# KennethLangedal/GNN-MWVC

Hardware: AMD Instinct MI355X
Metric: GNN forward edges/sec (higher is better)
Workload: dtype f32

## Files before the change

gnn-mwvc_amd/csrc/gnnvc_engine.cpp:

```cpp
#include <cmath>

#include "gnnvc_engine_state.h"

namespace {

struct Cursor {
    const char *p, *end;
    bool token(std::string &out) {
        while (p < end && isspace((unsigned char)*p)) ++p;
        if (p >= end) return false;
        const char *s = p;
        while (p < end && !isspace((unsigned char)*p)) ++p;
        out.assign(s, p);
        return true;
    }
    bool size(uint32_t &v) {
        std::string t;
        if (!token(t)) return false;
        char *q = nullptr;
        unsigned long x = strtoul(t.c_str(), &q, 10);
        if (!q || *q) return false;
        v = (uint32_t)x;
        return true;
    }
// ... 147 lines not shown
            const bool model_end = bare || at + 2 == left;
            const int end = bare ? gnnvc::kEndNone : L[at + 1].kind == kRelu ? gnnvc::kEndRelu
                            : (L[at + 1].kind == kSigmoid && model_end) ? gnnvc::kEndSigmoid : -1;
            gok = sp.nd < gnnvc::kMaxDenseLayers && (int)L[at].k == k && end >= 0;
            if (!gok) break;
            if (sp.nd == 0) sp.param_offset = L[at].w_off;
            sp.wn[sp.nd++] = k = (int)L[at].m;
            sp.end = end;
            sp.model_last = model_end;
            sp.sigmoid_last = end == gnnvc::kEndSigmoid;
            at += bare ? 1 : 2;
        }
        gok = gok && sp.nd >= 1 && (at == left || L[at].kind == kGraph);
        if (!gok) break;
        sp.n3 = sp.wn[sp.nd - 1];
        if (sp.nd == 3) { sp.n1 = sp.wn[0]; sp.n2 = sp.wn[1]; }
        sp.big_lds = e->big_lds;
        sp.feat_width = e->feat_width;
        gok = gnnvc::stage_any_fits(sp);
        gs.push_back(sp);
        f = sp.n3;
        i += at;
    }
    if (gok && !gs.empty()) e->gstages = std::move(gs);
}

int upload_params(gnnvc_engine *e) {
    std::vector<float> flat;
    for (const auto &l : e->layers)
        if (l.kind == kLinear) {
            flat.insert(flat.end(), l.W.begin(), l.W.end());
            flat.insert(flat.end(), l.bias.begin(), l.bias.end());
        }
    HIP_TRY(e, e->params.reserve(flat.size() + 64));
    if (!flat.empty())
        HIP_TRY(e, hipMemcpy(e->params.p, flat.data(), flat.size() * sizeof(float), hipMemcpyHostToDevice));
    return GNNVC_OK;
}

struct StageChoice {
    enum Sums {
        kGather,
        kLdsTable,
        kBlocked,
        kCompactPrepared,
        kCompactWhole,
        kTableTiles
    } sums = kGather;
    bool mfma = false;
    bool fused_counts = false;
    bool rounds = false;
    bool emit = false;
    bool emit_t4 = false;
    uint32_t long_thresh = 0xFFFFFFFFu;
    gnnvc::SortedOrder sorted;
};

int choose_stage(gnnvc_engine *e, int stage, uint32_t lo, uint32_t hi, const float *in, const float *out, bool in_forward,
                 StageChoice &c) {
    const bool longs = e->n_long > 0;
    const gnnvc::StagePlan &sp = e->stages[stage];
    if (e->pg.c4_prepared_stage != -1 && (stage != e->pg.c4_prepared_stage || out == e->c4_prepared_in)) e->pg.c4_prepared_stage = -1;
    const int fused_in = in_forward ? e->c4_fused_for : -1;
    e->c4_fused_for = -1;
    const bool may_emit = in_forward && e->pg.c4_ready && !e->pg.c4_range_mode && e->c4_base == 0 && e->c4_end == e->g.n && !longs &&
                          (size_t)stage + 1 < e->stages.size() && e->stages[stage + 1].f == 16 && lo == 0 && hi == e->g.n &&
                          e->opt.mfma != 1 && !e->pg.c4_stage_off[stage + 1];
    c.long_thresh = (sp.f == 16) ? e->thresh_f16 : e->long_thresh;
    c.mfma = e->opt.mfma == 1 || (e->opt.mfma == 2 && sp.f == 16);
    const bool t4 = in_forward && e->t4_now && lo == 0 && hi == e->g.n;
    c.emit_t4 = t4 && (size_t)stage + 1 < e->stages.size();
    if (stage == 0) {
        if (e->pg.graph_uses >= 1 && !e->pg.lt_tried) {
            int rc = build_lds_table(e);
            if (rc) return rc;
        }
        const uint32_t lt_need = std::min(192u, e->lt_chunks - e->lt_chunks / 4u);
        const bool lt_fits = e->pg.lt_ready && !e->pg.lt_off && hi > lo &&
                             (e->lt_mapped ? (lo == 0 && hi == e->g.n)
                                           : (lo >= e->lt_base && hi <= e->lt_end &&
                                              ((hi - 1 - e->lt_base) / e->lt_rows - (lo - e->lt_base) / e->lt_rows + 1) >= lt_need));
        if (e->pg.graph_uses >= 1 && !lt_fits && !e->pg.blocked_tried) {
            int rc = build_blocked(e);
            if (rc) return rc;
        }
        ++e->pg.graph_uses;
        c.sums = lt_fits ? StageChoice::kLdsTable : (e->pg.blocked_ready ? StageChoice::kBlocked : StageChoice::kGather);
        if (lt_fits && in_forward) e->pg.lt_used = true;
        if (lt_fits && e->lt_mapped) c.long_thresh = e->lt_plan_thresh;
        c.emit = may_emit;
        if (c.sums != StageChoice::kGather) return GNNVC_OK;
    } else if (sp.f == 16 && t4) {
        c.sums = StageChoice::kTableTiles;
    } else if (sp.f == 16) {
        const bool first_too = e->opt.compact_first_entries && e->g.nnz >= e->opt.compact_first_entries && lo == 0 && hi == e->g.n && in_forward;
        if (!e->pg.c4_range_mode && (e->pg.graph_uses >= 2 || first_too) && !e->pg.c4_tried) {
            int rc = build_compact(e);
            if (rc) return rc;
        }
        const bool whole_plan = e->pg.c4_ready && e->c4_base == 0 && e->c4_end == e->g.n && !e->pg.c4_stage_off[stage];
        const bool prepared = e->pg.c4_ready && e->pg.c4_prepared_stage == stage && e->c4_prepared_in == in &&
                              lo >= e->c4_base && hi <= e->c4_end && hi > lo;
        if (prepared && !longs) {
            const uint32_t nchunks = (hi - 1 - e->c4_base) / e->c4_rows - (lo - e->c4_base) / e->c4_rows + 1;
            if (nchunks >= 128u) c.sums = StageChoice::kCompactPrepared;
        } else if (!e->pg.c4_range_mode && whole_plan && !longs && (uint64_t)(hi - lo) * 2 >= e->g.n) {
// ... 41 lines not shown
        gr.off = e->gi_off.p;
        gr.slab = e->gi_slab.p;
        gr.agg = e->gi_agg.p;
        if (e->gi_maxseg > 1) {
            gr.segsum = e->gi_segsum.p;
            gr.segmap = e->gi_segmap.p;
            gr.maxseg = e->gi_maxseg;
        }
        gather_first = side && (e->opt.giant_gather_first < 0 ? (!long_on_main && (e->giant_entries <= (16ull << 20) || plain_f1))
                                                               : e->opt.giant_gather_first != 0);
        if (gather_first) HIP_TRY(e, gnnvc::launch_giant_stage(giant, gr, giant_from, gnnvc::GiantPart::kGather));
    }
    if (side) {
        HIP_TRY(e, hipEventRecord(e->ev_fork, e->stream));
        if (side_long) HIP_TRY(e, hipStreamWaitEvent(e->long_stream, e->ev_fork, 0));
    }
    if (e->n_giant) {
        if (long_on_main) HIP_TRY(e, hipStreamWaitEvent(e->giant_stream, e->ev_fork, 0));
        giant.stream = s_giant;
        HIP_TRY(e, gnnvc::launch_giant_stage(giant, gr, giant_from, gather_first ? gnnvc::GiantPart::kAfterGather : gnnvc::GiantPart::kAll));
        if (long_on_main) HIP_TRY(e, hipEventRecord(e->ev_giant, e->giant_stream));
    }
    const uint32_t long_from = gv.prune_eff ? std::min(thr, gv.eff_thresh) : thr;
    if ((e->n_giant < e->n_long || giant_from > e->giant_thresh) && long_from < giant_from) {
        gnnvc::StageCall lng = call;
        lng.stream = s_long;
        HIP_TRY(e, gnnvc::launch_long_stage(lng, {.list = e->long_list.p, .n = e->n_long, .min_deg = thr, .max_deg = giant_from}));
    }
    if (side_long) HIP_TRY(e, hipEventRecord(e->ev_long, e->long_stream));
    return GNNVC_OK;
}

int launch_main(gnnvc_engine *e, const StageChoice &c, const gnnvc::StageCall &call, const gnnvc::SortedOrder &so_p, int stage) {
    const gnnvc::StagePlan &sp = *call.sp;
    const GraphDev &gv = *call.g;
    const uint32_t lo = call.row_lo, hi = call.row_hi;
    const float *in = call.in;
    gnnvc::StageCall plain = call;
    plain.g = &e->g;
    gnnvc::EmitArgs emit;
    auto arm_emit = [&]() -> int {
        if (!c.emit) return GNNVC_OK;
        const bool zero = e->c4_emit_zero;
        e->c4_emit_zero = false;
        if (!zero) {
            ++e->plan_memsets;
            HIP_TRY(e, hipMemsetAsync(e->c4_emit_counts.p, 0, gnnvc::kEmitCounters * sizeof(unsigned long long), e->stream));
        }
        emit.spec = e->c4_desc.p + gnnvc_engine::kDescWords * stage;
        emit.table = e->c4_table.p;
        emit.counts = e->c4_emit_counts.p;
        e->c4_fused_for = stage + 1;
        return GNNVC_OK;
    };
    auto pilot = [&]() -> int {
        if (!c.emit || e->pg.c4_seeded[stage + 1] || !e->opt.pilot_rows) return GNNVC_OK;
        e->pg.c4_seeded[stage + 1] = true;
        const uint32_t rows = std::min(e->opt.pilot_rows, hi - lo);
        if ((uint64_t)rows * 8 > (uint64_t)(hi - lo)) return GNNVC_OK;
        uint32_t *cons = e->c4_desc.p + gnnvc_engine::kDescWords * stage;
        e->c4_emit_zero = false;
        ++e->plan_memsets;
        HIP_TRY(e, hipMemsetAsync(e->c4_emit_counts.p, 0, gnnvc::kEmitCounters * sizeof(unsigned long long), e->stream));
        gnnvc::EmitArgs pe;
        pe.spec = e->c4_desc.p + 2 * gnnvc_engine::kDescWords + 4;
        pe.table = e->c4_table.p;
        pe.counts = e->c4_emit_counts.p;
        gnnvc::StageCall first = plain;
        first.row_hi = lo + rows;
        first.logits = nullptr;
        HIP_TRY(e, gnnvc::launch_stage(first, {.interleave = true, .emit = pe}));
        HIP_TRY(e, gnnvc::compact_choose(e->c4_emit_counts.p, 64, rows, cons, 1u, e->stream, true));
        e->c4_emit_zero = true;
        return GNNVC_OK;
    };
    if (c.emit_t4) {
        const int cons = stage + 1;
        emit.spec = e->t4_desc_of(cons, e->t4_parity);
        emit.table = e->t4_table[cons - 1].p;
        emit.counts = e->t4_counts_of(cons, e->t4_parity);
    }
    if (c.sums == StageChoice::kTableTiles) {
        uint32_t *d_in = e->t4_desc_of(stage, e->t4_parity), *d_out = e->t4_desc_of(stage, e->t4_parity ^ 1u);
        const bool solo = e->t4_fit_seen[stage] && e->opt.t4_solo;
        HIP_TRY(e, gnnvc::launch_stage_t4(plain, {.table_in = e->t4_table[stage - 1].p,
                                                  .counts_in = e->t4_counts_of(stage, e->t4_parity),
                                                  .counts_zero = e->t4_counts_of(stage, e->t4_parity ^ 1u),
                                                  .desc_in = d_in, .desc_out = d_out, .emit = emit, .interleave = e->interleave, .solo = solo}));
        if (solo) return GNNVC_OK;
        return hip_rc(e, gnnvc::launch_stage(call, {.long_thresh = c.long_thresh, .mfma = c.mfma, .interleave = e->interleave,
                                                    .skip_flag = d_out + 8}));
    }
    if (c.sums == StageChoice::kLdsTable || c.sums == StageChoice::kBlocked) {
        int rc = pilot();
        if (rc) return rc;
        rc = arm_emit();
        if (rc) return rc;
    }
    if (c.sums == StageChoice::kLdsTable) {
        ++e->plan_memsets;
        return hip_rc(e, gnnvc::launch_stage0_lds_table(plain, lds_table_plan(e), e->lt_bytes.p, e->blk_acc.p, e->lt_bad.p,
                                                        {.long_thresh = c.long_thresh, .mfma = e->opt.mfma == 1,
                                                         .interleave = e->interleave, .emit = emit}));
    }
    if (c.sums == StageChoice::kBlocked)
        return hip_rc(e, gnnvc::launch_stage0_blocked(plain,
                                                      {.nblocks = e->blk_count, .bp = e->blk_ptr.p, .colb = e->blk_col.p, .acc = e->blk_acc.p},
                                                      {.long_thresh = e->long_thresh, .mfma = e->opt.mfma == 1,
                                                       .interleave = e->interleave, .emit = emit}));
    gnnvc::CompactSums sums;
    uint32_t *desc = nullptr;
    if (c.sums == StageChoice::kCompactPrepared || c.sums == StageChoice::kCompactWhole) {
        desc = e->c4_desc.p + gnnvc_engine::kDescWords * (stage - 1);
        e->c4_last_desc = gnnvc_engine::kDescWords * (stage - 1);
        if (c.sums == StageChoice::kCompactWhole) e->pg.fit_used[stage] = true;
        sums = {.acc4 = e->c4_acc.p, .c4desc = desc, .agg16 = e->c4_agg16.p, .table_in = (call.skip & 1u) ? e->c4_table.p : nullptr};
        const bool whole = c.sums == StageChoice::kCompactWhole;
        if (whole && !c.fused_counts) HIP_TRY(e, gnnvc::column_counts(in, e->g.n, e->c4_counts.p, e->stream));
        const bool fused = whole && c.fused_counts;
        const int what = !whole ? 2 : (c.rounds ? 1 : 3);
        if (fused) e->c4_emit_zero = false;
        if (!(what & 1)) ++e->plan_memsets;
        HIP_TRY(e, gnnvc::launch_compact_gather(e->g, compact_plan(e), in, fused ? e->c4_emit_counts.p : e->c4_counts.p, fused ? 64 : 1,
                                                desc, e->c4_table.p, e->c4_acc.p, lo, hi, e->c4_dirty.p, e->c4_dirty_cap,
                                                e->c4_agg16.p, e->stream, what, c.rounds ? e->c4_round_counts.p : nullptr, 256u * e->c4_rows, fused));
        if (fused) e->c4_emit_zero = true;
    }
    if (c.sums != StageChoice::kLdsTable && c.sums != StageChoice::kBlocked) {
        int rc = pilot();
        if (rc) return rc;
        rc = arm_emit();
        if (rc) return rc;
    }
    const gnnvc::SortedOrder *sop = c.sorted.n ? &c.sorted : nullptr;
    if (c.sums == StageChoice::kGather && e->opt.wide && e->g.n <= (sp.f == 16 ? e->opt.wide_max_n16 : e->opt.wide_max_n) && !e->g.sliced() && e->n_long == 0 && !sop &&
        !sums.acc4 && !emit.counts && gv.prune_bad == nullptr && gv.zero_bits == nullptr && sp.variant >= 0 && sp.variant <= 2) {
        e->pg.wide_used = true;
        e->stage_wide = true;
        return hip_rc(e, gnnvc::launch_stage_wide(plain));
    }
    HIP_TRY(e, gnnvc::launch_stage(call, {.long_thresh = c.long_thresh, .mfma = c.mfma, .so = sop, .interleave = e->interleave,
                                          .sums = sums, .mfma_agg = e->opt.mfma == 1, .emit = emit, .dense_part = !c.rounds,
                                          .so_pruned = so_p.vertex ? &so_p : nullptr}));
    if (!c.rounds) return GNNVC_OK;
    const uint32_t rows = e->c4_rows, c0 = (lo - e->c4_base) / rows, c1 = (hi - 1 - e->c4_base) / rows;
    const uint32_t nrounds = (c1 - c0) / 256u + 1u;
    if (nrounds > gnnvc::compact_rounds()) return fail(e, GNNVC_ERR_UNSUPPORTED, "too many rounds of the compact-table plan");
    {
        int rc = ensure_round_events(e, nrounds);
        if (rc) return rc;
    }
    for (uint32_t k = 0; k < nrounds; ++k) {
        const uint32_t ca = c0 + 256u * k, cb = std::min(c1 + 1u, ca + 256u);
        const uint32_t ra = std::max(lo, e->c4_base + ca * rows);
        const uint32_t rb = (uint32_t)std::min<uint64_t>(hi, (uint64_t)e->c4_base + (uint64_t)cb * rows);
        uint32_t *const count = e->c4_round_counts.p + k;
        const uint32_t slot_base = 256u * k * rows;
        HIP_TRY(e, gnnvc::compact_sums(e->g, compact_plan(e), desc, e->c4_table.p, e->c4_acc.p, ra, rb, e->c4_dirty.p, e->c4_dirty_cap,
                                       e->stream, count));
        const bool last = k + 1 == nrounds;
        hipStream_t ds = last ? e->stream : e->aux_stream;
        if (!last) {
            HIP_TRY(e, hipEventRecord(e->round_ev[k], e->stream));
            HIP_TRY(e, hipStreamWaitEvent(e->aux_stream, e->round_ev[k], 0));
        }
        HIP_TRY(e, gnnvc::compact_fix(e->g, in, desc, e->c4_dirty.p, e->c4_dirty_cap, e->c4_agg16.p, count, slot_base, ds,
                                      64));
        gnnvc::StageCall round = plain;
        round.row_lo = ra;
        round.row_hi = rb;
        round.stream = ds;
        HIP_TRY(e, gnnvc::launch_dense_sigmoid(round, sums, 0xFFFFFFFFu));
    }
    if (nrounds > 1) {
        HIP_TRY(e, hipEventRecord(e->ev_join, e->aux_stream));
        HIP_TRY(e, hipStreamWaitEvent(e->stream, e->ev_join, 0));
    }
    return GNNVC_OK;
}

std::string describe_stage(const gnnvc_engine *e, const StageChoice &c, const GraphDev &gv) {
    static const char *const kSums[] = {"gather", "lds_table", "blocked", "compact_prepared", "compact_whole", "table_tiles"};
    char buf[320];
    int at = snprintf(buf, sizeof buf, "sums=%s%s mfma=%d sorted_tiles=%d rounds=%d emit=%d pruned=%d filtered=%d short_lists=%d",
                      kSums[c.sums], e->stage_wide ? " (wide tiles)" : "", c.mfma ? 1 : 0, c.sorted.n ? 1 : 0, c.rounds ? 1 : 0,
                      (c.emit || c.emit_t4) ? 1 : 0, gv.prune_bad ? 1 : 0, gv.zero_bits ? 1 : 0, gv.short_col ? 1 : 0);
    if (e->n_long > 0 && at > 0 && at < (int)sizeof buf) {
        const char *lq = e->side_join == 1 ? "side" : "main";
        const char *gq = e->side_join == 0 ? "main" : (e->side_join == 1 ? "side" : "giant");
        at += snprintf(buf + at, sizeof buf - at, " long_rows=%u (from degree %u, %s queue)", e->n_long, c.long_thresh, lq);
        if (e->n_giant && at < (int)sizeof buf) snprintf(buf + at, sizeof buf - at, " giant_rows=%u (%s queue)", e->n_giant, gq);
    }
    return buf;
}

int run_stage(gnnvc_engine *e, int stage, uint32_t lo, uint32_t hi, const float *in, float *out, float *logits,
              bool in_forward = false, std::string *plan = nullptr) {
    e->stage_wide = false;
    StageChoice c;
    int rc = choose_stage(e, stage, lo, hi, in, out, in_forward, c);
    if (rc) return rc;
    const bool longs = e->n_long > 0;
    GraphDev gv;
    gnnvc::SortedOrder so_p;
    rc = gather_view(e, stage, lo, hi, in, c.sums == StageChoice::kGather, c.sorted.n != 0, gv, so_p, c.mfma, c.long_thresh);
    if (rc) return rc;
    gnnvc::StageCall call = stage_call(e, e->stages[stage], in, out, logits, lo, hi);
    call.g = &gv;
    if (longs) {
        rc = launch_side_rows(e, call, c.long_thresh, call.sp->f == 1 && c.sums == StageChoice::kGather);
        if (rc) return rc;
    }
    rc = launch_main(e, c, call, so_p, stage);
    if (rc) return rc;
    if (longs && e->side_join) {
        if (e->side_join == 1) HIP_TRY(e, hipStreamWaitEvent(e->stream, e->ev_long, 0));
        else if (e->n_giant) HIP_TRY(e, hipStreamWaitEvent(e->stream, e->ev_giant, 0));
    }
    if (plan) *plan = describe_stage(e, c, gv);
    return GNNVC_OK;
}

bool audit_tick(gnnvc_engine *e) {
    if (!e->opt.audit_period) return false;
    return ++e->audit_calls % e->opt.audit_period == 0;
}

int audit_stage(gnnvc_engine *e, int stage, uint32_t lo, uint32_t hi, const float *in, float *out, float *logits, std::string &plan,
                bool hook = true) {
    const std::vector<StagePlan> &st = e->stage_list();
    const size_t slot = e->audit_pending.size();
    if (slot == 0) {
        HIP_TRY(e, e->audit_rec.reserve(std::max<size_t>(st.size(), 1) * gnnvc::kAuditWords));
        HIP_TRY(e, hipMemsetAsync(e->audit_rec.p, 0, e->audit_rec.cap * sizeof(unsigned long long), e->stream));
    }
    if (slot >= st.size()) return fail(e, GNNVC_ERR_STATE, "more audited stages than the model has");
    const gnnvc::StagePlan &sp = st[stage];
    if (hook && e->opt.audit_flip_stage == stage && e->opt.audit_flip_row >= lo && e->opt.audit_flip_row < hi)
        HIP_TRY(e, gnnvc::launch_audit_flip(out, (size_t)e->opt.audit_flip_row * (size_t)sp.n3, e->stream));
    const gnnvc::StageCall call = stage_call(e, sp, in, out, sp.sigmoid_last ? logits : nullptr, lo, hi);
    unsigned long long *rec = e->audit_rec.p + slot * gnnvc::kAuditWords;
    if (e->generic_on()) HIP_TRY(e, gnnvc::launch_audit_any(call, rec, e->opt.audit_repair != 0));
    else HIP_TRY(e, gnnvc::launch_audit_stage(call, rec, e->opt.audit_repair != 0));
    e->audit_pending.push_back(gnnvc_engine::AuditCheck{stage, lo, hi, std::move(plan)});
    return GNNVC_OK;
}

int audit_finish(gnnvc_engine *e, int rc) {
    if (!e->audit_now) return rc;
    e->audit_now = false;
    std::vector<gnnvc_engine::AuditCheck> checks;
    checks.swap(e->audit_pending);
    if (rc != GNNVC_OK || checks.empty()) return rc;
    const size_t words = checks.size() * gnnvc::kAuditWords;
    HIP_TRY(e, e->audit_pin.reserve(std::max(e->stage_list().size(), checks.size()) * gnnvc::kAuditWords));
// ... 589 lines not shown
            unsigned long long info[2] = {0, 0};
            if (hipStreamSynchronize(e->stream) != hipSuccess ||
                hipMemcpy(info, e->filter_info.p + 4 * st, sizeof info, hipMemcpyDeviceToHost) != hipSuccess)
                return GNNVC_ERR_DEVICE;
            *value = (long)(info[0] * 100ull / e->g.nnz);
        }
    }
    else if (k == "pruned_vertices_stage1" || k == "pruned_vertices_stage2") *value = e->prune[k.back() - '0'].ready ? (long)e->prune[k.back() - '0'].members : 0;
    else if (k == "pruned_entries_stage1" || k == "pruned_entries_stage2") *value = e->prune[k.back() - '0'].ready ? (long)e->prune[k.back() - '0'].kept : 0;
    else if (k == "pruned_predicted_stage1") *value = e->prune[1].ready && e->prune[1].predicted ? 1 : 0;
    else if (k == "pruned_borrowed_stage2") *value = e->borrowed[2] ? 1 : 0;
    else if (k == "pruned_from_previous_stage2") *value = e->prune[2].ready && e->prune[2].from_prev ? 1 : 0;
    else if (k == "pruned_last_ok_stage1" || k == "pruned_last_ok_stage2") {
        const int st = k.back() - '0';
        *value = 0;
        if (e->prune[st].ready || e->borrowed[st]) {
            uint32_t bad = 1;
            if (hipSetDevice(e->device) != hipSuccess || hipStreamSynchronize(e->stream) != hipSuccess ||
                hipMemcpy(&bad, e->prune_flags.p + st, sizeof bad, hipMemcpyDeviceToHost) != hipSuccess)
                return GNNVC_ERR_DEVICE;
            *value = bad == 0 ? 1 : 0;
        }
    }
    else if (k == "wide_tiles_used") *value = e->pg.wide_used ? 1 : 0;
    else if (k == "table_tiles_active") *value = e->t4_ok ? 1 : 0;
    else if (k == "table_tiles_fit_stage1" || k == "table_tiles_fit_stage2") {
        *value = 0;
        if (e->t4_ok && e->t4_desc.p) {
            uint32_t fit = 0;
            gnnvc_engine *m = const_cast<gnnvc_engine *>(e);
            if (hipSetDevice(e->device) != hipSuccess || hipStreamSynchronize(e->stream) != hipSuccess ||
                hipMemcpy(&fit, m->t4_desc_of(k.back() - '0', e->t4_parity) + 8, sizeof fit, hipMemcpyDeviceToHost) != hipSuccess)
                return GNNVC_ERR_DEVICE;
            *value = (long)fit;
        }
    }
    else if (k == "lds_table_off") *value = e->pg.lt_off ? 1 : 0;
    else if (k == "lds_table_bits") *value = e->pg.lt_ready ? (long)e->lt_bits : 0;
    else if (k == "compact_gather_off_stage1" || k == "compact_gather_off_stage2") *value = e->pg.c4_stage_off[k.back() - '0'] ? 1 : 0;
    else if (k == "compact_gather_blocks") *value = e->pg.c4_ready ? (long)e->c4_nblocks : 0;
    else if (k == "compact_gather_last_ok" || k == "compact_gather_last_dirty" || k == "compact_gather_last_passes" ||
             k == "compact_table_written_by_producer") {
        *value = 0;
        if (e->pg.c4_ready && e->c4_desc.p) {
            uint32_t d[8] = {0};
            if (hipSetDevice(e->device) != hipSuccess || hipStreamSynchronize(e->stream) != hipSuccess ||
                hipMemcpy(d, e->c4_desc.p + e->c4_last_desc, sizeof d, hipMemcpyDeviceToHost) != hipSuccess)
                return GNNVC_ERR_DEVICE;
            if (k == "compact_table_written_by_producer") *value = (d[0] && !d[6]) ? 1 : 0;
            else *value = k == "compact_gather_last_ok" ? (d[0] ? 1 : 0) : (k == "compact_gather_last_passes" ? (long)d[0] : (long)d[5]);
        }
    }
    else if (k == "plan_memsets_last_forward") *value = (long)e->plan_memsets;
    else if (k == "lds_table_active") *value = e->pg.lt_ready ? 1 : 0;
    else if (k == "lds_table_last_ok") {
        *value = 0;
        if (e->pg.lt_ready && e->lt_bad.p) {
            uint32_t bad = 1;
            if (hipSetDevice(e->device) != hipSuccess || hipStreamSynchronize(e->stream) != hipSuccess ||
                hipMemcpy(&bad, e->lt_bad.p, sizeof bad, hipMemcpyDeviceToHost) != hipSuccess)
                return GNNVC_ERR_DEVICE;
            *value = bad == 0 ? 1 : 0;
        }
    }
    else if (k == "lds_table_mapped") *value = e->pg.lt_ready && e->lt_mapped ? 1 : 0;
    else if (k == "lds_table_blocks") *value = e->pg.lt_ready ? (long)e->lt_blocks : 0;
    else if (k == "lds_table_chunks") *value = e->pg.lt_ready ? (long)e->lt_chunks : 0;
    else if (k == "lds_table_steps") *value = e->pg.lt_ready ? (long)e->lt_steps_total : 0;
    else if (k == "blocked_stage0_active") *value = e->pg.blocked_ready ? 1 : 0;
    else if (k == "blocked_blocks") *value = e->pg.blocked_ready ? (long)e->blk_count : 0;
    else if (k == "block_cols") *value = e->pg.blocked_ready ? (long)e->blk_cols : 0;
    else if (k == "long_rows") *value = (long)e->n_long;
    else if (k == "plan_build_us") *value = (long)(e->pg.plan_build_ms * 1000.0);
    else if (k == "handoff_build_us") *value = (long)(e->handoff_build_ms * 1000.0);
    else if (k == "handoff_early_us") *value = (long)(e->pg.early_ms * 1000.0);
    else if (k == "graph_uses") *value = (long)e->pg.graph_uses;
    else if (k == "slice_rows") *value = e->empty_slice ? 0 : (long)(e->g.hi() - e->g.lo());
    else if (k == "slice_entries") *value = (long)e->g.nnz;
    else if (k == "giant_rows") *value = (long)e->n_giant;
    else if (k == "giant_segments") *value = e->n_giant ? (long)e->gi_maxseg : 0;
    else if (k == "giant_entries") *value = (long)e->giant_entries;
    else if (k == "giant_row_threshold") *value = e->n_giant ? (long)e->giant_thresh : 0;
    else if (k == "sorted_tiles_active") *value = e->sorted_wanted ? 1 : 0;
    else if (k == "tile_waste_x100") *value = (long)(e->srt_waste * 100.0);
    else if (k == "heavy_tail_x1000") *value = (long)(e->srt_tail * 1000.0);
    else if (k == "interleaved_tiles") *value = e->interleave ? 1 : 0;
    else if (k == "long_row_threshold") *value = e->n_long ? (long)e->long_thresh : 0;
    else return GNNVC_ERR_INVALID;
    return GNNVC_OK;
}

int gnnvc_num_layers(const gnnvc_engine *e) { return e ? (int)e->layers.size() : GNNVC_ERR_INVALID; }
int gnnvc_is_fused(const gnnvc_engine *e) { return e ? (e->stage_list().empty() ? 0 : 1) : GNNVC_ERR_INVALID; }
int gnnvc_in_width(const gnnvc_engine *e) { return e ? e->in_width : GNNVC_ERR_INVALID; }
int gnnvc_out_width(const gnnvc_engine *e) { return e ? e->out_width : GNNVC_ERR_INVALID; }
int gnnvc_num_stages(const gnnvc_engine *e) { return e ? (int)e->stage_list().size() : GNNVC_ERR_INVALID; }

int gnnvc_stage_widths(const gnnvc_engine *e, int stage, int *in_width, int *out_width) {
    if (!e || stage < 0 || stage >= (int)e->stage_list().size()) return GNNVC_ERR_INVALID;
    if (in_width) *in_width = e->stage_list()[stage].f;
    if (out_width) *out_width = e->stage_list()[stage].n3;
    return GNNVC_OK;
}

extern "C++" {
template <class RP>
// ... 494 lines not shown
        if (e->stage_list().empty()) return fail(e, GNNVC_ERR_UNSUPPORTED, "model is not fused into stages: there is nothing to audit");
        e->audit_now = true;
    } else {
        e->audit_now = audit && !e->stages.empty() && !e->generic_on();
    }
    const int rc = audit_finish(e, forward_single(e, d_x, d_scores, d_logits));
    if (audit && e->opt.audit_log) audit_log_line(e, rc);
    return rc;
}

int gnnvc_forward_device(gnnvc_engine *e, const float *d_x, float *d_scores, float *d_logits) {
    if (!e) return GNNVC_ERR_INVALID;
    return forward_device_impl(e, d_x, d_scores, d_logits, audit_tick(e), false);
}

int gnnvc_forward_audited_device(gnnvc_engine *e, const float *d_x, float *d_scores, float *d_logits) {
    if (!e) return GNNVC_ERR_INVALID;
    return forward_device_impl(e, d_x, d_scores, d_logits, true, true);
}

static int forward_single(gnnvc_engine *e, const float *d_x, float *d_scores, float *d_logits) {
    if (!e->have_graph) return fail(e, GNNVC_ERR_STATE, "no graph attached");
    const uint32_t n = e->g.n;
    e->ev_count = 0;
    e->live_seen.clear();
    if (e->layers.empty()) return fail(e, GNNVC_ERR_STATE, "engine was created without a model");
    if (n == 0) return GNNVC_OK;
    if (e->g.sliced() || e->empty_slice)
        return fail(e, GNNVC_ERR_STATE, "this engine holds a slice of the graph: run it stage by stage (gnnvc_stage_forward_device)");
    if (!d_x || !d_scores) return fail(e, GNNVC_ERR_INVALID, "null feature buffers");
    int rc = use_device(e);
    if (rc) return rc;
    e->plan_memsets = 0;
    e->generic_ran = e->generic_on();
    e->heavy_last_rows = 0;
    e->ggiant_last_rows = 0;
    e->ggiant_last_segmented = false;
    if (e->generic_ran || e->stages.empty()) {
        rc = ensure_events(e, 2);
        if (rc) return rc;
        if (e->opt.timing >= 1) HIP_TRY(e, hipEventRecord(e->ev[0], e->stream));
        rc = e->generic_ran ? forward_generic(e, d_x, d_scores, d_logits) : forward_unfused(e, d_x, d_scores, d_logits);
        if (rc) return rc;
        if (e->opt.timing >= 1) HIP_TRY(e, hipEventRecord(e->ev[1], e->stream));
        e->ev_count = e->opt.timing >= 1 ? 2 : 0;
        e->ev_stages = false;
        return GNNVC_OK;
    }
    const size_t ns = e->stages.size();
    rc = ensure_events(e, ns + 1);
    if (rc) return rc;
    const float *cur = d_x;
    e->c4_fused_for = -1;
    e->pg.c4_prepared_stage = -1;
    if (e->pg.fit_pending && hipEventQuery(e->ev_fit) == hipSuccess) {
        e->pg.fit_pending = false;
        const uint32_t before = e->pg.lt_unfit_runs + e->t4_unfit_runs + e->pg.c4_unfit_runs[1] + e->pg.c4_unfit_runs[2];
        const bool seen1 = e->t4_fit_seen[1], seen2 = e->t4_fit_seen[2];
        if (e->pg.lt_used && e->pg.lt_ready) {
            e->pg.lt_unfit_runs = e->fit_pin.p[2] != 0u ? e->pg.lt_unfit_runs + 1 : 0u;
            if (e->pg.lt_unfit_runs >= (e->lt_mapped ? 1u : 3u)) e->pg.lt_off = true;
        }
        if (e->t4_used && e->t4_ok) {
            e->t4_unfit_runs = e->fit_pin.p[3] == 0u ? e->t4_unfit_runs + 1 : 0u;
            if (e->t4_unfit_runs >= 4u) e->t4_ok = false;
            e->t4_fit_seen[1] = e->fit_pin.p[3] != 0u;
            e->t4_fit_seen[2] = e->fit_pin.p[4] != 0u;
        }
        for (int s = 1; s <= 2; ++s) {
            if (!e->pg.fit_used[s]) continue;
            if (s == 2 && e->pg.fit_used[1] && e->fit_pin.p[0] == 0u) continue;
            e->pg.c4_unfit_runs[s] = e->fit_pin.p[s - 1] == 0u ? e->pg.c4_unfit_runs[s] + 1 : 0u;
            if (e->pg.c4_unfit_runs[s] >= 3u) e->pg.c4_stage_off[s] = true;
        }
        const uint32_t after = e->pg.lt_unfit_runs + e->t4_unfit_runs + e->pg.c4_unfit_runs[1] + e->pg.c4_unfit_runs[2];
        const bool calm = after == 0u && before == 0u && seen1 == e->t4_fit_seen[1] && seen2 == e->t4_fit_seen[2];
        e->pg.fit_calm = calm ? e->pg.fit_calm + 1u : 0u;
    }
    if (!e->pg.fit_pending) {
        for (int s = 0; s < 4; ++s) e->pg.fit_used[s] = false;
        e->pg.lt_used = false;
        e->t4_used = false;
    }
    struct SinkGuard {
        ~SinkGuard() { gnnvc::set_kernel_trace(nullptr); }
    } sink_guard;
    if (e->opt.ktrace && e->ktrace.used < 16384) {
        e->ktrace.stream = e->stream;
        gnnvc::set_kernel_trace(&e->ktrace);
    }
    e->t4_now = e->t4_ok && (e->t4_choice_live || e->pg.graph_uses >= 1);
    const bool build_under_stage0 = ns >= 2 && !e->pg.c4_tried && !e->pg.c4_range_mode && e->aux_stream && e->n_long == 0 && !e->sorted_wanted &&
                                    e->opt.compact_first_entries && e->g.nnz >= e->opt.compact_first_entries;
    if (e->opt.timing >= 1 || build_under_stage0) HIP_TRY(e, hipEventRecord(e->ev[0], e->stream));
    if (e->opt.poison)
        for (size_t b = 0; b + 1 < ns && b < 2; ++b) HIP_TRY(e, hipMemsetAsync(e->h[b].p, 0xFF, (size_t)n * 16 * sizeof(float), e->stream));
    for (size_t s = 0; s < ns; ++s) {
        const bool last = s + 1 == ns;
        float *dst = last ? d_scores : e->h[s & 1].p;
        std::string plan;
        rc = run_stage(e, (int)s, 0, n, cur, dst, last ? d_logits : nullptr, true, e->audit_now ? &plan : nullptr);
        if (rc) break;
        if (e->audit_now && (rc = audit_stage(e, (int)s, 0, n, cur, dst, last ? d_logits : nullptr, plan)) != GNNVC_OK) break;
        if ((e->opt.timing >= 2 || (last && e->opt.timing == 1)) && hipEventRecord(e->ev[s + 1], e->stream) != hipSuccess) { rc = fail(e, GNNVC_ERR_DEVICE, "hipEventRecord failed"); break; }
        if (s == 0 && build_under_stage0 && !e->pg.c4_tried) {
            HIP_TRY(e, hipStreamWaitEvent(e->aux_stream, e->ev[0], 0));
// ... 511 lines not shown
```

gnn-mwvc_amd/csrc/gnnvc_engine_state.h:

```cpp
#pragma once
#include <hip/hip_runtime_api.h>

#include <algorithm>
#include <chrono>
#include <cctype>
#include <cstdarg>
#include <cstdio>
#include <cstdlib>
#include <cstring>
#include <new>
#include <string>
#include <vector>

#include "../../include/gnnvc.h"
#include "gnnvc_device_mem.h"
#include "gnnvc_kernels.h"
#include "gnnvc_multi.h"
#include "gnnvc_options.h"

using gnnvc::GraphDev;
using gnnvc::StagePlan;

namespace gnnvc_eng {

// ... 13 lines not shown
using gnnvc::PinBuf;
using gnnvc_eng::Layer;
using namespace gnnvc_eng;

struct gnnvc_engine {
    int device = 0;
    gnnvc::MultiState *multi = nullptr;
    std::string name;
    std::vector<Layer> layers;
    std::vector<StagePlan> stages;
    std::vector<StagePlan> gstages;
    bool generic_ran = false;
    uint32_t big_lds = 0;
    uint32_t feat_width = 0;
    uint32_t patterns = 0;
    uint32_t live_percent = 0;
    std::vector<uint8_t> live_seen;
    bool generic_on() const { return !gstages.empty() && (opt.generic == 2 || (opt.generic == 1 && stages.empty())); }
    const std::vector<StagePlan> &stage_list() const { return generic_on() ? gstages : stages; }
    uint32_t heavy_from = 512;
    uint32_t heavy_last_rows = 0;
    uint32_t ggiant_from = 16384;
    int ggiant_segments = -1;
    uint32_t ggiant_last_rows = 0;
    bool ggiant_last_segmented = false;
    int in_width = 1, out_width = 1;
    int max_width = 1;
    bool ends_in_sigmoid = false;
    float ws = 120.0f;

    gnnvc::Options opt;
    gnnvc::Stream own_stream, aux_stream;
    hipStream_t stream = nullptr;
    std::vector<gnnvc::Event> ev;
    int ev_count = 0;
    bool ev_stages = false;

    DevBuf<float> params;
    struct PerGraph {
        bool wide_used = false;
        bool blocked_ready = false, blocked_tried = false;
        uint32_t graph_uses = 0;
        bool lt_ready = false, lt_tried = false;
        bool lt_used = false, lt_off = false;
        uint32_t lt_unfit_runs = 0;
        bool c4_ready = false, c4_tried = false;
        bool c4_range_mode = false;
        int c4_prepared_stage = -1;
        bool c4_seeded[4] = {false, false, false, false};
        bool fit_pending = false, fit_used[4] = {false, false, false, false}, c4_stage_off[4] = {false, false, false, false};
        uint32_t c4_unfit_runs[4] = {0, 0, 0, 0};
        uint32_t fit_calm = 0;
        uint32_t fit_skip = 0;
        int short_from = 0;
        bool heavy_known = false;
        uint32_t heavy_rows = 0, heavy_thresh = 0;
        uint64_t heavy_entries = 0;
        uint32_t giant_from = 0, giant_rows = 0, giant_blocks = 0, giant_maxseg = 0, giant_min = 0xFFFFFFFFu;
        int giant_seg = -1;
        uint64_t giant_entries = 0;
        double plan_build_ms = 0.0;
        double early_ms = 0.0;
    };
    PerGraph pg;
    GraphDev g;
    bool have_graph = false;
    DevBuf<uint32_t> rowptr, col, w, nw;
    PinBuf<uint32_t> pin_rowptr, pin_col, pin_w, pin_nw;
    PinBuf<uint32_t> pin_small;
    uint32_t staged_n = 0;
    uint64_t staged_nnz = 0, staged_sent = 0;
    bool staging = false;
    DevBuf<float> x, h[2], scores, logits;
    DevBuf<float> scratch[2];
    DevBuf<float> live_table;
    DevBuf<unsigned long long> live_desc;

    uint32_t blk_count = 0, blk_cols = 0;
    DevBuf<uint32_t> blk_ptr, blk_col, blk_scratch, blk_flag;
    DevBuf<float> blk_acc;
    uint32_t lt_bits = 8;
    bool lt_mapped = false;
    uint32_t lt_plan_thresh = 0xFFFFFFFFu;
    DevBuf<uint32_t> lt_rowmap, lt_first, lt_bstart;
    uint32_t lt_rows = 0, lt_chunks = 0, lt_blocks = 0, lt_steps_total = 0, lt_last_entry = 0;
    uint32_t lt_base = 0, lt_end = 0;
    struct PlanBuild {
        bool open = false, mapped = false;
        uint32_t base = 0, end = 0, slice_rows = 0, slices = 0, chunks = 0, rows = 0, nblocks = 0, bc = 0, slack = 0, done = 0;
        uint32_t plan_rows = 0, passes = 1;
        uint64_t entry_cap = 0, plan_nnz = 0;
        gnnvc::PlanMap pm;
    };
    PlanBuild lt_pb, c4_pb;
    bool early_open = false, early_declined = false;
    gnnvc::Event ev_piece;
    DevBuf<uint8_t> lt_bytes;
    DevBuf<uint32_t> lt_entries, lt_segcnt, lt_stepptr, lt_stepcnt, lt_bad;
    DevBuf<uint4> lt_steps;
    uint32_t c4_rows = 0, c4_chunks = 0, c4_steps_total = 0, c4_block = 0, c4_last_entry = 0, c4_nblocks = 0;
    DevBuf<uint32_t> c4_entries, c4_segcnt, c4_stepptr, c4_stepcnt, c4_desc;
    uint32_t c4_nslices = 0;
    DevBuf<uint32_t> c4_map_vertex;
    DevBuf<uint32_t> map_coarse;
    DevBuf<uint4> c4_map_meta;
    DevBuf<uint4> c4_steps;
    DevBuf<float> c4_table, c4_acc, c4_agg16;
    DevBuf<uint32_t> c4_round_counts;
    std::vector<gnnvc::Event> round_ev;
    DevBuf<uint32_t> c4_dirty;
    uint32_t c4_dirty_cap = 0;
    DevBuf<unsigned long long> c4_counts, c4_emit_counts;
    uint32_t plan_memsets = 0;
    bool c4_emit_zero = false;
    uint32_t c4_base = 0, c4_end = 0;
    const float *c4_prepared_in = nullptr;
    int c4_fused_for = -1;
    struct PrunePlan {
        bool tried = false, ready = false, deferred = false;
        bool predicted = false, verified = false;
        void forget() { tried = ready = deferred = predicted = verified = false; }
        bool from_prev = false;
        uint64_t kept = 0;
        uint64_t members = 0;
        DevBuf<uint32_t> prp, pcol, heavy;
        DevBuf<uint32_t> svertex;
        DevBuf<uint4> smeta;
        uint32_t sn = 0;
        bool slist = false;
        uint32_t eff_thresh = 0xFFFFFFFFu;
    };
    PrunePlan prune[4];
    DevBuf<uint32_t> prune_flags, prune_scratch, prune_off;
    DevBuf<unsigned long long> prune_mask;
    int side_join = 0;
    DevBuf<uint32_t> filter_bits[4];
    DevBuf<unsigned long long> filter_info;
    bool filtered[4] = {false, false, false, false};
    bool borrowed[4] = {false, false, false, false};
    uint32_t short_min = 0, short_max = 0;
    bool short_used[4] = {false, false, false, false};
    PinBuf<uint32_t> fit_pin;
    gnnvc::Event ev_fit;
    int c4_last_desc = 0;
    static constexpr int kDescWords = 16;

    bool t4_ok = false;
    bool t4_used = false;
    bool t4_fit_seen[4] = {false, false, false, false};
    uint32_t t4_unfit_runs = 0;
    uint32_t *fit_dev = nullptr;
    bool t4_now = false;
    bool t4_choice_live = false;
    uint32_t t4_parity = 0;
    DevBuf<float> t4_table[2];
    DevBuf<uint32_t> t4_desc;
    DevBuf<unsigned long long> t4_counts[2];
    unsigned long long *t4_counts_of(int stage, uint32_t parity) { return t4_counts[stage - 1].p + (size_t)parity * gnnvc::kEmitCounters; }
    uint32_t *t4_desc_of(int stage, uint32_t parity) { return t4_desc.p + ((size_t)(stage - 1) * 2 + parity) * 16; }

    uint32_t thresh_f16 = 0xFFFFFFFFu;
    bool interleave = false;
    bool sorted_wanted = false;
    struct SortedRange {
        bool valid = false, use = false;
        uint32_t lo = 0, hi = 0, n = 0;
        uint64_t stamp = 0;
        DevBuf<uint32_t> vertex;
        DevBuf<uint4> meta;
// ... 172 lines not shown
```

gnn-mwvc_amd/csrc/gnnvc_kernels.h:

```cpp
#pragma once
#include <hip/hip_runtime_api.h>
#include <stdint.h>
#include <hip/hip_vector_types.h>

#include <atomic>
#include <vector>

#include "gnnvc_device_mem.h"

namespace gnnvc {

struct GraphDev {
    uint32_t n = 0;
    uint64_t nnz = 0;
    const uint32_t *rowptr = nullptr;
    const uint32_t *col = nullptr;
    const uint32_t *w = nullptr;
    const uint32_t *nw = nullptr;
    uint32_t row_base = 0, row_end = 0;
    const uint32_t *prp = nullptr, *pcol = nullptr, *prune_bad = nullptr;
    uint32_t prune_eff = 0, eff_giant = 0xFFFFFFFFu, eff_thresh = 0xFFFFFFFFu;
    const uint32_t *zero_bits = nullptr;
    const unsigned long long *zero_info = nullptr;
    uint32_t zero_min_pct = 50;
// ... 14 lines not shown
};

constexpr int kMaxDenseLayers = 6;
struct StagePlan {
    int f = 0;
    int n1 = 0, n2 = 0, n3 = 0;
    int sigmoid_last = 0;
    size_t param_offset = 0;
    int variant = -1;
    int nd = 3;
    int wn[kMaxDenseLayers] = {0, 0, 0, 0, 0, 0};
    uint32_t big_lds = 0;
    uint32_t feat_width = 0;
    int dense = 0;
    int end = 0;
    int model_last = 0;
    uint32_t patterns = 0;
    uint32_t skip_ok = 0;
};

struct SortedOrder {
    uint32_t n = 0;
    const uint32_t *vertex = nullptr;
    const uint4 *meta = nullptr;
};

struct KernelTraceSink {
    struct Rec {
        const char *name = nullptr;
        Event a, b;
    };
    hipStream_t stream = nullptr;
    std::vector<Rec> recs;
    size_t used = 0;
};
void set_kernel_trace(KernelTraceSink *sink);

int stage_variant(int f, int n1, int n2, int n3, int sigmoid_last);

struct StageCall {
    const StagePlan *sp = nullptr;
    const GraphDev *g = nullptr;
    float ws = 0.0f;
    const float *params = nullptr;
    const float *in = nullptr;
    float *out = nullptr, *logits = nullptr;
    uint32_t row_lo = 0, row_hi = 0;
    hipStream_t stream = nullptr;
    uint32_t skip = 0;
    float *live_table = nullptr;
    void *live_desc = nullptr;
};

struct EmitArgs {
    const uint32_t *spec = nullptr;
    float *table = nullptr;
    unsigned long long *counts = nullptr;
};
constexpr int kEmitCounters = 64 * 17;

struct CompactSums {
    const float *acc4 = nullptr;
    const uint32_t *c4desc = nullptr;
    const float *agg16 = nullptr;
    const float *table_in = nullptr;
};

struct TileArgs {
    uint32_t long_thresh = 0xFFFFFFFFu;
    bool mfma = false;
    const SortedOrder *so = nullptr;
    bool interleave = false;
    CompactSums sums;
    const uint32_t *skip_flag = nullptr;
    bool mfma_agg = false;
    EmitArgs emit;
    bool dense_part = true;
    const SortedOrder *so_pruned = nullptr;
};
hipError_t launch_stage(const StageCall &c, const TileArgs &a);
struct GraphClassArgs {
    bool cuts = false, waste = false, longs = false;
    uint32_t waste_thresh = 0xFFFFFFFFu, heavy_from = 1, long_thresh = 0xFFFFFFFFu;
    uint32_t *long_list = nullptr;
};
hipError_t classify_graph(const GraphDev &g, const GraphClassArgs &a, uint32_t *dev_words, uint32_t *out_dev, hipStream_t stream);

struct VerdictWords {
    const uint32_t *src[8] = {nullptr, nullptr, nullptr, nullptr, nullptr, nullptr, nullptr, nullptr};
};
hipError_t write_verdicts(const VerdictWords &vw, uint32_t *out_dev, hipStream_t stream);

constexpr int kAuditWords = 8;
hipError_t launch_audit_stage(const StageCall &c, unsigned long long *rec, bool repair);
hipError_t launch_audit_any(const StageCall &c, unsigned long long *rec, bool repair);
hipError_t launch_audit_flip(float *out, size_t at, hipStream_t stream);

constexpr int kAnyMaxF = 32, kAnySmallHidden = 64, kAnyBigHidden = 128, kAnyMaxLast = 32;
constexpr int kAnyFeatMax = 64;
constexpr uint32_t kPatternPrologue = 1u, kPatternOpenEnd = 2u;
enum { kEndRelu = 0, kEndSigmoid = 1, kEndNone = 2 };
struct AnyRoute {
    bool ok = false, big = false, feat = false;
    int threads = 256;
    size_t lds256 = 0, lds = 0;
};
AnyRoute stage_any_route(const StagePlan &sp);
bool stage_any_fits(const StagePlan &sp);
hipError_t allow_big_stages();
hipError_t allow_feat_stages();
hipError_t allow_dynamic_lds(const void *func, int bytes, std::atomic<uint64_t> &done);
struct AnyHeavyRows {
    const uint32_t *list = nullptr;
    uint32_t n = 0, from = 0;
    float *hsum = nullptr;
    uint32_t below = 0xFFFFFFFFu;
};
enum class AnyRows { kAll, kLight, kListed };
hipError_t launch_stage_any(const StageCall &c, AnyRows rows = AnyRows::kAll, const AnyHeavyRows &hr = AnyHeavyRows());
hipError_t launch_any_heavy_sums(const StageCall &c, const AnyHeavyRows &hr);
hipError_t launch_any_live(const StageCall &c, uint32_t max_percent);

hipError_t launch_stage_wide(const StageCall &c);
struct TableTileArgs {
    const float *table_in = nullptr;
    const unsigned long long *counts_in = nullptr;
    unsigned long long *counts_zero = nullptr;
    const uint32_t *desc_in = nullptr;
    uint32_t *desc_out = nullptr;
// ... 16 lines not shown

hipError_t find_long_rows(const GraphDev &g, uint32_t thresh, uint32_t *list, uint32_t *count,
                          hipStream_t stream);
struct LongRows {
    const uint32_t *list = nullptr;
    uint32_t n = 0, min_deg = 0, max_deg = 0xFFFFFFFFu;
};
hipError_t launch_long_stage(const StageCall &c, const LongRows &lr);

struct GiantRows {
    uint32_t n = 0, blocks = 0;
    const void *meta = nullptr;
    const unsigned long long *off = nullptr;
    float *slab = nullptr, *agg = nullptr;
    float *segsum = nullptr;
    void *segmap = nullptr;
    uint32_t maxseg = 0;
};
uint32_t giant_segments(uint32_t len);
uint32_t giant_window();
uint32_t giant_block();
hipError_t find_giant_rows(const GraphDev &g, const uint32_t *list, uint32_t n_long, uint32_t thresh, void *meta, uint32_t *count,
                           hipStream_t stream);
enum class GiantPart { kAll, kGather, kAfterGather };
hipError_t launch_giant_stage(const StageCall &c, const GiantRows &gr, uint32_t min_deg, GiantPart part);
hipError_t launch_giant_sums(const GiantRows &gr, uint32_t F, uint32_t row_lo, uint32_t row_hi, hipStream_t stream);

struct AnyGiantRows {
    GiantRows gr;
    const uint32_t *pos = nullptr;
};
hipError_t find_any_giant_rows(const GraphDev &g, const uint32_t *list, uint32_t n_list, uint32_t thresh, void *meta, uint32_t *count,
                               hipStream_t stream);
enum class AnyGiantPart { kGather, kPlace };
hipError_t launch_any_giant(const StageCall &c, const AnyGiantRows &ar, float *hsum, AnyGiantPart part);
hipError_t stream_sums(const float *streams_dev, uint32_t streams, uint32_t len, void *meta, unsigned long long *off, float *agg,
                       int mode , hipStream_t stream, float *segsum = nullptr,
                       void *segmap = nullptr);

size_t blocked_scan_scratch_elems(size_t n_elems);
hipError_t build_blocked_index(const GraphDev &g, uint32_t wb, uint32_t nblocks, uint32_t long_thresh,
                               uint32_t *bp, uint32_t *colb, uint32_t *scratch, uint32_t *bad_flag,
                               hipStream_t stream);
struct BlockedPlan {
    uint32_t nblocks = 0;
    const uint32_t *bp = nullptr, *colb = nullptr;
    float *acc = nullptr;
};
struct Stage0Args {
    uint32_t long_thresh = 0xFFFFFFFFu;
    bool mfma = false;
    bool interleave = false;
    EmitArgs emit;
};
hipError_t launch_stage0_blocked(const StageCall &c, const BlockedPlan &bp, const Stage0Args &a);

hipError_t launch_graph_layer(const GraphDev &g, float ws, uint32_t f, const float *in,
                              float *out, hipStream_t stream);
hipError_t launch_linear(uint32_t n, uint32_t k, uint32_t m, const float *in, const float *W,
                         const float *bias, float *out, hipStream_t stream);
hipError_t launch_relu(size_t count, const float *in, float *out, hipStream_t stream);
hipError_t launch_sigmoid(size_t count, const float *in, float *out, hipStream_t stream);
hipError_t launch_sgemm(int ta, int tb, uint32_t m, uint32_t n, uint32_t k, const float *A,
                        uint32_t lda, const float *B, uint32_t ldb, float beta, float *C,
                        uint32_t ldc, hipStream_t stream);

uint32_t lds_table_max_rows(uint32_t bits = 8);
uint32_t lds_table_bits_for(uint32_t kmax);
size_t lds_table_bytes_for(uint32_t bits, size_t n);
hipError_t lds_table_wmax(const uint32_t *w, uint32_t n, uint32_t *wmax, hipStream_t stream);
struct PlanMap {
    const uint32_t *rowmap = nullptr, *first = nullptr, *bstart = nullptr;
    const uint16_t *coarse = nullptr;
};
uint32_t lds_table_block(uint32_t bits = 8);
uint32_t lds_table_step();
uint32_t lds_table_record_words();
hipError_t lds_table_wsteps(const GraphDev &g, uint32_t slice_rows, uint32_t nchunks, uint32_t nblocks, const uint32_t *seg_cnt,
                            const uint32_t *step_ptr, uint32_t *step_count, uint32_t *recs, bool write, uint32_t slack,
                            hipStream_t stream, const PlanMap &pm = PlanMap(), uint32_t row_base = 0, uint32_t row_end = 0xFFFFFFFFu,
                            uint32_t bits = 8);
bool lds_table_is_flat(uint32_t rows_per_chunk, const PlanMap &pm = PlanMap());
hipError_t lds_table_count(const GraphDev &g, uint32_t rows_per_chunk, uint32_t nchunks, uint32_t nblocks, uint32_t block_cols,
                           uint32_t *seg_cnt, uint32_t *bad, hipStream_t stream, uint32_t row_base = 0,
                           uint32_t row_end = 0xFFFFFFFFu, const PlanMap &pm = PlanMap(), uint32_t chunk0 = 0,
                           uint32_t chunk1 = 0xFFFFFFFFu);
hipError_t lds_table_steps(const GraphDev &g, uint32_t rows_per_chunk, uint32_t nchunks, uint32_t nblocks, const uint32_t *seg_cnt,
                           const uint32_t *step_ptr, uint32_t *step_count, void *steps, bool write, hipStream_t stream,
                           uint32_t row_base = 0, uint32_t row_end = 0xFFFFFFFFu, uint32_t cap = 0 ,
                           uint32_t slack = 0 ,
                           uint32_t block_cols = 0 ,
                           const PlanMap &pm = PlanMap());
hipError_t lds_table_scatter(const GraphDev &g, uint32_t rows_per_chunk, uint32_t nchunks, uint32_t nblocks, uint32_t block_cols,
                             const uint32_t *seg_cnt, uint32_t *entries, hipStream_t stream, uint32_t shift,
                             uint32_t row_base, uint32_t row_end, uint32_t slack, const PlanMap &pm,
                             uint32_t *bad ,
                             uint32_t chunk0 = 0, uint32_t chunk1 = 0xFFFFFFFFu);
hipError_t prune_mark_zero(const GraphDev &g, const float *feat, uint32_t *heavy_bits, hipStream_t stream);
hipError_t predict_zero_rows(const StagePlan &sp0, const GraphDev &g, float ws, const float *params, uint32_t *heavy_bits, hipStream_t stream);
hipError_t filter_mark(const GraphDev &g, const float *feat, uint32_t *bits, unsigned long long *info, hipStream_t stream,
                       const uint32_t *prev_bits = nullptr, const unsigned long long *prev_info = nullptr);
hipError_t prune_mass(const GraphDev &g, const uint32_t *heavy_bits, unsigned long long *mass, hipStream_t stream,
                      const uint32_t *prev_bits = nullptr);
hipError_t prune_count(const GraphDev &g, const uint32_t *heavy_bits, unsigned long long *mask, uint32_t *off, uint32_t *scratch,
                       hipStream_t stream);
hipError_t prune_fill(const GraphDev &g, const unsigned long long *mask, const uint32_t *off, uint32_t *pcol, uint32_t *prp,
                      hipStream_t stream);
hipError_t prune_check(const GraphDev &g, const float *feat, const uint32_t *heavy_bits, uint32_t *bad, hipStream_t stream);
hipError_t deal_rows(const GraphDev &g, const uint32_t *sorted_rows, uint32_t m, uint32_t slice_rows, uint32_t nslices,
                     uint32_t *rowmap, uint32_t *weight, hipStream_t stream);
hipError_t mass_bounds(const GraphDev &g, unsigned long long target, uint32_t count, uint32_t *cand, hipStream_t stream);
struct LdsTablePlan {
    uint32_t rows_per_chunk = 0;
    uint32_t plan_base = 0, plan_end = 0xFFFFFFFFu;
    uint32_t bits = 8;
    uint32_t last_entry = 0;
    uint32_t mapped_chunks = 0;
    const uint32_t *step_ptr = nullptr;
    const void *steps = nullptr;
    const uint32_t *entries = nullptr;
    const uint32_t *rowmap = nullptr;
};
hipError_t launch_stage0_lds_table(const StageCall &c, const LdsTablePlan &lp, uint8_t *wbyte, float *acc, uint32_t *bad,
                                   const Stage0Args &a);

uint32_t compact_max_rows();
uint32_t compact_block();
uint32_t compact_shift();
uint32_t compact_slices();
uint32_t compact_step();
uint32_t compact_rounds();
struct CompactPlan {
    uint32_t rows_per_chunk = 0, block_cols = 0, nblocks = 0, plan_base = 0, plan_end = 0;
    uint32_t last_entry = 0;
    uint32_t nslices = 0;
    uint32_t max_passes = 1;
    const uint32_t *step_ptr = nullptr;
    const void *steps = nullptr;
    const uint32_t *entries = nullptr;
    const uint32_t *rowmap = nullptr;
};
hipError_t launch_compact_gather(const GraphDev &g, const CompactPlan &cp, const float *in, unsigned long long *counts,
                                 int count_slots, uint32_t *desc, float *table, float *acc4, uint32_t row_lo, uint32_t row_hi,
                                 uint32_t *dirty_rows, uint32_t dirty_cap, float *agg16, hipStream_t stream,
                                 int what = 3 ,
                                 uint32_t *round_counts = nullptr ,
                                 uint32_t round_stride = 0 ,
                                 bool clear_counts = false );

hipError_t compact_choose(unsigned long long *counts, int count_slots, uint32_t rows, uint32_t *desc, uint32_t max_passes,
                          hipStream_t stream, bool clear_counts = false);
hipError_t compact_sums(const GraphDev &g, const CompactPlan &cp, uint32_t *desc, const float *table, float *acc4, uint32_t row_lo,
                        uint32_t row_hi, uint32_t *dirty_rows, uint32_t dirty_cap, hipStream_t stream,
                        uint32_t *round_count = nullptr);
hipError_t compact_fix(const GraphDev &g, const float *in, uint32_t *desc, const uint32_t *dirty_rows, uint32_t dirty_cap,
                       float *agg16, const uint32_t *dirty_count, uint32_t slot_base, hipStream_t stream, uint32_t blocks = 1024);

hipError_t derive_tails(const GraphDev &old_g, const uint32_t *old_row, uint32_t n_new, const uint32_t *rowptr_new, uint32_t *new_of,
                        uint32_t *tail, uint32_t *bad, hipStream_t stream);
hipError_t derive_fill(const GraphDev &old_g, const uint32_t *old_row, const uint32_t *new_of, const uint32_t *rowptr_new,
                       const uint32_t *tail_ptr, const uint32_t *tail_cols, uint32_t n_new, uint32_t *col_new, hipStream_t stream);
hipError_t row_hashes(const GraphDev &g, unsigned long long *out, hipStream_t stream);

hipError_t score_keys(const float *scores, size_t n, float *keys, uint8_t *above_half, hipStream_t stream);

hipError_t live_columns(const float *feat, size_t rows, uint32_t *mask, hipStream_t stream);
hipError_t column_counts(const float *feat, size_t rows, unsigned long long *counts, hipStream_t stream);
hipError_t pack_rows(const float *feat, uint32_t row_lo, uint32_t row_hi, uint32_t mask, uint32_t kp, float *dense,
                     uint32_t *exc, uint32_t cap, uint32_t *flag, hipStream_t stream);
hipError_t unpack_rows(const float *dense, const uint32_t *exc, uint32_t cap, uint32_t row_lo, uint32_t row_hi,
                       uint32_t mask, uint32_t kp, float *feat, hipStream_t stream);

hipError_t unpack_gathered(const float *buf, uint32_t world, uint32_t skip, size_t piece_words, uint32_t dense_rows,
                           uint32_t cap, uint32_t per, uint32_t off, uint32_t size, uint32_t n, uint32_t mask, uint32_t kp,
                           float *feat, hipStream_t stream);

struct UnpackPiece {
    const float *region;
    uint32_t row_lo, row_hi;
};
hipError_t push_piece(const float *region, uint32_t rows, uint32_t kp, uint32_t cap, uint32_t n_dst, float *const *dst, hipStream_t stream);
hipError_t unpack_pieces(const UnpackPiece *pieces, uint32_t n_pieces, uint32_t cap, uint32_t mask, uint32_t kp, float *feat, hipStream_t stream);
hipError_t push_rows(const float *src, size_t words, uint32_t n_dst, float *const *dst, hipStream_t stream);

hipError_t launch_reduction_flags(const GraphDev &g, uint32_t max_degree, uint8_t *flags, hipStream_t stream);

hipError_t validate_graph(const GraphDev &g, uint32_t *flags, hipStream_t stream);
hipError_t validate_rowptr(const GraphDev &g, uint32_t *flags, hipStream_t stream);
hipError_t narrow_rowptr(const void *in_u64, uint32_t *out, size_t count, hipStream_t stream);

hipError_t streams_run_side_by_side(hipStream_t a, hipStream_t b, bool *yes);
hipError_t launch_zero_pad_row(float *buf, uint32_t n, uint32_t width, hipStream_t stream);

}
```

gnn-mwvc_amd/csrc/gnnvc_kernels.hip:

```cpp
#include <hip/hip_runtime.h>

#include <algorithm>
#include <atomic>

#include "exact_sum.h"
#include "expf_glibc.h"
#include "gnnvc_kernels.h"

namespace gnnvc {

namespace {

#ifndef GNNVC_PHASE_PROBE
#define GNNVC_PHASE_PROBE 0
#endif
#if GNNVC_PHASE_PROBE
__device__ unsigned long long *gnnvc_probe_buf = nullptr;
__device__ int gnnvc_probe_kind = 0;
__device__ __forceinline__ void probe_mark(int kind, int phase) {
    if (gnnvc_probe_buf && gnnvc_probe_kind == kind && (threadIdx.x & 63) == 0)
        gnnvc_probe_buf[((size_t)blockIdx.x * 4 + (threadIdx.x >> 6)) * 16 + phase] = wall_clock64();
}
#define GNNVC_PROBE(kind, phase) probe_mark(kind, phase)
#else
// ... 200 lines not shown
    float acc = 0.0f;
#pragma unroll
    for (int r = 0; r < 4; ++r) acc = __builtin_fmaf(d[r], w[r], acc);
    float t = __shfl_xor(acc, 32);
    acc = h ? t : acc;
#pragma unroll
    for (int r = 0; r < 4; ++r) acc = __builtin_fmaf(d[r], w[r], acc);
    t = __shfl_xor(acc, 32);
    acc = h ? acc : t;
#pragma unroll
    for (int r = 4; r < 8; ++r) acc = __builtin_fmaf(d[r], w[r], acc);
    t = __shfl_xor(acc, 32);
    acc = h ? t : acc;
#pragma unroll
    for (int r = 4; r < 8; ++r) acc = __builtin_fmaf(d[r], w[r], acc);
    return acc;
}

template <int N1, int N2, int N3, bool SIGMOID>
__device__ __forceinline__ void mfma_tail(f32x16 (&d)[2], const float *__restrict__ W2, const float *__restrict__ b2,
                                          const float *__restrict__ W3, const float *__restrict__ b3, float *T,
                                          int v, int h, float (&logit)[2]) {
    static_assert(N1 == 32, "layer-2 input is a full 32-feature tile");
    float a[16];
    mfma_load_a<N2, 16>(W2, v, h, a);
#pragma unroll
    for (int vt = 0; vt < 2; ++vt) {
        d[vt] = mfma_layer_acc<32>(d[vt], a);
        mfma_bias_act<N2, 0>(d[vt], b2, h);
    }
    if constexpr (SIGMOID) {
        static_assert(N2 == 16 && N3 == 1, "sigmoid tail is 16 -> 1");
#pragma unroll
        for (int vt = 0; vt < 2; ++vt) logit[vt] = mfma_tail_16to1(d[vt], W3, h) + b3[0];
    } else {
        static_assert(N3 == 16, "feature stages emit 16 floats per vertex");
        mfma_load_a<N3, N2 / 2>(W3, v, h, a);
#pragma unroll
        for (int vt = 0; vt < 2; ++vt) {
            d[vt] = mfma_layer_acc<N2>(d[vt], a);
            mfma_bias_act<N3, 0>(d[vt], b3, h);
        }
        wave_lds_sync();
#pragma unroll
        for (int vt = 0; vt < 2; ++vt)
#pragma unroll
            for (int r = 0; r < 8; ++r) T[(32 * vt + v) * kOutPitch + mfma_feat(r, h)] = d[vt][r];
    }
}

typedef float c4row __attribute__((ext_vector_type(4)));
constexpr int kEmitSlots = 64, kEmitStride = 17;

__device__ __forceinline__ void c4_emit_with(const float *trow, uint32_t nz, uint32_t u, bool mine, int lane, uint32_t spec_ok,
                                             uint32_t s0, uint32_t s1, uint32_t s2, uint32_t s3, c4row *__restrict__ table,
                                             unsigned long long *__restrict__ counts) {
    uint32_t my = 0;
#pragma unroll
    for (int cidx = 0; cidx < 16; ++cidx) {
        const uint32_t cnt = (uint32_t)__popcll(__ballot(mine && (nz >> cidx & 1u)));
        if (lane == cidx) my = cnt;
    }
    const uint32_t rows = (uint32_t)__popcll(__ballot(mine));
    if (lane == 16) my = rows;
    if (lane <= 16 && my) atomicAdd(&counts[(blockIdx.x & (kEmitSlots - 1)) * kEmitStride + lane], (unsigned long long)my);
    if (spec_ok == 1u && mine) {
        const float a = trow[s0], b = trow[s1], c = trow[s2], d = trow[s3];
        c4row out = {a == 0.0f ? 0.0f : a, b == 0.0f ? 0.0f : b, c == 0.0f ? 0.0f : c, d == 0.0f ? 0.0f : d};
        const bool odd = !(a >= 0.0f) || !(b >= 0.0f) || !(c >= 0.0f) || !(d >= 0.0f);
        if (odd || (nz & ~((1u << s0) | (1u << s1) | (1u << s2) | (1u << s3))))
            out[0] = __uint_as_float(__float_as_uint(out[0]) | 0x80000000u);
        if (odd) out[1] = __uint_as_float(__float_as_uint(out[1]) | 0x80000000u);
        table[u] = out;
    }
}
__device__ __forceinline__ void c4_emit(const float *trow, uint32_t nz, uint32_t u, bool mine, int lane,
                                        const uint32_t *__restrict__ spec, c4row *__restrict__ table,
                                        unsigned long long *__restrict__ counts) {
    const uint32_t ok = spec[0];
    c4_emit_with(trow, nz, u, mine, lane, ok, ok == 1u ? spec[1] : 0u, ok == 1u ? spec[2] : 0u, ok == 1u ? spec[3] : 0u,
                 ok == 1u ? spec[4] : 0u, table, counts);
}

template <int LANE>
__device__ __forceinline__ uint32_t put_lane(uint32_t v, uint32_t s ) {
    asm("v_writelane_b32 %0, %1, %2" : "+v"(v) : "s"(s), "n"(LANE));
    return v;
}
template <int J>
__device__ __forceinline__ void c4_count_cols(const float (&x)[16], unsigned long long mm, uint32_t tcols, uint32_t &my,
                                              unsigned long long &stray) {
    if constexpr (J < 16) {
        const unsigned long long nzj = __ballot(x[J] != 0.0f);
        my = put_lane<J>(my, (uint32_t)__popcll(nzj & mm));
        stray |= (tcols >> J & 1u) ? 0ull : nzj;
        c4_count_cols<J + 1>(x, mm, tcols, my, stray);
    }
}
__device__ __forceinline__ void c4_emit_regs(const float (&x)[16], const float *trow, uint32_t u, bool mine, int lane,
                                             const uint32_t *__restrict__ spec, c4row *__restrict__ table,
                                             unsigned long long *__restrict__ counts) {
    const uint32_t ok = spec[0];
    const uint32_t s0 = ok == 1u ? spec[1] : 0u, s1 = ok == 1u ? spec[2] : 0u, s2 = ok == 1u ? spec[3] : 0u, s3 = ok == 1u ? spec[4] : 0u;
    const uint32_t tcols = (1u << (s0 & 31u)) | (1u << (s1 & 31u)) | (1u << (s2 & 31u)) | (1u << (s3 & 31u));
    const unsigned long long mm = __ballot(mine);
    unsigned long long stray = 0;
    uint32_t my = 0;
    c4_count_cols<0>(x, mm, tcols, my, stray);
    my = put_lane<16>(my, (uint32_t)__popcll(mm));
    if (lane <= 16 && my) atomicAdd(&counts[(blockIdx.x & (kEmitSlots - 1)) * kEmitStride + lane], (unsigned long long)my);
    if (ok == 1u && mine) {
        const float a = trow[s0], b = trow[s1], c = trow[s2], d = trow[s3];
        c4row out = {a == 0.0f ? 0.0f : a, b == 0.0f ? 0.0f : b, c == 0.0f ? 0.0f : c, d == 0.0f ? 0.0f : d};
        const bool odd = !(a >= 0.0f) || !(b >= 0.0f) || !(c >= 0.0f) || !(d >= 0.0f);
        if (odd || (stray >> lane & 1ull)) out[0] = __uint_as_float(__float_as_uint(out[0]) | 0x80000000u);
        if (odd) out[1] = __uint_as_float(__float_as_uint(out[1]) | 0x80000000u);
        table[u] = out;
    }
}

#ifndef GNNVC_EMIT_REGS
#define GNNVC_EMIT_REGS 1
#endif
__device__ __forceinline__ void c4_emit_row(const float (&x)[16], const float *trow, uint32_t u, bool mine, int lane,
                                            const uint32_t *__restrict__ spec, c4row *__restrict__ table,
                                            unsigned long long *__restrict__ counts) {
    if constexpr (GNNVC_EMIT_REGS) {
        c4_emit_regs(x, trow, u, mine, lane, spec, table, counts);
    } else {
        uint32_t nz = 0;
#pragma unroll
        for (int j = 0; j < 16; ++j) nz |= (x[j] != 0.0f ? 1u : 0u) << j;
        c4_emit(trow, nz, u, mine, lane, spec, table, counts);
    }
}

__device__ __forceinline__ bool filter_worth_info(const GraphDev &g, const unsigned long long *info) {
    return info[0] * 100ull >= g.nnz * (unsigned long long)g.zero_min_pct;
}
__device__ __forceinline__ bool filter_worth(const GraphDev &g) { return g.zero_bits != nullptr && filter_worth_info(g, g.zero_info); }

template <int N1, int N2, int N3, bool SIGMOID, int S, bool MFMA, bool SORTED, bool AGGONLY = false, bool FILTER = false>
__global__ __launch_bounds__(kBlock) __attribute__((amdgpu_waves_per_eu(3))) void k_stage_f16(
        GraphDev g, float ws, const float4 *__restrict__ fin, float *__restrict__ fout,
        float *__restrict__ logits, const float *__restrict__ P, uint32_t row_lo,
        uint32_t row_hi, uint32_t long_thresh, const uint32_t *__restrict__ srt_vertex,
        const uint4 *__restrict__ srt_meta, uint32_t n_sorted, int interleave,
        const float4 *__restrict__ acc4, const uint32_t *__restrict__ c4desc, const float4 *__restrict__ agg16,
        const uint32_t *__restrict__ emit_spec, c4row *__restrict__ emit_table, unsigned long long *__restrict__ emit_counts,
        const uint32_t *__restrict__ srt_vertex_p = nullptr, const uint4 *__restrict__ srt_meta_p = nullptr, uint32_t n_sorted_p = 0) {
    __shared__ __attribute__((aligned(16))) float lds[kWavesPerBlock][kRegionFloats];
    const int lane = threadIdx.x & 63;
    GNNVC_PROBE((SIGMOID ? 2 : 1), 0);
    float *T = lds[threadIdx.x >> 6];
    uint32_t *stage = reinterpret_cast<uint32_t *>(T);
    if constexpr (AGGONLY) {
        if (c4desc[0] == 0) return;
    } else {
        if (c4desc && c4desc[0] != 0) return;
    }
    const bool pruned = !AGGONLY && g.prune_bad != nullptr && *g.prune_bad == 0u;
    const uint32_t *__restrict__ grp = pruned ? g.prp : g.rowptr;
    const uint32_t *__restrict__ gcol = pruned ? g.pcol : g.col;
    const bool by_left = pruned && g.prune_eff != 0u;
    const bool filt = FILTER && !pruned && filter_worth(g);
    if (SORTED && by_left) {
        srt_vertex = srt_vertex_p;
        srt_meta = srt_meta_p;
        n_sorted = n_sorted_p;
    }
    const uint32_t ntiles = SORTED ? (n_sorted + kWave - 1) / kWave : (row_hi - row_lo + kWave - 1) / kWave;
    const uint32_t grid_tiles = SORTED ? (max(n_sorted, n_sorted_p) + kWave - 1) / kWave : ntiles;
    uint32_t tile = tile_for_wave(grid_tiles, SORTED || interleave);
    if (tile >= ntiles) return;
    if (SORTED && GNNVC_SORTED_MIX) {
        tile = (tile & 1u) ? ntiles - 1u - (tile >> 1) : (tile >> 1);
    }
    const uint32_t v0 = row_lo + tile * kWave;

    uint32_t u, rs, re;
    bool mine;
    float f_deg, f_w, f_nw;
    if constexpr (SORTED) {
        const uint32_t slot = tile * kWave + lane;
        mine = slot < n_sorted;
        const uint32_t sl = mine ? slot : n_sorted - 1;
// ... 216 lines not shown
}

template <int N>
__device__ __forceinline__ void fma_term(f32x2 (&acc)[N / 2], float a, const float *__restrict__ Wrow) {
    const f32x2 aa = {a, a};
#pragma unroll
    for (int j = 0; j < N / 2; ++j) acc[j] = __builtin_elementwise_fma(aa, f32x2{Wrow[2 * j], Wrow[2 * j + 1]}, acc[j]);
}
template <int N>
__device__ __forceinline__ uint32_t bias_relu(const f32x2 (&acc)[N / 2], float (&out)[N], const float *__restrict__ b) {
    uint32_t live = 0;
#pragma unroll
    for (int j = 0; j < N; ++j) out[j] = relu_live(acc[j / 2][j % 2] + b[j], live);
    return live;
}
template <int K, int N>
__device__ __forceinline__ uint32_t dense_relu_live(const float (&in)[K], float (&out)[N], const float *__restrict__ W,
                                                    const float *__restrict__ b) {
    f32x2 acc[N / 2];
#pragma unroll
    for (int j = 0; j < N / 2; ++j) acc[j] = f32x2{0.0f, 0.0f};
#pragma unroll
    for (int k = 0; k < K; ++k) fma_term<N>(acc, in[k], W + k * N);
    return bias_relu<N>(acc, out, b);
}
template <int K, int N>
__device__ __forceinline__ void live_terms(f32x2 (&acc)[N / 2], const float (&in)[K], const float *__restrict__ W, uint32_t all) {
    static_assert(K % 2 == 0, "inputs in pairs");
    f32x2 pin[K / 2];
#pragma unroll
    for (int k = 0; k < K / 2; ++k) {
        pin[k] = f32x2{in[2 * k], in[2 * k + 1]};
        asm volatile("" : "+v"(pin[k]));
    }
#pragma unroll
    for (int k = 0; k < K; ++k) {
        const float a = pin[k / 2][k % 2];
        if (__any(((__float_as_uint(a) << 1) | all) != 0u)) fma_term<N>(acc, a, W + k * N);
#pragma unroll
        for (int j = 0; j < N / 2; ++j) asm volatile("" : "+v"(acc[j]));
    }
}
#ifndef GNNVC_ROUTE_C_GROUPS
#define GNNVC_ROUTE_C_GROUPS 1
#endif

template <int N1, int N2, int N3, bool SIGMOID>
__global__ __launch_bounds__(kBlock) void k_dense_f16(GraphDev g, float ws, const float4 *__restrict__ fin, float *__restrict__ fout,
                                                      float *__restrict__ logits, const float *__restrict__ P, uint32_t row_lo,
                                                      uint32_t row_hi, const float4 *__restrict__ acc4,
                                                      const uint32_t *__restrict__ c4desc, const float4 *__restrict__ agg16,
                                                      const float4 *table_in , uint32_t long_thresh,
                                                      const uint32_t *__restrict__ emit_spec, c4row *__restrict__ emit_table,
                                                      unsigned long long *__restrict__ emit_counts, uint32_t skip) {
    static_assert(SIGMOID ? N3 == 1 : N3 == 16, "a feature stage writes 16 floats per row, the last stage one score");
    __shared__ float lds[SIGMOID ? 1 : kWavesPerBlock][SIGMOID ? 1 : kWave * kOutPitch];
    if (c4desc[0] == 0) return;
    const int lane = threadIdx.x & 63;
    const uint32_t uu = row_lo + blockIdx.x * kBlock + threadIdx.x;
    const uint32_t u = uu < row_hi ? uu : row_hi - 1;
    const uint32_t deg = g.rowptr[u + 1] - g.rowptr[u];
    const bool mine = uu < row_hi && deg < long_thresh;
    const uint32_t npass = c4desc[0];
    const uint32_t d0 = c4desc[1], d1 = c4desc[2], d2 = c4desc[3], d3 = c4desc[4];
    const float4 a = acc4[u];
    const bool dirty = (__float_as_uint(a.x) >> 31) != 0;
    const float4 t = (table_in != nullptr && npass == 1u) ? table_in[u] : make_float4(-0.0f, 0.f, 0.f, 0.f);
    const bool stray = (__float_as_uint(t.x) >> 31) != 0;
    const float f_deg = (float)deg, f_w = (float)g.w[u] / ws, f_nw = (float)g.nw[u] / ws;
    const float *W1 = P, *b1 = W1 + 35 * N1;
    const float *W2 = b1 + N1, *b2 = W2 + N1 * N2;
    const float *W3 = b2 + N2, *b3 = W3 + N2 * N3;
    float x1[N1];
    uint32_t live1;
    const bool ascending = (d0 < d1 || d1 == 0xFFFFFFFFu) && (d1 < d2 || d2 == 0xFFFFFFFFu) && (d2 < d3 || d3 == 0xFFFFFFFFu);
    if (!__any(stray) && (ascending || !__any(dirty))) {
        static_assert(N1 % 2 == 0, "outputs in pairs");
        f32x2 acc[N1 / 2];
        auto own_terms = [&]() {
            if (d0 == 0u) fma_term<N1>(acc, t.x, W1 + 16 * N1);
            fma_term<N1>(acc, f_deg, W1 + 17 * N1);
            fma_term<N1>(acc, f_w, W1 + 18 * N1);
            fma_term<N1>(acc, f_nw, W1 + 19 * N1);
            if (d0 >= 4u && d0 < 16u) fma_term<N1>(acc, t.x, W1 + (16u + d0) * N1);
            if (d1 >= 4u && d1 < 16u) fma_term<N1>(acc, t.y, W1 + (16u + d1) * N1);
            if (d2 >= 4u && d2 < 16u) fma_term<N1>(acc, t.z, W1 + (16u + d2) * N1);
            if (d3 >= 4u && d3 < 16u) fma_term<N1>(acc, t.w, W1 + (16u + d3) * N1);
        };
#pragma unroll
        for (int j = 0; j < N1 / 2; ++j) acc[j] = f32x2{0.0f, 0.0f};
        if (!__any(dirty)) {
            if (d0 < 16u) fma_term<N1>(acc, a.x, W1 + d0 * N1);
            if (d1 < 16u) fma_term<N1>(acc, a.y, W1 + d1 * N1);
            if (d2 < 16u) fma_term<N1>(acc, a.z, W1 + d2 * N1);
            if (d3 < 16u) fma_term<N1>(acc, a.w, W1 + d3 * N1);
        } else {
            const size_t slot = dirty ? (size_t)__float_as_uint(a.y) : 0;
            const float4 g0 = agg16[slot * 4], g1 = agg16[slot * 4 + 1], g2 = agg16[slot * 4 + 2], g3 = agg16[slot * 4 + 3];
            const float gg[16] = {g0.x, g0.y, g0.z, g0.w, g1.x, g1.y, g1.z, g1.w, g2.x, g2.y, g2.z, g2.w, g3.x, g3.y, g3.z, g3.w};
            float v[16], c0 = a.x, c1 = a.y, c2 = a.z, c3 = a.w;
            uint32_t e0 = d0, e1 = d1, e2 = d2, e3 = d3;
#pragma unroll
            for (int k = 0; k < 16; ++k) {
                float clean = 0.0f;
                if ((uint32_t)k == e0) {
                    clean = c0;
                    c0 = c1; c1 = c2; c2 = c3;
                    e0 = e1; e1 = e2; e2 = e3; e3 = 0xFFFFFFFFu;
                }
                v[k] = dirty ? gg[k] : clean;
                asm volatile("" : "+v"(v[k]));
            }
#pragma unroll
            for (int k = 0; k < 16; ++k)
                if (__any((__float_as_uint(v[k]) << 1) != 0u)) fma_term<N1>(acc, v[k], W1 + k * N1);
        }
        own_terms();
        live1 = bias_relu<N1>(acc, x1, b1);
    } else if constexpr (GNNVC_ROUTE_C_GROUPS) {
        const uint32_t all = (skip & 1u) ? 0u : 1u;
        f32x2 acc[N1 / 2];
        {
            float s[16];
#pragma unroll
            for (int k = 0; k < 16; ++k) s[k] = 0.0f;
            for (uint32_t qp = 0; qp < npass; ++qp) {
                const uint32_t *dc = c4desc + (qp == 0 ? 1 : 4 + 4 * qp);
                const uint32_t e0 = dc[0], e1 = dc[1], e2 = dc[2], e3 = dc[3];
                const float4 aq = qp == 0 ? a : acc4[(size_t)qp * g.n + u];
#pragma unroll
                for (int k = 0; k < 16; ++k)
                    s[k] = ((uint32_t)k == e0) ? aq.x : ((uint32_t)k == e1) ? aq.y : ((uint32_t)k == e2) ? aq.z : ((uint32_t)k == e3) ? aq.w : s[k];
            }
            if (__any(dirty)) {
                const size_t slot = dirty ? (size_t)__float_as_uint(a.y) : 0;
                const float4 g0 = agg16[slot * 4], g1 = agg16[slot * 4 + 1], g2 = agg16[slot * 4 + 2], g3 = agg16[slot * 4 + 3];
                const float gg[16] = {g0.x, g0.y, g0.z, g0.w, g1.x, g1.y, g1.z, g1.w, g2.x, g2.y, g2.z, g2.w, g3.x, g3.y, g3.z, g3.w};
#pragma unroll
                for (int k = 0; k < 16; ++k) s[k] = dirty ? gg[k] : s[k];
            }
#pragma unroll
            for (int j = 0; j < N1 / 2; ++j) acc[j] = f32x2{0.0f, 0.0f};
            live_terms<16, N1>(acc, s, W1, all);
        }
        size_t own = (size_t)u * 4;
        {
            float s[4] = {fin[own].x, f_deg, f_w, f_nw};
            live_terms<4, N1>(acc, s, W1 + 16 * N1, all);
        }
        {
            asm volatile("" : "+v"(own));
            const float4 h1 = fin[own + 1], h2 = fin[own + 2], h3 = fin[own + 3];
            float s[12] = {h1.x, h1.y, h1.z, h1.w, h2.x, h2.y, h2.z, h2.w, h3.x, h3.y, h3.z, h3.w};
            live_terms<12, N1>(acc, s, W1 + 20 * N1, all);
        }
        live1 = bias_relu<N1>(acc, x1, b1);
    } else {
        const float4 h0 = fin[(size_t)u * 4], h1 = fin[(size_t)u * 4 + 1], h2 = fin[(size_t)u * 4 + 2], h3 = fin[(size_t)u * 4 + 3];
        float x0[32];
#pragma unroll
        for (int k = 0; k < 16; ++k) x0[k] = 0.0f;
        for (uint32_t qp = 0; qp < npass; ++qp) {
            const uint32_t *dc = c4desc + (qp == 0 ? 1 : 4 + 4 * qp);
            const uint32_t e0 = dc[0], e1 = dc[1], e2 = dc[2], e3 = dc[3];
            const float4 aq = qp == 0 ? a : acc4[(size_t)qp * g.n + u];
#pragma unroll
            for (int k = 0; k < 16; ++k)
                x0[k] = ((uint32_t)k == e0) ? aq.x : ((uint32_t)k == e1) ? aq.y : ((uint32_t)k == e2) ? aq.z : ((uint32_t)k == e3) ? aq.w : x0[k];
        }
        if (__any(dirty)) {
            const size_t slot = dirty ? (size_t)__float_as_uint(a.y) : 0;
            const float4 g0 = agg16[slot * 4], g1 = agg16[slot * 4 + 1], g2 = agg16[slot * 4 + 2], g3 = agg16[slot * 4 + 3];
            const float gg[16] = {g0.x, g0.y, g0.z, g0.w, g1.x, g1.y, g1.z, g1.w, g2.x, g2.y, g2.z, g2.w, g3.x, g3.y, g3.z, g3.w};
#pragma unroll
            for (int k = 0; k < 16; ++k) x0[k] = dirty ? gg[k] : x0[k];
        }
        x0[16] = h0.x;
        x0[17] = f_deg;
        x0[18] = f_w;
        x0[19] = f_nw;
        x0[20] = h1.x; x0[21] = h1.y; x0[22] = h1.z; x0[23] = h1.w;
        x0[24] = h2.x; x0[25] = h2.y; x0[26] = h2.z; x0[27] = h2.w;
        x0[28] = h3.x; x0[29] = h3.y; x0[30] = h3.z; x0[31] = h3.w;
        live1 = dense_live<32, N1, 0>(x0, x1, W1, b1, (skip & 1u) != 0);
    }
    float x2[N2], x3[N3];
    const uint32_t live2 = dense_live<N1, N2, 0, !SIGMOID>(x1, x2, W2, b2, (skip & 2u) != 0, live1);
    if constexpr (SIGMOID) dense<N2, N2, N3, 1>(x2, x3, W3, b3);
    else dense_live<N2, N3, 0, true>(x2, x3, W3, b3, (skip & 4u) != 0, live2);
    if constexpr (SIGMOID) {
        if (mine) {
            if (logits) logits[u] = x3[0];
            fout[u] = sigmoid_ref(x3[0]);
        }
    } else {
        float *T = lds[threadIdx.x >> 6];
#pragma unroll
        for (int j = 0; j < 16; ++j) T[lane * kOutPitch + j] = x3[j];
        if (emit_counts) c4_emit_row(x3, &T[lane * kOutPitch], u, mine, lane, emit_spec, emit_table, emit_counts);
        wave_lds_sync();
        const int q = lane >> 2, c = lane & 3;
#pragma unroll
        for (int p = 0; p < 4; ++p) {
            const int src_lane = 16 * p + q;
            const float *src = &T[src_lane * kOutPitch + 4 * c];
            const float4 o = make_float4(src[0], src[1], src[2], src[3]);
            const uint32_t row = __shfl(u, src_lane);
            if (__shfl((int)mine, src_lane)) reinterpret_cast<float4 *>(fout)[(size_t)row * 4 + c] = o;
        }
    }
}

struct T4Choice {
    uint32_t fit, d0, d1, d2, d3;
};
__device__ __forceinline__ T4Choice t4_choose(const unsigned long long *__restrict__ counts, uint32_t n, const uint32_t *__restrict__ desc_in,
                                              uint32_t *__restrict__ desc_out, int lane, bool write) {
    unsigned long long part[kEmitStride], mine = 0;
#pragma unroll
    for (int t = 0; t < kEmitStride; ++t) part[t] = counts[t * 64 + lane];
    for (int c = 0; c < kEmitStride; ++c) {
        unsigned long long v = 0;
#pragma unroll
        for (int t = 0; t < kEmitStride; ++t) v += ((t * 64 + lane) % kEmitStride == c) ? part[t] : 0ull;
#pragma unroll
        for (int off = 32; off; off >>= 1)
            v += ((unsigned long long)__shfl_xor((unsigned)(v >> 32), off) << 32) | __shfl_xor((unsigned)v, off);
        if (lane == c) mine = v;
    }
    const unsigned long long rows = ((unsigned long long)__shfl((unsigned)(mine >> 32), 16) << 32) | __shfl((unsigned)mine, 16);
    const bool prev_ok = desc_in[0] == 1u && rows == n;
    const uint32_t p1 = desc_in[1], p2 = desc_in[2], p3 = desc_in[3], p4 = desc_in[4];
    T4Choice r = {0u, 0xFFFFFFFFu, 0xFFFFFFFFu, 0xFFFFFFFFu, 0xFFFFFFFFu};
    uint32_t np = 0;
    if (rows == n) {
        const unsigned long long c = lane < 16 ? mine : 0ull;
        uint32_t rank = 0;
#pragma unroll
        for (int k = 0; k < 16; ++k) {
            const unsigned long long ck = ((unsigned long long)__shfl((unsigned)(c >> 32), k) << 32) | __shfl((unsigned)c, k);
            rank += (ck > c || (ck == c && k < lane)) ? 1u : 0u;
        }
        unsigned long long rest = (lane < 16 && rank >= 4u) ? c : 0ull;
#pragma unroll
        for (int off = 8; off; off >>= 1)
            rest += ((unsigned long long)__shfl_xor((unsigned)(rest >> 32), off) << 32) | __shfl_xor((unsigned)rest, off);
        rest = ((unsigned long long)__shfl((unsigned)(rest >> 32), 0) << 32) | __shfl((unsigned)rest, 0);
        if (rest <= (unsigned long long)n / 512) np = 1;
        const unsigned long long cm = np ? __ballot(lane < 16 && rank < 4u) : 0ull;
        const uint32_t m0 = (uint32_t)cm, m1 = m0 & (m0 - 1), m2 = m1 & (m1 - 1), m3 = m2 & (m2 - 1);
        r.d0 = m0 ? (uint32_t)__builtin_ctz(m0) : 0xFFFFFFFFu;
        r.d1 = m1 ? (uint32_t)__builtin_ctz(m1) : 0xFFFFFFFFu;
        r.d2 = m2 ? (uint32_t)__builtin_ctz(m2) : 0xFFFFFFFFu;
        r.d3 = m3 ? (uint32_t)__builtin_ctz(m3) : 0xFFFFFFFFu;
        r.fit = (np == 1u && prev_ok && p1 == r.d0 && p2 == r.d1 && p3 == r.d2 && p4 == r.d3) ? 1u : 0u;
    }
    if (write && lane == 0) {
        desc_out[0] = np;
        desc_out[1] = r.d0; desc_out[2] = r.d1; desc_out[3] = r.d2; desc_out[4] = r.d3;
        desc_out[5] = 0; desc_out[6] = 0; desc_out[7] = 0;
        desc_out[8] = prev_ok ? 1u : 0u;
// ... 379 lines not shown
        const bool valid = uu < row_hi;
        const uint32_t u = valid ? uu : row_hi - 1;
        const uint32_t rs = g.rowptr[u], re_full = g.rowptr[u + 1];
        const uint32_t re = valid ? re_full : rs;
        const float xself = xin[u];
        float agg = 0.0f;
        uint32_t n0 = g.col[rs + j], n1 = g.col[rs + 4 + j];
        for (uint32_t e = rs; e < re; e += 8) {
            const bool in0 = e + j < re, in1 = e + 4 + j < re;
            const float r0 = xin[in0 ? n0 : u], r1 = xin[in1 ? n1 : u];
            n0 = g.col[e + 8 + j];
            n1 = g.col[e + 12 + j];
            const float a0 = in0 ? r0 : 0.0f, a1 = in1 ? r1 : 0.0f;
#define GNNVC_QUAD_BCAST(x_, t_) __builtin_bit_cast(float, __builtin_amdgcn_update_dpp(0, __builtin_bit_cast(int, x_), (t_) * 0x55, 0xf, 0xf, false))
            agg += GNNVC_QUAD_BCAST(a0, 0);
            agg += GNNVC_QUAD_BCAST(a0, 1);
            agg += GNNVC_QUAD_BCAST(a0, 2);
            agg += GNNVC_QUAD_BCAST(a0, 3);
            agg += GNNVC_QUAD_BCAST(a1, 0);
            agg += GNNVC_QUAD_BCAST(a1, 1);
            agg += GNNVC_QUAD_BCAST(a1, 2);
            agg += GNNVC_QUAD_BCAST(a1, 3);
#undef GNNVC_QUAD_BCAST
        }
        if (j == 0) {
            float *row = &A[vq * kWidePitch];
            row[0] = agg;
            row[1] = xself;
            row[2] = (float)(re_full - rs);
            row[3] = (float)g.w[u] / ws;
            row[4] = (float)g.nw[u] / ws;
        }
    }
    __syncthreads();
    const float *W1 = P, *b1 = W1 + 5 * N1;
    const float *W2 = b1 + N1, *b2 = W2 + N1 * N2;
    const float *W3 = b2 + N2, *b3 = W3 + N2 * N3;
    float x0[5];
#pragma unroll
    for (int k = 0; k < 5; ++k) x0[k] = A[lane * kWidePitch + k];
    float o1[N1 / 4];
    dense_cols<5, 5, N1, N1 / 4, 0>(x0, o1, W1, b1, (N1 / 4) * q);
    wide_tail<N1, N2, N3, false>(o1, A, B, W2, b2, W3, b3, lane, q, v0, row_hi, fout, nullptr);
}

template <int N1, int N2, int N3, int S, bool MFMA, bool SLIM = false>
__global__ __launch_bounds__(kBlock) void k_stage_f1(
        GraphDev g, float ws, const float *__restrict__ xin, float *__restrict__ fout,
        const float *__restrict__ P, uint32_t row_lo, uint32_t row_hi,
        const uint32_t *__restrict__ ep, const uint32_t *__restrict__ ecol,
        const float *__restrict__ acc_in, uint32_t long_thresh, int interleave,
        const uint32_t *__restrict__ acc_bad,
        const uint32_t *__restrict__ emit_spec, c4row *__restrict__ emit_table, unsigned long long *__restrict__ emit_counts,
        const uint32_t *__restrict__ srt_vertex, const uint4 *__restrict__ srt_meta, uint32_t n_sorted, uint32_t skip) {
    static_assert(!(SLIM && MFMA), "the matrix cores' input tile needs the full region");
    __shared__ __attribute__((aligned(16))) float lds[kWavesPerBlock][SLIM ? kSlimRegionFloats : kRegionFloats];
    const bool acc_full = acc_bad && *acc_bad == 0;
    if (acc_bad && !acc_full) acc_in = nullptr;
    const bool sorted = srt_vertex != nullptr;
    const int lane = threadIdx.x & 63;
    float *T = lds[threadIdx.x >> 6];
    uint32_t *stage = reinterpret_cast<uint32_t *>(T);
    const uint32_t ntiles = sorted ? (n_sorted + kWave - 1) / kWave : (row_hi - row_lo + kWave - 1) / kWave;
    uint32_t tile = tile_for_wave(ntiles, sorted || interleave != 0);
    if (tile >= ntiles) return;
    if (sorted && GNNVC_SORTED_MIX) tile = (tile & 1u) ? ntiles - 1u - (tile >> 1) : (tile >> 1);
    const uint32_t v0 = row_lo + tile * kWave;
    uint32_t u, uc, deg, rs, re;
    bool mine, staged = false;
    uint32_t sbase = 0;
    float f_w, f_nw;
    if (sorted) {
        const uint32_t slot = tile * kWave + lane;
        const bool in = slot < n_sorted;
        const uint4 meta = srt_meta[in ? slot : n_sorted - 1];
        u = uc = srt_vertex[in ? slot : n_sorted - 1];
        deg = meta.y - meta.x;
        mine = in && deg < long_thresh;
        rs = meta.x;
        re = mine ? meta.y : rs;
        f_w = (float)meta.z / ws;
        f_nw = (float)meta.w / ws;
    } else {
        u = v0 + lane;
        const bool valid = u < row_hi;
        uc = valid ? u : row_hi - 1;
        deg = g.rowptr[uc + 1] - g.rowptr[uc];
        mine = valid && deg < long_thresh;
        rs = ep[uc];
        re = (mine && !acc_full) ? ep[uc + 1] : rs;
        const uint32_t c0 = __builtin_amdgcn_readfirstlane(rs);
        const uint32_t vend = (v0 + kWave < row_hi) ? v0 + kWave : row_hi;
        if constexpr (!SLIM) {
            const uint32_t c1 = acc_full ? c0 : ep[vend];
            staged = (c1 - c0) <= kStageCap;
            if (staged) sbase = stage_cols(ecol, c0, c1, stage, lane);
        }
        f_w = (float)g.w[uc] / ws;
        f_nw = (float)g.nw[uc] / ws;
    }
    const float f_deg = (float)deg;
    const float xself = xin[uc];
    float agg = acc_in ? acc_in[uc] : 0.0f;
    wave_lds_sync();

    for (uint32_t eb = rs; eb < re; eb += S) {
        float xs[S];
// ... 3 lines not shown
            const uint32_t cv = (!SLIM && staged) ? stage[ee - sbase] : ecol[ee];
            const float v = xin[(ee < re) ? cv : uc];
            xs[s] = (ee < re) ? v : 0.0f;
        }
#pragma unroll
        for (int s = 0; s < S; ++s) agg += xs[s];
    }
    float x0[5];
    x0[0] = agg;
    x0[1] = xself;
    x0[2] = f_deg;
    x0[3] = f_w;
    x0[4] = f_nw;
    const float *W1 = P, *b1 = W1 + 5 * N1;
    const float *W2 = b1 + N1, *b2 = W2 + N1 * N2;
    const float *W3 = b2 + N2, *b3 = W3 + N2 * N3;
    float x1[N1];
    uint32_t live1 = 0;
    if constexpr (MFMA) dense<5, 5, N1, 0>(x0, x1, W1, b1);
    else live1 = dense_relu_live<5, N1>(x0, x1, W1, b1);
    static_assert(N3 == 16, "feature stages emit 16 floats per vertex");
    const int q = lane >> 2, c = lane & 3;
    wave_lds_sync();
    if constexpr (MFMA) {
#pragma unroll
        for (int j = 0; j < N1; ++j) T[lane * kInPitch + j] = x1[j];
        wave_lds_sync();
        const int v = lane & 31, h = lane >> 5;
        f32x16 d[2];
        float a[16];
        mfma_load_a<N2, 16>(W2, v, h, a);
#pragma unroll
        for (int vt = 0; vt < 2; ++vt) {
            d[vt] = mfma_layer_lds(T, vt, v, h, a);
            mfma_bias_act<N2, 0>(d[vt], b2, h);
        }
        mfma_load_a<N3, N2 / 2>(W3, v, h, a);
#pragma unroll
        for (int vt = 0; vt < 2; ++vt) {
            d[vt] = mfma_layer_acc<N2>(d[vt], a);
            mfma_bias_act<N3, 0>(d[vt], b3, h);
        }
        wave_lds_sync();
#pragma unroll
        for (int vt = 0; vt < 2; ++vt)
#pragma unroll
            for (int r = 0; r < 8; ++r) T[(32 * vt + v) * kOutPitch + mfma_feat(r, h)] = d[vt][r];
    } else {
        float x2[N2], x3[N3];
        const uint32_t live2 = dense_live<N1, N2, 0, true>(x1, x2, W2, b2, (skip & 2u) != 0, live1);
        dense_live<N2, N3, 0, true>(x2, x3, W3, b3, (skip & 4u) != 0, live2);
#pragma unroll
        for (int j = 0; j < 16; ++j) T[lane * kOutPitch + j] = x3[j];
        if (emit_counts) c4_emit_row(x3, &T[lane * kOutPitch], u, mine, lane, emit_spec, emit_table, emit_counts);
    }
    wave_lds_sync();
#pragma unroll
    for (int p = 0; p < 4; ++p) {
        const uint32_t row = __shfl(u, 16 * p + q);
        const float *src = &T[(16 * p + q) * kOutPitch + 4 * c];
        const float4 o = make_float4(src[0], src[1], src[2], src[3]);
        if (__shfl((int)mine, 16 * p + q)) reinterpret_cast<float4 *>(fout)[(size_t)row * 4 + c] = o;
    }
}

__global__ __launch_bounds__(256) void k_find_long(GraphDev g, uint32_t thresh, uint32_t *__restrict__ list,
                                                   uint32_t *__restrict__ count) {
    __shared__ unsigned long long part[4];
    __shared__ uint32_t wcnt[4][4];
    __shared__ uint32_t trip_first;
    const uint32_t lane = threadIdx.x & 63, wave = threadIdx.x >> 6;
    const uint64_t lo = g.lo(), hi = g.hi();
    unsigned long long mine = 0;
    for (uint64_t base = lo + (uint64_t)blockIdx.x * 1024u; base < hi; base += (uint64_t)gridDim.x * 1024u) {
        uint32_t d[4];
        unsigned long long m[4];
#pragma unroll
        for (int j = 0; j < 4; ++j) {
            const uint64_t u = base + 256u * j + threadIdx.x;
            d[j] = u < hi ? g.rowptr[u + 1] - g.rowptr[u] : 0u;
            m[j] = __ballot(u < hi && d[j] >= thresh);
            if (lane == 0) wcnt[j][wave] = (uint32_t)__popcll(m[j]);
        }
        __syncthreads();
        if (threadIdx.x == 0) {
            uint32_t total = 0;
#pragma unroll
            for (int k = 0; k < 16; ++k) total += wcnt[k >> 2][k & 3];
            trip_first = total ? atomicAdd(count, total) : 0u;
        }
        __syncthreads();
#pragma unroll
        for (int j = 0; j < 4; ++j) {
            const uint64_t u = base + 256u * j + threadIdx.x;
            if (u < hi && d[j] >= thresh) {
                uint32_t before = trip_first;
                for (int k = 0; k < 4 * j + (int)wave; ++k) before += wcnt[k >> 2][k & 3];
                list[before + (uint32_t)__popcll(m[j] & ((1ull << lane) - 1ull))] = (uint32_t)u;
                mine += d[j];
            }
        }
        __syncthreads();
    }
#pragma unroll
    for (int off = 32; off; off >>= 1)
        mine += ((unsigned long long)__shfl_xor((unsigned)(mine >> 32), off) << 32) | __shfl_xor((unsigned)mine, off);
    if (lane == 0) part[threadIdx.x >> 6] = mine;
// ... 1334 lines not shown
                s1 += ltw_sel(r[3] == r[1], val[3]);
                float s2 = a[2] + val[2];
                s2 += ltw_sel(r[3] == r[2], val[3]);
                float s3 = a[3] + val[3];
                const bool o0 = h0 && r[0] == r[3], o1 = h1 && r[1] == r[3], o2 = h2 && r[2] == r[3], o3 = h3;
                float x = o0 ? s0 : o1 ? s1 : o2 ? s2 : s3;
                bool more = (o0 || o1 || o2 || o3) && r[3] != kLtwNoRow;
                for (;;) {
#pragma unroll
                    for (int k = 0; k < 4; ++k) x += ltw_sel(more && nr[k] == r[3], nv[k]);
                    more = more && nr[3] == r[3];
                    if (!__any(more)) break;
#pragma unroll
                    for (int k = 0; k < 4; ++k) {
                        nr[k] = lane_next(nr[k]);
                        nv[k] = lane_next(nv[k]);
                        if (lane == 63) nr[k] = kLtwNoRow;
                    }
                }
                if (o0) s0 = x;
                if (o1) s1 = x;
                if (o2) s2 = x;
                if (o3) s3 = x;
                if (h0) A[r[0]] = s0;
                if (h1) A[r[1]] = s1;
                if (h2) A[r[2]] = s2;
                if (h3) A[r[3]] = s3;
            }
            __syncthreads();
#pragma unroll
            for (int k = 0; k < SW; ++k) reinterpret_cast<u32x4 *>(slice)[tid + 1024 * k] = sr[k];
            __syncthreads();
        }
    }
    for (uint32_t i = lane; i < slice_rows; i += 64) {
        const uint32_t row = rowmap ? rowmap[(size_t)(chunk * 16 + wave) * slice_rows + i] : row0 + i;
        if (row < row_end) agg[row] = A[i];
    }
}

constexpr uint32_t kC4Block = 131072;
constexpr uint32_t kC4Shift = 18;
constexpr uint32_t kC4Slices = 16;
constexpr uint32_t kC4MaxPasses = 3;
constexpr uint32_t kC4SliceRows = 632;
constexpr uint32_t kC4MaxRows = kC4Slices * kC4SliceRows;
constexpr int kC4LaneEntries = 3;
constexpr uint32_t kC4Step = 64u * kC4LaneEntries;
constexpr uint32_t kC4DirtyWords = (kC4SliceRows + 31) / 32;
constexpr uint32_t kC4NoRow = (1u << (32 - kC4Shift)) - 1u;
constexpr uint32_t kC4Rounds = 64;
static_assert(kC4SliceRows < kC4NoRow - 1u, "row field too narrow");

__global__ __launch_bounds__(64) void k_c4_choose(unsigned long long *__restrict__ counts, int slots, uint32_t n,
                                                  uint32_t *__restrict__ desc, uint32_t max_passes, uint32_t *__restrict__ round_counts,
                                                  uint32_t round_stride, int clear_counts) {
    const int lane = threadIdx.x;
    unsigned long long mine = 0;
    if (slots == 1) {
        mine = lane < 16 ? counts[lane] : (lane == 16 ? (unsigned long long)n : 0ull);
    } else {
        unsigned long long part[kEmitStride];
#pragma unroll
        for (int t = 0; t < kEmitStride; ++t) {
            const int idx = t * 64 + lane;
            part[t] = idx < slots * kEmitStride ? counts[idx] : 0ull;
            if (clear_counts && idx < slots * kEmitStride) counts[idx] = 0ull;
        }
        for (int c = 0; c < kEmitStride; ++c) {
            unsigned long long v = 0;
#pragma unroll
            for (int t = 0; t < kEmitStride; ++t) v += ((t * 64 + lane) % kEmitStride == c) ? part[t] : 0ull;
#pragma unroll
            for (int off = 32; off; off >>= 1)
                v += ((unsigned long long)__shfl_xor((unsigned)(v >> 32), off) << 32) | __shfl_xor((unsigned)v, off);
            if (lane == c) mine = v;
        }
    }
    const unsigned long long rows = ((unsigned long long)__shfl((unsigned)(mine >> 32), 16) << 32) | __shfl((unsigned)mine, 16);
    static_assert(kC4Rounds == 64, "one lane per round counter");
    if (round_counts) round_counts[lane] = (uint32_t)lane * round_stride;
    if (lane == 0) desc[5] = 0u;
    const bool prev_ok = desc[0] == 1u;
    const uint32_t p1 = desc[1], p2 = desc[2], p3 = desc[3], p4 = desc[4];
    if (rows != n) {
        if (lane == 0) {
            desc[0] = 0;
            desc[6] = 0;
        }
        return;
    }
    const unsigned long long c = lane < 16 ? mine : 0ull;
    uint32_t rank = 0;
#pragma unroll
    for (int k = 0; k < 16; ++k) {
        const unsigned long long ck = ((unsigned long long)__shfl((unsigned)(c >> 32), k) << 32) | __shfl((unsigned)c, k);
        rank += (ck > c || (ck == c && k < lane)) ? 1u : 0u;
    }
    uint32_t np = 0;
#pragma unroll
    for (uint32_t t = 3; t >= 1; --t) {
        unsigned long long rest = (lane < 16 && rank >= 4 * t) ? c : 0ull;
#pragma unroll
        for (int off = 8; off; off >>= 1)
            rest += ((unsigned long long)__shfl_xor((unsigned)(rest >> 32), off) << 32) | __shfl_xor((unsigned)rest, off);
        rest = ((unsigned long long)__shfl((unsigned)(rest >> 32), 0) << 32) | __shfl((unsigned)rest, 0);
        if (t <= max_passes && rest <= (unsigned long long)n / 512) np = t;
    }
    const bool chosen = lane < 16 && rank < 4 * np;
    const unsigned long long cm = __ballot(chosen);
    const uint32_t pos = (uint32_t)__popcll(cm & ((1ull << lane) - 1ull));
    const uint32_t c0 = (uint32_t)__builtin_ctzll(cm | (1ull << 63));
    const uint32_t m1 = (uint32_t)(cm & (cm - 1)), m2 = m1 & (m1 - 1), m3 = m2 & (m2 - 1);
    const uint32_t c1 = m1 ? (uint32_t)__builtin_ctz(m1) : 64u, c2 = m2 ? (uint32_t)__builtin_ctz(m2) : 64u,
                   c3 = m3 ? (uint32_t)__builtin_ctz(m3) : 64u;
    const bool table_written = slots > 1 && prev_ok && np == 1u && p1 == c0 && p2 == c1 && p3 == c2 && p4 == c3;
    if (lane < 12) desc[lane < 4 ? 1 + lane : 4 + lane] = 0xFFFFFFFFu;
    if (chosen) desc[pos < 4 ? 1 + pos : 4 + pos] = (uint32_t)lane;
    if (lane == 0) {
        desc[0] = np;
        desc[6] = (np && !table_written) ? 1u : 0u;
    }
}

__global__ __launch_bounds__(256) void k_c4_compact(const float4 *__restrict__ feat, uint32_t n, uint32_t *__restrict__ desc,
                                                    f32x4 *__restrict__ table) {
    if (!desc[0] || !desc[6]) return;
    const uint32_t npass = desc[0];
    uint32_t mask = 0;
    for (uint32_t q = 0; q < npass; ++q)
        for (int k = 0; k < 4; ++k) {
            const uint32_t cc = desc[(q == 0 ? 1 : 4 + 4 * q) + k];
            if (cc < 16u) mask |= 1u << cc;
        }
    bool negative = false;
    for (size_t v = (size_t)blockIdx.x * blockDim.x + threadIdx.x; v <= n; v += (size_t)gridDim.x * blockDim.x) {
        uint32_t nz = 0;
        float r[16];
        if (v < n) {
            const float4 q0 = feat[v * 4], q1 = feat[v * 4 + 1], q2 = feat[v * 4 + 2], q3 = feat[v * 4 + 3];
            const float rr[16] = {q0.x, q0.y, q0.z, q0.w, q1.x, q1.y, q1.z, q1.w, q2.x, q2.y, q2.z, q2.w, q3.x, q3.y, q3.z, q3.w};
#pragma unroll
            for (int i = 0; i < 16; ++i) {
                r[i] = rr[i];
                nz |= (rr[i] != 0.0f ? 1u : 0u) << i;
                negative |= rr[i] < 0.0f;
            }
        }
        for (uint32_t q = 0; q < npass; ++q) {
            f32x4 out = {0.0f, 0.0f, 0.0f, 0.0f};
            if (v < n) {
                const uint32_t *dc = desc + (q == 0 ? 1 : 4 + 4 * q);
                const float *row = reinterpret_cast<const float *>(feat) + v * 16;
#pragma unroll
                for (int k = 0; k < 4; ++k) {
                    const uint32_t cc = dc[k];
                    const float a = cc < 16u ? row[cc] : 0.0f;
                    out[k] = a == 0.0f ? 0.0f : a;
                }
                if (nz & ~mask) out[0] = __uint_as_float(__float_as_uint(out[0]) | 0x80000000u);
            }
            table[(size_t)q * ((size_t)n + 1) + v] = out;
        }
        (void)r;
    }
    if (__any(negative) && (threadIdx.x & 63) == 0) atomicAnd(&desc[0], 0u);
}

__device__ __forceinline__ f32x4 lane_next(f32x4 v) {
    f32x4 r;
#pragma unroll
    for (int i = 0; i < 4; ++i) r[i] = __uint_as_float(lane_next(__float_as_uint(v[i])));
    return r;
}
__device__ __forceinline__ f32x4 c4_sel(bool c, f32x4 v) {
    return f32x4{c ? v[0] : 0.0f, c ? v[1] : 0.0f, c ? v[2] : 0.0f, c ? v[3] : 0.0f};
}

template <int TAG>
__global__ __launch_bounds__(1024) void k_c4_agg(const uint32_t *__restrict__ step_ptr, const uint4 *__restrict__ steps,
                                                 const uint32_t *__restrict__ entries, const f32x4 *__restrict__ table,
                                                 f32x4 *__restrict__ agg, uint32_t n, uint32_t slice_rows, uint32_t slice0,
                                                 uint32_t slice1, uint32_t nslices, uint32_t last_entry, uint32_t *__restrict__ desc,
                                                 uint32_t *__restrict__ dirty_rows, uint32_t dirty_cap, uint32_t block_cols,
                                                 uint32_t nblocks, uint32_t row_base, uint32_t row_end, uint32_t pass,
                                                 const uint32_t *__restrict__ rowmap, uint32_t *__restrict__ dirty_count) {
    extern __shared__ __attribute__((aligned(16))) unsigned char c4_smem[];
    if (desc[0] <= pass) return;
    const uint32_t lane = threadIdx.x & 63, wave = threadIdx.x >> 6;
    f32x4 *A = reinterpret_cast<f32x4 *>(c4_smem) + wave * slice_rows;
    uint32_t *dirty = reinterpret_cast<uint32_t *>(c4_smem + (size_t)kC4Slices * slice_rows * 16) + wave * kC4DirtyWords;
    for (uint32_t base = slice0 + blockIdx.x * kC4Slices; base < slice1; base += gridDim.x * kC4Slices) {
        const bool live = base + wave < slice1;
        const uint32_t wc = live ? base + wave : nslices;
        const uint32_t row0 = row_base + (live ? wc * slice_rows : 0u);
        uint32_t cur_blk = 0;
        for (uint32_t i = lane; i < slice_rows; i += 64) A[i] = f32x4{0.0f, 0.0f, 0.0f, 0.0f};
        if (lane < kC4DirtyWords) dirty[lane] = 0;
        const uint32_t st0 = __builtin_amdgcn_readfirstlane(step_ptr[wc]);
        const int nsteps = (int)(__builtin_amdgcn_readfirstlane(step_ptr[wc + 1]) - st0);
        constexpr int E = kC4LaneEntries;
        uint32_t e[4][E];
        f32x4 v[2][E];
        uint32_t cb[4], cnt[4], bk[4];
#pragma unroll
        for (int a = 0; a < 4; ++a) {
            cb[a] = 0;
            bk[a] = 0;
            cnt[a] = 0;
#pragma unroll
// ... 89 lines not shown
                        f32x4 x = sum[E - 1];
#pragma unroll
                        for (int i = E - 1; i >= 0; --i) {
                            o[i] = h[i] && r[i] == r[E - 1];
                            any_o = any_o || o[i];
                            if (o[i]) x = sum[i];
                        }
                        bool more = any_o && r[E - 1] != kC4NoRow;
                        for (;;) {
#pragma unroll
                            for (int k = 0; k < E; ++k) x += c4_sel(more && nr[k] == r[E - 1], nv[k]);
                            more = more && nr[E - 1] == r[E - 1];
                            if (!__any(more)) break;
#pragma unroll
                            for (int k = 0; k < E; ++k) {
                                nr[k] = lane_next(nr[k]);
                                nv[k] = lane_next(nv[k]);
                                if (lane == 63) nr[k] = kC4NoRow;
                            }
                        }
#pragma unroll
                        for (int i = 0; i < E; ++i) {
                            if (o[i]) sum[i] = x;
                            if (h[i]) A[r[i]] = sum[i];
                        }
                    }
                }
            }
        }
        while (cur_blk < nblocks) {
            __syncthreads();
            ++cur_blk;
        }
        if (live)
            for (uint32_t i = lane; i < slice_rows; i += 64) {
                const uint32_t row = rowmap ? rowmap[(size_t)wc * slice_rows + i] : row0 + i;
                if (row >= row_end) continue;
                f32x4 a = A[i];
                if (dirty[i >> 5] >> (i & 31) & 1u) {
                    if (pass == 0) {
                        const uint32_t slot = atomicAdd(dirty_count, 1u);
                        if (slot < dirty_cap) dirty_rows[slot] = row;
                        a[0] = __uint_as_float(0x80000000u);
                        a[1] = __uint_as_float(slot < dirty_cap ? slot : 0xFFFFFFFFu);
                    }
                }
                agg[row] = a;
            }
    }
}

__global__ __launch_bounds__(256) void k_c4_fix(GraphDev g, const float4 *__restrict__ fin, uint32_t *__restrict__ desc,
                                                const uint32_t *__restrict__ dirty_rows, uint32_t dirty_cap,
                                                float4 *__restrict__ agg16, const uint32_t *__restrict__ dirty_count, uint32_t slot_base) {
    if (!desc[0]) return;
    const uint32_t first = min(slot_base, dirty_cap);
    const uint32_t count = min(*dirty_count, dirty_cap);
    if (dirty_count != desc + 5 && blockIdx.x == 0 && threadIdx.x == 0) atomicAdd(&desc[5], *dirty_count - slot_base);
    const uint32_t c = threadIdx.x & 3;
    for (uint32_t slot = first + ((blockIdx.x * blockDim.x + threadIdx.x) >> 2); slot < count; slot += (gridDim.x * blockDim.x) >> 2) {
        const uint32_t u = dirty_rows[slot];
        uint32_t e = g.rowptr[u];
        const uint32_t end = g.rowptr[u + 1];
        float4 a = make_float4(0.f, 0.f, 0.f, 0.f);
        for (; e + 1 < end; e += 2) {
            const float4 r0 = fin[(size_t)g.col[e] * 4 + c], r1 = fin[(size_t)g.col[e + 1] * 4 + c];
            a.x += r0.x; a.y += r0.y; a.z += r0.z; a.w += r0.w;
            a.x += r1.x; a.y += r1.y; a.z += r1.z; a.w += r1.w;
        }
        if (e < end) {
            const float4 r0 = fin[(size_t)g.col[e] * 4 + c];
            a.x += r0.x; a.y += r0.y; a.z += r0.z; a.w += r0.w;
        }
        agg16[(size_t)slot * 4 + c] = a;
    }
}

__global__ __launch_bounds__(256) void k_prune_mark_zero(const float4 *__restrict__ feat, uint32_t n, uint32_t *__restrict__ heavy_bits) {
    const uint32_t u = blockIdx.x * blockDim.x + threadIdx.x;
    bool zero = false;
    if (u < n) {
        const float4 a = feat[(size_t)u * 4], b = feat[(size_t)u * 4 + 1], c = feat[(size_t)u * 4 + 2], d = feat[(size_t)u * 4 + 3];
        zero = !(a.x != 0.f || a.y != 0.f || a.z != 0.f || a.w != 0.f || b.x != 0.f || b.y != 0.f || b.z != 0.f || b.w != 0.f ||
                 c.x != 0.f || c.y != 0.f || c.z != 0.f || c.w != 0.f || d.x != 0.f || d.y != 0.f || d.z != 0.f || d.w != 0.f);
    }
    const unsigned long long m = __ballot(zero);
    const uint32_t w0 = (u & ~63u) >> 5, words = (n + 31) / 32;
    if ((threadIdx.x & 63) == 0 && w0 < words) heavy_bits[w0] = (uint32_t)m;
    if ((threadIdx.x & 63) == 1 && w0 + 1 < words) heavy_bits[w0 + 1] = (uint32_t)(m >> 32);
}

template <int N1, int N2, int N3>
__global__ __launch_bounds__(256) void k_predict_zero_f1(GraphDev g, float ws, const float *__restrict__ P, uint32_t *__restrict__ heavy_bits) {
    const uint32_t u = blockIdx.x * blockDim.x + threadIdx.x;
    const uint32_t uc = u < g.n ? u : g.n - 1;
    const uint32_t deg = g.rowptr[uc + 1] - g.rowptr[uc];
    bool zero = false;
    if (__any(u < g.n && deg != 0)) {
        float x0[5];
        x0[1] = (float)g.w[uc] / ws;
        x0[2] = (float)deg;
        x0[3] = x0[1];
        x0[4] = (float)g.nw[uc] / ws;
        x0[0] = x0[4];
        const float *W1 = P, *b1 = W1 + 5 * N1;
        const float *W2 = b1 + N1, *b2 = W2 + N1 * N2;
        const float *W3 = b2 + N2, *b3 = W3 + N2 * N3;
        float x1[N1], x2[N2], x3[N3];
        dense<5, 5, N1, 0>(x0, x1, W1, b1);
        dense<N1, N1, N2, 0>(x1, x2, W2, b2);
        dense<N2, N2, N3, 1>(x2, x3, W3, b3);
        float top = x3[0], scale = 0.0f;
#pragma unroll
        for (int j = 0; j < N3; ++j) {
            top = x3[j] > top ? x3[j] : top;
            scale = fabsf(x3[j]) > scale ? fabsf(x3[j]) : scale;
        }
#pragma unroll
        for (int k = 0; k < N2; ++k) scale = x2[k] > scale ? x2[k] : scale;
        zero = u < g.n && deg != 0 && top <= -1e-3f * (1.0f + scale);
    }
    const unsigned long long m = __ballot(zero);
    const uint32_t w0 = (u & ~63u) >> 5, words = (g.n + 31) / 32;
    if ((threadIdx.x & 63) == 0 && w0 < words) heavy_bits[w0] = (uint32_t)m;
    if ((threadIdx.x & 63) == 1 && w0 + 1 < words) heavy_bits[w0 + 1] = (uint32_t)(m >> 32);
}

// ... 1024 lines not shown
    const dim3 grid((c.row_hi - c.row_lo + kWave - 1) / kWave), block(kBlock);
    const float *P = c.params + sp.param_offset;
    switch (sp.variant) {
    case 0:
        GNNVC_LAUNCH((k_stage_w1<32, 32, 16>), grid, block, 0, c.stream, *c.g, c.ws, c.in, c.out, P, c.row_lo, c.row_hi);
        break;
    case 1:
        GNNVC_LAUNCH((k_stage_w16<32, 32, 16, false>), grid, block, 0, c.stream, *c.g, c.ws, reinterpret_cast<const float4 *>(c.in), c.out,
                     (float *)nullptr, P, c.row_lo, c.row_hi);
        break;
    case 2:
        GNNVC_LAUNCH((k_stage_w16<32, 16, 1, true>), grid, block, 0, c.stream, *c.g, c.ws, reinterpret_cast<const float4 *>(c.in), c.out,
                     c.logits, P, c.row_lo, c.row_hi);
        break;
    default:
        return hipErrorInvalidValue;
    }
    return hipGetLastError();
}

#ifndef GNNVC_T4_S
#define GNNVC_T4_S 4
#endif
hipError_t launch_stage_t4(const StageCall &c, const TableTileArgs &a) {
    if (c.row_hi <= c.row_lo) return hipSuccess;
    const StagePlan &sp = *c.sp;
    if (sp.f != 16 || (sp.variant != 1 && sp.variant != 2) || !a.table_in || !a.counts_in || !a.counts_zero || a.counts_zero == a.counts_in ||
        !a.desc_in || !a.desc_out || a.desc_in == a.desc_out)
        return hipErrorInvalidValue;
    const uint32_t ntiles = (c.row_hi - c.row_lo + kWave - 1) / kWave;
    const uint32_t per_xcd = (ntiles + 7) / 8;
    const uint32_t blocks_per_xcd = (per_xcd + kWavesPerBlock - 1) / kWavesPerBlock;
    const dim3 grid(blocks_per_xcd * 8 + 1), block(kBlock);
    const float *P = c.params + sp.param_offset;
    const float4 *in4 = reinterpret_cast<const float4 *>(c.in), *tab = reinterpret_cast<const float4 *>(a.table_in);
    if (sp.variant == 1)
        GNNVC_LAUNCH((k_stage_t4<32, 32, 16, false, GNNVC_T4_S>), grid, block, 0, c.stream, *c.g, c.ws, in4, c.out, (float *)nullptr, P,
                     c.row_lo, c.row_hi, a.interleave ? 1 : 0, tab, a.counts_in, a.counts_zero, a.desc_in, a.desc_out, a.emit.spec,
                     reinterpret_cast<c4row *>(a.emit.table), a.emit.counts, a.solo ? 1 : 0);
    else
        GNNVC_LAUNCH((k_stage_t4<32, 16, 1, true, GNNVC_T4_S>), grid, block, 0, c.stream, *c.g, c.ws, in4, c.out, c.logits, P,
                     c.row_lo, c.row_hi, a.interleave ? 1 : 0, tab, a.counts_in, a.counts_zero, a.desc_in, a.desc_out,
                     (const uint32_t *)nullptr, (c4row *)nullptr, (unsigned long long *)nullptr, a.solo ? 1 : 0);
    return hipGetLastError();
}

hipError_t launch_dense_sigmoid(const StageCall &c, const CompactSums &s, uint32_t long_thresh) {
    if (c.row_hi <= c.row_lo) return hipSuccess;
    if (c.sp->f != 16 || c.sp->variant != 2 || !s.acc4 || !s.c4desc) return hipErrorInvalidValue;
    const dim3 grid((c.row_hi - c.row_lo + kBlock - 1) / kBlock), block(kBlock);
    GNNVC_LAUNCH((k_dense_f16<32, 16, 1, true>), grid, block, 0, c.stream, *c.g, c.ws, reinterpret_cast<const float4 *>(c.in), c.out,
                       c.logits, c.params + c.sp->param_offset, c.row_lo, c.row_hi, reinterpret_cast<const float4 *>(s.acc4), s.c4desc,
                       reinterpret_cast<const float4 *>(s.agg16), reinterpret_cast<const float4 *>(s.table_in), long_thresh,
                       (const uint32_t *)nullptr, (c4row *)nullptr, (unsigned long long *)nullptr, c.skip);
    return hipGetLastError();
}

hipError_t launch_stage(const StageCall &c, const TileArgs &a) {
    if (c.row_hi <= c.row_lo) return hipSuccess;
    const StagePlan &sp = *c.sp;
    const GraphDev &g = *c.g;
    const SortedOrder *so = a.so, *so_pruned = a.so_pruned;
    const CompactSums &s = a.sums;
    const bool sorted = so && so->n > 0;
    const bool with_p = sorted && g.prune_eff && so_pruned && so_pruned->vertex;
    if (g.prune_eff && sorted && !with_p) return hipErrorInvalidValue;
    if (so && so->n == 0 && !with_p) return hipSuccess;
    const uint32_t n_p = with_p ? so_pruned->n : 0u;
    const uint32_t ntiles = sorted ? (std::max(so->n, n_p) + kWave - 1) / kWave : (c.row_hi - c.row_lo + kWave - 1) / kWave;
    const uint32_t per_xcd = (ntiles + 7) / 8;
    const uint32_t blocks_per_xcd = (per_xcd + kWavesPerBlock - 1) / kWavesPerBlock;
    const dim3 grid(blocks_per_xcd * 8), block(kBlock);
    const float *P = c.params + sp.param_offset;
    const float4 *in4 = reinterpret_cast<const float4 *>(c.in);
    const float *nofloat = nullptr;
    const int il = a.interleave ? 1 : 0;
    switch (sp.variant * 2 + (a.mfma ? 1 : 0)) {
    case 0:
        GNNVC_LAUNCH((k_stage_f1<32, 32, 16, 4, false>), grid, block, 0, c.stream, g, c.ws, c.in, c.out, P,
                           c.row_lo, c.row_hi, g.rowptr, g.col, nofloat, a.long_thresh, il, (const uint32_t *)nullptr,
                           a.emit.spec, reinterpret_cast<c4row *>(a.emit.table), a.emit.counts, sorted ? so->vertex : nullptr,
                           sorted ? reinterpret_cast<const uint4 *>(so->meta) : nullptr, sorted ? so->n : 0u, c.skip);
        break;
    case 1:
        GNNVC_LAUNCH((k_stage_f1<32, 32, 16, 4, true>), grid, block, 0, c.stream, g, c.ws, c.in, c.out, P,
                           c.row_lo, c.row_hi, g.rowptr, g.col, nofloat, a.long_thresh, il, (const uint32_t *)nullptr,
                           (const uint32_t *)nullptr, (c4row *)nullptr, (unsigned long long *)nullptr,
                           sorted ? so->vertex : nullptr, sorted ? reinterpret_cast<const uint4 *>(so->meta) : nullptr,
                           sorted ? so->n : 0u, c.skip);
        break;
#ifndef GNNVC_GATHER_S
#define GNNVC_GATHER_S 2
#endif
#ifndef GNNVC_GATHER_S_SORTED
#define GNNVC_GATHER_S_SORTED 3
#endif
#define GNNVC_F16_ARGS(SIG_, MF_, LG_)                                                                              \
                       grid, block, 0, c.stream, g, c.ws, in4, c.out,                                               \
                       LG_, P, c.row_lo, c.row_hi, a.long_thresh, sorted ? so->vertex : nullptr,                    \
                       sorted ? so->meta : nullptr, sorted ? so->n : 0u, il,                                        \
                       (const float4 *)nullptr, s.acc4 ? s.c4desc : a.skip_flag, (const float4 *)nullptr,           \
                       (MF_ || SIG_) ? nullptr : a.emit.spec, reinterpret_cast<c4row *>((MF_ || SIG_) ? nullptr : a.emit.table), \
                       (MF_ || SIG_) ? nullptr : a.emit.counts,                                                     \
                       with_p ? so_pruned->vertex : nullptr, with_p ? so_pruned->meta : nullptr, n_p
#define GNNVC_LAUNCH_X(...) GNNVC_LAUNCH(__VA_ARGS__)
#define GNNVC_LAUNCH_F16(N2_, N3_, SIG_, MF_, SRT_, S_, LG_) \
    GNNVC_LAUNCH_X((k_stage_f16<32, N2_, N3_, SIG_, S_, MF_, SRT_>), GNNVC_F16_ARGS(SIG_, MF_, LG_))
#define GNNVC_LAUNCH_F16F(N2_, N3_, SIG_, MF_, SRT_, S_, LG_, FLT_) \
    GNNVC_LAUNCH_X((k_stage_f16<32, N2_, N3_, SIG_, S_, MF_, SRT_, false, FLT_>), GNNVC_F16_ARGS(SIG_, MF_, LG_))
    case 2:
        if (sorted) GNNVC_LAUNCH_F16(32, 16, false, false, true, GNNVC_GATHER_S_SORTED, nullptr);
        else GNNVC_LAUNCH_F16(32, 16, false, false, false, GNNVC_GATHER_S, nullptr);
        break;
    case 3:
        if (g.zero_bits) {
            if (sorted) GNNVC_LAUNCH_F16F(32, 16, false, true, true, GNNVC_GATHER_S_SORTED, nullptr, true);
            else GNNVC_LAUNCH_F16F(32, 16, false, true, false, GNNVC_GATHER_S, nullptr, true);
        } else if (sorted) GNNVC_LAUNCH_F16(32, 16, false, true, true, GNNVC_GATHER_S_SORTED, nullptr);
        else GNNVC_LAUNCH_F16(32, 16, false, true, false, GNNVC_GATHER_S, nullptr);
        break;
    case 4:
        if (sorted) GNNVC_LAUNCH_F16(16, 1, true, false, true, GNNVC_GATHER_S_SORTED, c.logits);
        else GNNVC_LAUNCH_F16(16, 1, true, false, false, GNNVC_GATHER_S, c.logits);
        break;
    case 5:
        if (g.zero_bits) {
            if (sorted) GNNVC_LAUNCH_F16F(16, 1, true, true, true, GNNVC_GATHER_S_SORTED, c.logits, true);
            else GNNVC_LAUNCH_F16F(16, 1, true, true, false, GNNVC_GATHER_S, c.logits, true);
        } else if (sorted) GNNVC_LAUNCH_F16(16, 1, true, true, true, GNNVC_GATHER_S_SORTED, c.logits);
        else GNNVC_LAUNCH_F16(16, 1, true, true, false, GNNVC_GATHER_S, c.logits);
        break;
#undef GNNVC_LAUNCH_F16
#undef GNNVC_LAUNCH_F16F
#undef GNNVC_F16_ARGS
#undef GNNVC_LAUNCH_X
    default:
        return hipErrorInvalidValue;
    }
    if (s.acc4 && sp.f == 16 && a.dense_part) {
        const uint32_t nt = (c.row_hi - c.row_lo + kWave - 1) / kWave;
        const dim3 grid((((nt + 7) / 8 + kWavesPerBlock - 1) / kWavesPerBlock) * 8);
#define GNNVC_LAUNCH_AGG(N2_, N3_, SIG_, MF_, LG_)                                                        \
        GNNVC_LAUNCH((k_stage_f16<32, N2_, N3_, SIG_, 2, MF_, false, true>), grid, block, 0, c.stream, g, c.ws, in4, \
                           c.out, LG_, P, c.row_lo, c.row_hi, a.long_thresh, (const uint32_t *)nullptr, (const uint4 *)nullptr, \
                           0u, il, reinterpret_cast<const float4 *>(s.acc4), s.c4desc, reinterpret_cast<const float4 *>(s.agg16), \
                           (MF_ || SIG_) ? nullptr : a.emit.spec, reinterpret_cast<c4row *>((MF_ || SIG_) ? nullptr : a.emit.table), \
                           (MF_ || SIG_) ? nullptr : a.emit.counts)
        if (sp.variant == 1) {
            if (a.mfma_agg) {
                GNNVC_LAUNCH_AGG(32, 16, false, true, nullptr);
            } else {
                const dim3 dgrid((c.row_hi - c.row_lo + kBlock - 1) / kBlock);
                GNNVC_LAUNCH((k_dense_f16<32, 32, 16, false>), dgrid, block, 0, c.stream, g, c.ws, in4, c.out, (float *)nullptr, P, c.row_lo, c.row_hi,
                                   reinterpret_cast<const float4 *>(s.acc4), s.c4desc, reinterpret_cast<const float4 *>(s.agg16),
                                   reinterpret_cast<const float4 *>(s.table_in), a.long_thresh, a.emit.spec,
                                   reinterpret_cast<c4row *>(a.emit.table), a.emit.counts, c.skip);
            }
        } else {
            if (a.mfma_agg) GNNVC_LAUNCH_AGG(16, 1, true, true, c.logits);
            else return launch_dense_sigmoid(c, s, a.long_thresh);
        }
#undef GNNVC_LAUNCH_AGG
    }
    return hipGetLastError();
}

__global__ void k_spin(unsigned long long ticks) {
    const unsigned long long t0 = wall_clock64();
    for (int i = 0; i < (1 << 22) && wall_clock64() - t0 < ticks; ++i) __builtin_amdgcn_s_sleep(16);
}
struct WordList {
    const uint32_t *src[24];
};
__global__ void k_words(WordList wl, uint32_t *__restrict__ out) {
    const int i = threadIdx.x;
    if (i < 24 && wl.src[i]) out[i] = *wl.src[i];
}
hipError_t classify_graph(const GraphDev &g, const GraphClassArgs &a, uint32_t *dev_words, uint32_t *out_dev, hipStream_t stream) {
    hipError_t rc = hipMemsetAsync(dev_words, 0, 16 * sizeof(uint32_t), stream);
    if (rc != hipSuccess) return rc;
    WordList wl;
    for (auto &p : wl.src) p = nullptr;
    wl.src[0] = dev_words;
    if (g.n) GNNVC_LAUNCH(k_validate_graph, dim3(2048), dim3(256), 0, stream, g, dev_words);
    const uint32_t lo = g.lo(), hi = g.hi();
    if (a.cuts && hi > lo)
        for (int k = 0; k <= 8; ++k) wl.src[1 + k] = g.rowptr + lo + (size_t)((uint64_t)(hi - lo) * k / 8);
    if (a.waste && hi > lo) {
        GNNVC_LAUNCH(k_tile_waste, dim3(std::min<unsigned>((hi - lo + 255) / 256, 512u)), dim3(256), 0, stream, g, lo, hi, a.waste_thresh,
                     reinterpret_cast<unsigned long long *>(dev_words + 2), a.heavy_from);
        for (int k = 0; k < 4; ++k) wl.src[10 + k] = dev_words + 2 + k;
    }
    if (a.longs && hi > lo && a.long_list) {
        GNNVC_LAUNCH(k_find_long, dim3(std::min<unsigned>((hi - lo + 1023) / 1024, 2048u)), dim3(256), 0, stream, g, a.long_thresh, a.long_list,
                     dev_words + 8);
        for (int k = 0; k < 4; ++k) wl.src[14 + k] = dev_words + 8 + k;
    }
    GNNVC_LAUNCH(k_words, dim3(1), dim3(64), 0, stream, wl, out_dev);
    return hipGetLastError();
}

__global__ void k_verdicts(VerdictWords vw, uint32_t *__restrict__ out) {
    const int i = threadIdx.x;
    if (i < 8) out[i] = vw.src[i] ? *vw.src[i] : 0u;
}
hipError_t write_verdicts(const VerdictWords &vw, uint32_t *out_dev, hipStream_t stream) {
    GNNVC_LAUNCH(k_verdicts, dim3(1), dim3(64), 0, stream, vw, out_dev);
    return hipGetLastError();
}
// ... 101 lines not shown
    return hipGetLastError();
}

static hipError_t scan_u32(uint32_t *data, size_t n, uint32_t *scratch, hipStream_t stream) {
    if (n == 0) return hipSuccess;
    const size_t chunks = (n + kScanChunk - 1) / kScanChunk;
    GNNVC_LAUNCH(k_scan_chunks, dim3((unsigned)chunks), dim3(256), 0, stream, data, n, scratch);
    if (chunks > 1) {
        hipError_t rc = scan_u32(scratch, chunks, scratch + chunks, stream);
        if (rc != hipSuccess) return rc;
        GNNVC_LAUNCH(k_scan_add, dim3((unsigned)((n + 255) / 256)), dim3(256), 0, stream, data, n,
                           scratch);
    }
    return hipGetLastError();
}

size_t blocked_scan_scratch_elems(size_t n_elems) { return n_elems / 2048 + 8192; }

hipError_t build_blocked_index(const GraphDev &g, uint32_t wb, uint32_t nblocks, uint32_t long_thresh,
                               uint32_t *bp, uint32_t *colb, uint32_t *scratch, uint32_t *bad_flag,
                               hipStream_t stream) {
    const size_t elems = (size_t)nblocks * g.n + 1;
    hipError_t rc = hipMemsetAsync(bp, 0, elems * sizeof(uint32_t), stream);
    if (rc != hipSuccess) return rc;
    rc = hipMemsetAsync(bad_flag, 0, sizeof(uint32_t), stream);
    if (rc != hipSuccess) return rc;
    const unsigned nb = (g.n + 255) / 256;
    GNNVC_LAUNCH(k_blk_count, dim3(nb), dim3(256), 0, stream, g, wb, long_thresh, bp, bad_flag);
    rc = scan_u32(bp, elems, scratch, stream);
    if (rc != hipSuccess) return rc;
    GNNVC_LAUNCH(k_blk_scatter, dim3(nb), dim3(256), 0, stream, g, wb, long_thresh, bp, colb);
    return hipGetLastError();
}

hipError_t launch_stage0_blocked(const StageCall &c, const BlockedPlan &bp, const Stage0Args &a) {
    if (c.row_hi <= c.row_lo) return hipSuccess;
    const StagePlan &sp = *c.sp;
    const GraphDev &g = *c.g;
    if (sp.variant != 0) return hipErrorInvalidValue;
    const unsigned nb = (c.row_hi - c.row_lo + 255) / 256;
    for (uint32_t k = 0; k + 1 < bp.nblocks; ++k)
        GNNVC_LAUNCH(k_blk_accumulate, dim3(nb), dim3(256), 0, c.stream, bp.bp + (size_t)k * g.n, bp.colb, c.in,
                           bp.acc, c.row_lo, c.row_hi, k == 0 ? 1 : 0);
    const uint32_t ntiles = (c.row_hi - c.row_lo + kWave - 1) / kWave;
    const uint32_t per_xcd = (ntiles + 7) / 8;
    const uint32_t blocks_per_xcd = (per_xcd + kWavesPerBlock - 1) / kWavesPerBlock;
    const uint32_t *ep = bp.bp + (size_t)(bp.nblocks - 1) * g.n;
    const float *acc_in = bp.nblocks > 1 ? bp.acc : nullptr;
    const dim3 grid(blocks_per_xcd * 8), block(kBlock);
    if (a.mfma)
        GNNVC_LAUNCH((k_stage_f1<32, 32, 16, 4, true>), grid, block, 0, c.stream, g, c.ws, c.in, c.out,
                           c.params + sp.param_offset, c.row_lo, c.row_hi, ep, bp.colb, acc_in, a.long_thresh, a.interleave ? 1 : 0,
                           (const uint32_t *)nullptr, (const uint32_t *)nullptr, (c4row *)nullptr, (unsigned long long *)nullptr,
                           (const uint32_t *)nullptr, (const uint4 *)nullptr, 0u, c.skip);
    else
        GNNVC_LAUNCH((k_stage_f1<32, 32, 16, 4, false>), grid, block, 0, c.stream, g, c.ws, c.in, c.out,
                           c.params + sp.param_offset, c.row_lo, c.row_hi, ep, bp.colb, acc_in, a.long_thresh, a.interleave ? 1 : 0,
                           (const uint32_t *)nullptr, a.emit.spec, reinterpret_cast<c4row *>(a.emit.table), a.emit.counts,
                           (const uint32_t *)nullptr, (const uint4 *)nullptr, 0u, c.skip);
    return hipGetLastError();
}

hipError_t allow_dynamic_lds(const void *func, int bytes, std::atomic<uint64_t> &done) {
    int dev = 0;
    hipError_t rc = hipGetDevice(&dev);
    if (rc != hipSuccess) return rc;
    if (dev >= 0 && dev < 64 && (done.load(std::memory_order_acquire) >> dev & 1u)) return hipSuccess;
    rc = hipFuncSetAttribute(func, hipFuncAttributeMaxDynamicSharedMemorySize, bytes);
    if (rc == hipSuccess && dev >= 0 && dev < 64) done.fetch_or(1ull << dev, std::memory_order_release);
    return rc;
}

static bool lt_flat_plan(uint32_t rows_per_chunk, const PlanMap &pm) { return !pm.rowmap && !pm.bstart && rows_per_chunk <= kLtFlatRows; }
static uint32_t lt_flat_threads() {
    return 256u;
}

uint32_t lds_table_max_rows(uint32_t bits) { return 16u * lt_slice_rows_max(bits); }
uint32_t lds_table_block(uint32_t bits) { return lt_block_cols(bits); }
uint32_t lds_table_bits_for(uint32_t kmax) { return kmax <= 255u ? 8u : (kmax <= 1023u ? 10u : (kmax <= 65535u ? 16u : 0u)); }
size_t lds_table_bytes_for(uint32_t bits, size_t n) { return lt_table_bytes(bits, n); }
uint32_t lds_table_step() { return kLtwStep; }
uint32_t lds_table_record_words() { return kLtwRec; }

hipError_t lds_table_wsteps(const GraphDev &g, uint32_t slice_rows, uint32_t nchunks, uint32_t nblocks, const uint32_t *seg_cnt,
                            const uint32_t *step_ptr, uint32_t *step_count, uint32_t *recs, bool write, uint32_t slack,
                            hipStream_t stream, const PlanMap &pm, uint32_t row_base, uint32_t row_end, uint32_t bits) {
    if (slack < 3u * nblocks + 4u) return hipErrorInvalidValue;
    if (bits != 8 && bits != 10 && bits != 16) return hipErrorInvalidValue;
    if (row_end > g.n) row_end = g.n;
    GNNVC_LAUNCH(k_ltw_steps, dim3((nchunks + 63) / 64), dim3(64), 0, stream, g, slice_rows, nchunks, nblocks, seg_cnt,
                       step_ptr, step_count, recs, write ? 1 : 0, kLtwStep, slack, lt_block_cols(bits), pm, row_base, row_end,
                       lt_piece_cols(bits));
    return hipGetLastError();
}

hipError_t lds_table_wmax(const uint32_t *w, uint32_t n, uint32_t *wmax, hipStream_t stream) {
    hipError_t rc = hipMemsetAsync(wmax, 0, sizeof(uint32_t), stream);
    if (rc != hipSuccess || !n) return rc;
    GNNVC_LAUNCH(k_lt_wmax, dim3(std::min<unsigned>((n + 255) / 256, 1024u)), dim3(256), 0, stream, w, n, wmax);
    return hipGetLastError();
}

bool lds_table_is_flat(uint32_t rows_per_chunk, const PlanMap &pm) { return lt_flat_plan(rows_per_chunk, pm); }

hipError_t lds_table_count(const GraphDev &g, uint32_t rows_per_chunk, uint32_t nchunks, uint32_t nblocks, uint32_t block_cols,
                           uint32_t *seg_cnt, uint32_t *bad, hipStream_t stream, uint32_t row_base, uint32_t row_end,
                           const PlanMap &pm, uint32_t chunk0, uint32_t chunk1) {
    if (row_end > g.n) row_end = g.n;
    if (nblocks > 4096 || block_cols > (1u << 18) || rows_per_chunk > (1u << 15)) return hipErrorInvalidValue;
    if (chunk1 > nchunks) chunk1 = nchunks;
    if (chunk0 >= chunk1) return hipSuccess;
// ... 112 lines not shown
    GNNVC_LAUNCH(k_map_deal, dim3((nslices + 3) / 4), dim3(256), 0, stream, g, sorted_rows, m, slice_rows, nslices, rowmap, weight);
    return hipGetLastError();
}

hipError_t mass_bounds(const GraphDev &g, unsigned long long target, uint32_t count, uint32_t *cand, hipStream_t stream) {
    if (!count) return hipSuccess;
    GNNVC_LAUNCH(k_mass_bounds, dim3((count + 255) / 256), dim3(256), 0, stream, g, target, count, cand);
    return hipGetLastError();
}

hipError_t launch_stage0_lds_table(const StageCall &c, const LdsTablePlan &lp, uint8_t *wbyte, float *acc, uint32_t *bad,
                                   const Stage0Args &a) {
    if (c.row_hi <= c.row_lo) return hipSuccess;
    const StagePlan &sp = *c.sp;
    const GraphDev &g = *c.g;
    if (lp.bits != 8 && lp.bits != 10 && lp.bits != 16) return hipErrorInvalidValue;
    if (lp.rowmap && lp.bits != 8) return hipErrorInvalidValue;
    const uint32_t plan_end = std::min(lp.plan_end, g.n);
    if (c.row_lo < lp.plan_base || c.row_hi > plan_end) return hipErrorInvalidValue;
    if (lp.rowmap && (c.row_lo != 0 || c.row_hi != g.n || lp.mapped_chunks == 0)) return hipErrorInvalidValue;
    if (sp.variant != 0 || lp.rows_per_chunk == 0 || lp.rows_per_chunk > 16u * lt_slice_rows_max(lp.bits) || lp.rows_per_chunk % 16u || g.nnz == 0)
        return hipErrorInvalidValue;
    hipError_t rc = hipMemsetAsync(bad, 0, sizeof(uint32_t), c.stream);
    if (rc != hipSuccess) return rc;
    const dim3 tgrid(std::min<unsigned>((g.n / 4 + 255) / 256 + 1, 4096u));
    const uint32_t c0 = lp.rowmap ? 0u : (c.row_lo - lp.plan_base) / lp.rows_per_chunk;
    const uint32_t c1 = lp.rowmap ? lp.mapped_chunks - 1 : (c.row_hi - 1 - lp.plan_base) / lp.rows_per_chunk;
    const uint32_t slice_rows = lp.rows_per_chunk / 16u;
    constexpr size_t lds_max = (size_t)16 * kLtwSliceRows * 4 + 1024 + kLtwBlock;
    static_assert(lds_max <= 160 * 1024, "LDS budget of k_lt_agg");
    const size_t lds = (size_t)16 * slice_rows * 4 + lt_lut_floats(lp.bits) * 4 + kLtwBlock;
#define GNNVC_LT_AGG(B_)                                                                                                          \
    {                                                                                                                             \
        GNNVC_LAUNCH(k_lt_bytes_x<B_>, tgrid, dim3(256), 0, c.stream, c.in, c.ws, g.n, wbyte, bad);                               \
        static std::atomic<uint64_t> lds_ok{0};                                                                                   \
        rc = allow_dynamic_lds(reinterpret_cast<const void *>(k_lt_agg<B_>), (int)lds_max, lds_ok);                               \
        if (rc != hipSuccess) return rc;                                                                                          \
        GNNVC_LAUNCH(k_lt_agg<B_>, dim3(c1 - c0 + 1), dim3(1024), lds, c.stream, lp.step_ptr,                                     \
                     reinterpret_cast<const uint32_t *>(lp.steps), lp.entries, wbyte, c.ws, acc, g.n, slice_rows, c0, lp.last_entry, bad, \
                     lp.rowmap, lp.rowmap ? 0u : lp.plan_base, lp.rowmap ? g.n : plan_end);                                       \
    }
    if (lp.bits == 8) GNNVC_LT_AGG(8)
    else if (lp.bits == 10) GNNVC_LT_AGG(10)
    else GNNVC_LT_AGG(16)
#undef GNNVC_LT_AGG
    const uint32_t ntiles = (c.row_hi - c.row_lo + kWave - 1) / kWave;
    const uint32_t per_xcd = (ntiles + 7) / 8;
    const uint32_t blocks_per_xcd = (per_xcd + kWavesPerBlock - 1) / kWavesPerBlock;
    const dim3 grid(blocks_per_xcd * 8), block(kBlock);
    if (a.mfma)
        GNNVC_LAUNCH((k_stage_f1<32, 32, 16, 4, true>), grid, block, 0, c.stream, g, c.ws, c.in, c.out, c.params + sp.param_offset,
                           c.row_lo, c.row_hi, g.rowptr, g.col, acc, a.long_thresh, a.interleave ? 1 : 0, (const uint32_t *)bad,
                           (const uint32_t *)nullptr, (c4row *)nullptr, (unsigned long long *)nullptr,
                           (const uint32_t *)nullptr, (const uint4 *)nullptr, 0u, c.skip);
    else
        GNNVC_LAUNCH((k_stage_f1<32, 32, 16, 4, false, GNNVC_STAGE0_SLIM != 0>), grid, block, 0, c.stream, g, c.ws, c.in, c.out, c.params + sp.param_offset,
                           c.row_lo, c.row_hi, g.rowptr, g.col, acc, a.long_thresh, a.interleave ? 1 : 0, (const uint32_t *)bad,
                           a.emit.spec, reinterpret_cast<c4row *>(a.emit.table), a.emit.counts,
                           (const uint32_t *)nullptr, (const uint4 *)nullptr, 0u, c.skip);
    return hipGetLastError();
}

uint32_t compact_max_rows() { return kC4MaxRows; }
uint32_t compact_block() { return kC4Block; }
uint32_t compact_shift() { return kC4Shift; }
uint32_t compact_slices() { return kC4Slices; }
uint32_t compact_step() { return kC4Step; }
uint32_t compact_rounds() { return kC4Rounds; }

hipError_t launch_compact_gather(const GraphDev &g, const CompactPlan &cp, const float *in, unsigned long long *counts,
                                 int count_slots, uint32_t *desc, float *table, float *acc4, uint32_t row_lo, uint32_t row_hi,
                                 uint32_t *dirty_rows, uint32_t dirty_cap, float *agg16, hipStream_t stream, int what,
                                 uint32_t *round_counts, uint32_t round_stride, bool clear_counts) {
    if (row_hi <= row_lo || g.nnz == 0 || row_lo < cp.plan_base || row_hi > cp.plan_end) return hipErrorInvalidValue;
    if (cp.rows_per_chunk == 0 || cp.rows_per_chunk > kC4MaxRows || cp.rows_per_chunk % kC4Slices) return hipErrorInvalidValue;
    if (cp.max_passes < 1 || cp.max_passes > kC4MaxPasses) return hipErrorInvalidValue;
    if (what & 1) {
        GNNVC_LAUNCH(k_c4_choose, dim3(1), dim3(64), 0, stream, counts, count_slots, g.n, desc, cp.max_passes, round_counts,
                     round_stride, clear_counts ? 1 : 0);
        GNNVC_LAUNCH(k_c4_compact, dim3(std::min<unsigned>((g.n + 256) / 256, 4096u)), dim3(256), 0, stream,
                           reinterpret_cast<const float4 *>(in), g.n, desc, reinterpret_cast<f32x4 *>(table));
    }
    if (!(what & 2)) return hipGetLastError();
    hipError_t rc0 = hipSuccess;
    if (!(what & 1)) rc0 = hipMemsetAsync(desc + 5, 0, sizeof(uint32_t), stream);
    if (rc0 != hipSuccess) return rc0;
    rc0 = compact_sums(g, cp, desc, table, acc4, row_lo, row_hi, dirty_rows, dirty_cap, stream);
    if (rc0 != hipSuccess) return rc0;
    return compact_fix(g, in, desc, dirty_rows, dirty_cap, agg16, desc + 5, 0, stream);
}

hipError_t compact_choose(unsigned long long *counts, int count_slots, uint32_t rows, uint32_t *desc, uint32_t max_passes,
                          hipStream_t stream, bool clear_counts) {
    GNNVC_LAUNCH(k_c4_choose, dim3(1), dim3(64), 0, stream, counts, count_slots, rows, desc, max_passes, (uint32_t *)nullptr,
                 0u, clear_counts ? 1 : 0);
    return hipGetLastError();
}

hipError_t compact_sums(const GraphDev &g, const CompactPlan &cp, uint32_t *desc, const float *table, float *acc4, uint32_t row_lo,
                        uint32_t row_hi, uint32_t *dirty_rows, uint32_t dirty_cap, hipStream_t stream, uint32_t *round_count) {
    const bool one_round = round_count != nullptr;
    uint32_t *const dirty_count = one_round ? round_count : desc + 5;
    if (row_hi <= row_lo || g.nnz == 0 || row_lo < cp.plan_base || row_hi > cp.plan_end) return hipErrorInvalidValue;
    if (cp.rows_per_chunk == 0 || cp.rows_per_chunk > kC4MaxRows || cp.rows_per_chunk % kC4Slices) return hipErrorInvalidValue;
    if (cp.rowmap && one_round) return hipErrorInvalidValue;
    const uint32_t slice_rows = cp.rows_per_chunk / kC4Slices;
    const uint32_t nslices = cp.rowmap ? cp.nslices : ((cp.plan_end - cp.plan_base + cp.rows_per_chunk - 1) / cp.rows_per_chunk) * kC4Slices;
    const uint32_t c0 = cp.rowmap ? 0u : (row_lo - cp.plan_base) / cp.rows_per_chunk;
    const uint32_t c1 = cp.rowmap ? nslices / kC4Slices : (row_hi - 1 - cp.plan_base) / cp.rows_per_chunk + 1;
    constexpr size_t lds_max = (size_t)kC4Slices * (kC4SliceRows * 16 + kC4DirtyWords * 4);
    static_assert(lds_max <= 160 * 1024, "LDS budget of k_c4_agg");
    const size_t lds = (size_t)kC4Slices * ((size_t)slice_rows * 16 + kC4DirtyWords * 4);
    static std::atomic<uint64_t> lds_ok0{0}, lds_ok1{0};
    {
        hipError_t rc = allow_dynamic_lds(reinterpret_cast<const void *>(k_c4_agg<0>), (int)lds_max, lds_ok0);
        if (rc == hipSuccess) rc = allow_dynamic_lds(reinterpret_cast<const void *>(k_c4_agg<1>), (int)lds_max, lds_ok1);
        if (rc != hipSuccess) return rc;
    }
    const dim3 grid(std::min<uint32_t>(256u, c1 - c0)), block(1024);
    for (uint32_t pass = 0; pass < cp.max_passes; ++pass) {
        const f32x4 *tq = reinterpret_cast<const f32x4 *>(table) + (size_t)pass * ((size_t)g.n + 1);
        f32x4 *aq = reinterpret_cast<f32x4 *>(acc4) + (size_t)pass * g.n;
        if (one_round)
            GNNVC_LAUNCH(k_c4_agg<1>, grid, block, lds, stream, cp.step_ptr, reinterpret_cast<const uint4 *>(cp.steps), cp.entries, tq, aq,
                               g.n, slice_rows, c0 * kC4Slices, std::min(c1 * kC4Slices, nslices), nslices, cp.last_entry, desc,
                               dirty_rows, dirty_cap, cp.block_cols, cp.nblocks, cp.plan_base, cp.plan_end, pass, cp.rowmap, dirty_count);
        else
            GNNVC_LAUNCH(k_c4_agg<0>, grid, block, lds, stream, cp.step_ptr, reinterpret_cast<const uint4 *>(cp.steps), cp.entries, tq, aq,
                               g.n, slice_rows, c0 * kC4Slices, std::min(c1 * kC4Slices, nslices), nslices, cp.last_entry, desc,
                               dirty_rows, dirty_cap, cp.block_cols, cp.nblocks, cp.plan_base, cp.plan_end, pass, cp.rowmap, dirty_count);
    }
    return hipGetLastError();
}

hipError_t compact_fix(const GraphDev &g, const float *in, uint32_t *desc, const uint32_t *dirty_rows, uint32_t dirty_cap,
                       float *agg16, const uint32_t *dirty_count, uint32_t slot_base, hipStream_t stream, uint32_t blocks) {
    GNNVC_LAUNCH(k_c4_fix, dim3(std::min<uint32_t>((dirty_cap + 63) / 64, blocks)), dim3(256), 0, stream, g,
                       reinterpret_cast<const float4 *>(in), desc, dirty_rows, dirty_cap, reinterpret_cast<float4 *>(agg16), dirty_count,
                       slot_base);
    return hipGetLastError();
}

hipError_t measure_tile_waste(const GraphDev &g, uint32_t row_lo, uint32_t row_hi, uint32_t long_thresh,
                              unsigned long long *sum_max , hipStream_t stream,
                              uint32_t heavy_from) {
    hipError_t rc = hipMemsetAsync(sum_max, 0, 2 * sizeof(unsigned long long), stream);
    if (rc != hipSuccess || row_hi <= row_lo) return rc;
    GNNVC_LAUNCH(k_tile_waste, dim3(std::min<unsigned>((row_hi - row_lo + 255) / 256, 512u)), dim3(256), 0, stream, g,
                       row_lo, row_hi, long_thresh, sum_max, heavy_from);
    return hipGetLastError();
}

hipError_t degree_histogram(const GraphDev &g, uint32_t row_lo, uint32_t row_hi, uint32_t long_thresh,
                            uint32_t bins, uint32_t *hist, hipStream_t stream, const uint32_t *skip_rowptr, uint32_t skip_from) {
    hipError_t rc = hipMemsetAsync(hist, 0, bins * sizeof(uint32_t), stream);
    if (rc != hipSuccess || row_hi <= row_lo) return rc;
    const unsigned nb = std::min<unsigned>((row_hi - row_lo + 255) / 256, 2048u);
    GNNVC_LAUNCH(k_deg_hist, dim3(nb), dim3(256), 0, stream, g, row_lo, row_hi, long_thresh, bins, hist, skip_rowptr, skip_from);
    return hipGetLastError();
}

hipError_t degree_starts(uint32_t *hist, uint32_t bins, uint32_t *info, hipStream_t stream) {
    if (bins == 0 || bins > 4096) return hipErrorInvalidValue;
    GNNVC_LAUNCH(k_deg_starts, dim3(1), dim3(64), 0, stream, hist, bins, info);
    return hipGetLastError();
}

hipError_t degree_scatter(const GraphDev &g, uint32_t row_lo, uint32_t row_hi, uint32_t long_thresh,
                          uint32_t bins, uint32_t *cursor, uint32_t *vertex, void *meta, hipStream_t stream,
                          const uint32_t *skip_rowptr, uint32_t skip_from) {
    if (row_hi <= row_lo) return hipSuccess;
    GNNVC_LAUNCH(k_deg_scatter, dim3((row_hi - row_lo + 256 * kDegScatterRows - 1) / (256 * kDegScatterRows)), dim3(256), 0, stream, g, row_lo, row_hi,
                       long_thresh, bins, cursor, vertex, reinterpret_cast<uint4 *>(meta), skip_rowptr, skip_from);
    return hipGetLastError();
}

hipError_t find_long_rows(const GraphDev &g, uint32_t thresh, uint32_t *list, uint32_t *count,
                          hipStream_t stream) {
    hipError_t rc = hipMemsetAsync(count, 0, 4 * sizeof(uint32_t), stream);
    if (rc != hipSuccess || g.hi() <= g.lo()) return rc;
    GNNVC_LAUNCH(k_find_long, dim3(std::min<unsigned>((g.hi() - g.lo() + 1023) / 1024, 2048u)), dim3(256), 0, stream, g, thresh, list, count);
    return hipGetLastError();
}

hipError_t derive_tails(const GraphDev &old_g, const uint32_t *old_row, uint32_t n_new, const uint32_t *rowptr_new, uint32_t *new_of,
                        uint32_t *tail, uint32_t *bad, hipStream_t stream) {
    hipError_t rc = hipMemsetAsync(new_of, 0xFF, (size_t)std::max<uint32_t>(old_g.n, 1u) * sizeof(uint32_t), stream);
    if (rc == hipSuccess) rc = hipMemsetAsync(bad, 0, sizeof(uint32_t), stream);
    if (rc != hipSuccess || n_new == 0) return rc;
    const dim3 grid((n_new + 255) / 256), block(256);
    GNNVC_LAUNCH(k_derive_map, grid, block, 0, stream, old_row, n_new, old_g.n, new_of, bad);
    GNNVC_LAUNCH(k_derive_tails, grid, block, 0, stream, old_g, old_row, new_of, rowptr_new, n_new, tail, bad);
// ... 313 lines not shown
```

Before: 25.82 billion.

## Skip dense row writes when compact table captures the activation rows

Adds a sparse-rows mode. Producer stages that already emit the compact 4-column table can skip writing full 16-float rows for rows whose nonzeros fit in the table. The next stage then reads those rows from the table, both in the compact gather/fix path and in the dense kernel's own-row fetch. When the consumer cannot read that form, a new expand kernel rebuilds the dense rows first. This is meant to cut global write and read traffic for activations, at the cost of extra branching and bookkeeping and a fallback expand pass.

```diff
diff --git a/gnn-mwvc_amd/csrc/gnnvc_engine.cpp b/gnn-mwvc_amd/csrc/gnnvc_engine.cpp
--- a/gnn-mwvc_amd/csrc/gnnvc_engine.cpp
+++ b/gnn-mwvc_amd/csrc/gnnvc_engine.cpp
@@ -223,6 +223,7 @@
     bool rounds = false;
     bool emit = false;
     bool emit_t4 = false;
+    bool sparse_in = false;
     uint32_t long_thresh = 0xFFFFFFFFu;
     gnnvc::SortedOrder sorted;
 };
@@ -370,6 +371,20 @@
         emit.counts = e->c4_emit_counts.p;
         e->c4_fused_for = stage + 1;
         return GNNVC_OK;
+    };
+    auto sparse_out = [&](bool f1_kernel) -> bool {
+        const int mode = GNNVC_SPARSE_ROWS;
+        if (mode == 0 || (mode == 2 && !f1_kernel) || (mode == 3 && f1_kernel)) return false;
+        if (!c.emit || !emit.counts || e->audit_now || e->n_long != 0 || (size_t)stage + 1 >= e->stages.size()) return false;
+        if (call.out != e->h[0].p && call.out != e->h[1].p) return false;
+        if ((size_t)stage + 2 < e->stages.size() && e->stages[stage + 2].f == 16 && !e->pg.c4_seeded[stage + 2] && e->opt.pilot_rows)
+            return false;
+        if (!e->opt.dense_skip) return false;
+        for (size_t s = 1; s < e->stages.size(); ++s)
+            if (e->stages[s].f == 16 && !(e->stages[s].skip_ok & 1u)) return false;
+        e->sparse_buf = call.out;
+        e->sparse_last |= 1u << stage;
+        return true;
     };
     auto pilot = [&]() -> int {
         if (!c.emit || e->pg.c4_seeded[stage + 1] || !e->opt.pilot_rows) return GNNVC_OK;
@@ -419,13 +434,15 @@
         ++e->plan_memsets;
         return hip_rc(e, gnnvc::launch_stage0_lds_table(plain, lds_table_plan(e), e->lt_bytes.p, e->blk_acc.p, e->lt_bad.p,
                                                         {.long_thresh = c.long_thresh, .mfma = e->opt.mfma == 1,
-                                                         .interleave = e->interleave, .emit = emit}));
+                                                         .interleave = e->interleave, .emit = emit,
+                                                         .sparse_out = e->opt.mfma != 1 && sparse_out(true)}));
     }
     if (c.sums == StageChoice::kBlocked)
         return hip_rc(e, gnnvc::launch_stage0_blocked(plain,
                                                       {.nblocks = e->blk_count, .bp = e->blk_ptr.p, .colb = e->blk_col.p, .acc = e->blk_acc.p},
                                                       {.long_thresh = e->long_thresh, .mfma = e->opt.mfma == 1,
-                                                       .interleave = e->interleave, .emit = emit}));
+                                                       .interleave = e->interleave, .emit = emit,
+                                                       .sparse_out = e->opt.mfma != 1 && sparse_out(true)}));
     gnnvc::CompactSums sums;
     uint32_t *desc = nullptr;
     if (c.sums == StageChoice::kCompactPrepared || c.sums == StageChoice::kCompactWhole) {
@@ -441,7 +458,8 @@
         if (!(what & 1)) ++e->plan_memsets;
         HIP_TRY(e, gnnvc::launch_compact_gather(e->g, compact_plan(e), in, fused ? e->c4_emit_counts.p : e->c4_counts.p, fused ? 64 : 1,
                                                 desc, e->c4_table.p, e->c4_acc.p, lo, hi, e->c4_dirty.p, e->c4_dirty_cap,
-                                                e->c4_agg16.p, e->stream, what, c.rounds ? e->c4_round_counts.p : nullptr, 256u * e->c4_rows, fused));
+                                                e->c4_agg16.p, e->stream, what, c.rounds ? e->c4_round_counts.p : nullptr, 256u * e->c4_rows, fused,
+                                                c.sparse_in ? const_cast<float *>(in) : nullptr));
         if (fused) e->c4_emit_zero = true;
     }
     if (c.sums != StageChoice::kLdsTable && c.sums != StageChoice::kBlocked) {
@@ -458,7 +476,10 @@
         return hip_rc(e, gnnvc::launch_stage_wide(plain));
     }
     HIP_TRY(e, gnnvc::launch_stage(call, {.long_thresh = c.long_thresh, .mfma = c.mfma, .so = sop, .interleave = e->interleave,
-                                          .sums = sums, .mfma_agg = e->opt.mfma == 1, .emit = emit, .dense_part = !c.rounds,
+                                          .sums = sums, .mfma_agg = e->opt.mfma == 1, .emit = emit,
+                                          .sparse_out = c.sums == StageChoice::kCompactWhole && sp.variant == 1 && !c.rounds &&
+                                                        e->opt.mfma != 1 && sparse_out(false),
+                                          .dense_part = !c.rounds,
                                           .so_pruned = so_p.vertex ? &so_p : nullptr}));
     if (!c.rounds) return GNNVC_OK;
     const uint32_t rows = e->c4_rows, c0 = (lo - e->c4_base) / rows, c1 = (hi - 1 - e->c4_base) / rows;
@@ -483,7 +504,7 @@
             HIP_TRY(e, hipStreamWaitEvent(e->aux_stream, e->round_ev[k], 0));
         }
         HIP_TRY(e, gnnvc::compact_fix(e->g, in, desc, e->c4_dirty.p, e->c4_dirty_cap, e->c4_agg16.p, count, slot_base, ds,
-                                      64));
+                                      64, c.sparse_in ? e->c4_table.p : nullptr));
         gnnvc::StageCall round = plain;
         round.row_lo = ra;
         round.row_hi = rb;
@@ -519,6 +540,26 @@
     int rc = choose_stage(e, stage, lo, hi, in, out, in_forward, c);
     if (rc) return rc;
     const bool longs = e->n_long > 0;
+    if (!in_forward) e->sparse_buf = nullptr;
+    if (e->sparse_buf) {
+        const float *buf = e->sparse_buf;
+        e->sparse_buf = nullptr;
+        const gnnvc::StagePlan &sp = e->stages[stage];
+        const bool copes = in_forward && buf == in && c.sums == StageChoice::kCompactWhole && c.fused_counts && !c.sorted.n && !longs &&
+                           e->opt.mfma != 1 && !e->audit_now && e->opt.dense_skip && (sp.skip_ok & 1u) &&
+                           !(c.emit && !e->pg.c4_seeded[stage + 1] && e->opt.pilot_rows);
+        if (copes) {
+            c.sparse_in = true;
+        } else {
+            if (stage < 1 || !e->c4_desc.p || !e->c4_table.p || !e->c4_emit_counts.p)
+                return fail(e, GNNVC_ERR_STATE, "sparse rows without the compact-table plan's buffers");
+            float *rows = buf == e->h[0].p ? e->h[0].p : e->h[1].p;
+            HIP_TRY(e, gnnvc::compact_expand(rows, e->g.n, e->c4_desc.p + gnnvc_engine::kDescWords * (stage - 1), e->c4_table.p,
+                                             e->c4_emit_counts.p, e->stream));
+            if (!e->sparse_expanded_now) ++e->pg.sparse_expanded;
+            e->sparse_expanded_now = true;
+        }
+    }
     GraphDev gv;
     gnnvc::SortedOrder so_p;
     rc = gather_view(e, stage, lo, hi, in, c.sums == StageChoice::kGather, c.sorted.n != 0, gv, so_p, c.mfma, c.long_thresh);
@@ -1214,6 +1255,8 @@
         }
     }
     else if (k == "plan_memsets_last_forward") *value = (long)e->plan_memsets;
+    else if (k == "sparse_rows_last_forward") *value = (long)e->sparse_last;
+    else if (k == "sparse_rows_expanded") *value = (long)e->pg.sparse_expanded;
     else if (k == "lds_table_active") *value = e->pg.lt_ready ? 1 : 0;
     else if (k == "lds_table_last_ok") {
         *value = 0;
@@ -1814,6 +1857,9 @@
     if (rc) return rc;
     const float *cur = d_x;
     e->c4_fused_for = -1;
+    e->sparse_buf = nullptr;
+    e->sparse_last = 0;
+    e->sparse_expanded_now = false;
     e->pg.c4_prepared_stage = -1;
     if (e->pg.fit_pending && hipEventQuery(e->ev_fit) == hipSuccess) {
         e->pg.fit_pending = false;
diff --git a/gnn-mwvc_amd/csrc/gnnvc_engine_state.h b/gnn-mwvc_amd/csrc/gnnvc_engine_state.h
--- a/gnn-mwvc_amd/csrc/gnnvc_engine_state.h
+++ b/gnn-mwvc_amd/csrc/gnnvc_engine_state.h
@@ -89,6 +89,7 @@
         uint32_t c4_unfit_runs[4] = {0, 0, 0, 0};
         uint32_t fit_calm = 0;
         uint32_t fit_skip = 0;
+        uint64_t sparse_expanded = 0;
         int short_from = 0;
         bool heavy_known = false;
         uint32_t heavy_rows = 0, heavy_thresh = 0;
@@ -152,6 +153,9 @@
     bool c4_emit_zero = false;
     uint32_t c4_base = 0, c4_end = 0;
     const float *c4_prepared_in = nullptr;
+    const float *sparse_buf = nullptr;
+    uint32_t sparse_last = 0;
+    bool sparse_expanded_now = false;
     int c4_fused_for = -1;
     struct PrunePlan {
         bool tried = false, ready = false, deferred = false;
diff --git a/gnn-mwvc_amd/csrc/gnnvc_kernels.h b/gnn-mwvc_amd/csrc/gnnvc_kernels.h
--- a/gnn-mwvc_amd/csrc/gnnvc_kernels.h
+++ b/gnn-mwvc_amd/csrc/gnnvc_kernels.h
@@ -90,6 +90,9 @@
     void *live_desc = nullptr;
 };
 
+#ifndef GNNVC_SPARSE_ROWS
+#define GNNVC_SPARSE_ROWS 1
+#endif
 struct EmitArgs {
     const uint32_t *spec = nullptr;
     float *table = nullptr;
@@ -113,6 +116,7 @@
     const uint32_t *skip_flag = nullptr;
     bool mfma_agg = false;
     EmitArgs emit;
+    bool sparse_out = false;
     bool dense_part = true;
     const SortedOrder *so_pruned = nullptr;
 };
@@ -235,6 +239,7 @@
     bool mfma = false;
     bool interleave = false;
     EmitArgs emit;
+    bool sparse_out = false;
 };
 hipError_t launch_stage0_blocked(const StageCall &c, const BlockedPlan &bp, const Stage0Args &a);
 
@@ -329,7 +334,8 @@
                                  int what = 3 ,
                                  uint32_t *round_counts = nullptr ,
                                  uint32_t round_stride = 0 ,
-                                 bool clear_counts = false );
+                                 bool clear_counts = false ,
+                                 float *sparse_rows = nullptr );
 
 hipError_t compact_choose(unsigned long long *counts, int count_slots, uint32_t rows, uint32_t *desc, uint32_t max_passes,
                           hipStream_t stream, bool clear_counts = false);
@@ -337,7 +343,10 @@
                         uint32_t row_hi, uint32_t *dirty_rows, uint32_t dirty_cap, hipStream_t stream,
                         uint32_t *round_count = nullptr);
 hipError_t compact_fix(const GraphDev &g, const float *in, uint32_t *desc, const uint32_t *dirty_rows, uint32_t dirty_cap,
-                       float *agg16, const uint32_t *dirty_count, uint32_t slot_base, hipStream_t stream, uint32_t blocks = 1024);
+                       float *agg16, const uint32_t *dirty_count, uint32_t slot_base, hipStream_t stream, uint32_t blocks = 1024,
+                       const float *table = nullptr );
+hipError_t compact_expand(float *rows, uint32_t n, const uint32_t *desc, const float *table, const unsigned long long *counts,
+                          hipStream_t stream);
 
 hipError_t derive_tails(const GraphDev &old_g, const uint32_t *old_row, uint32_t n_new, const uint32_t *rowptr_new, uint32_t *new_of,
                         uint32_t *tail, uint32_t *bad, hipStream_t stream);
diff --git a/gnn-mwvc_amd/csrc/gnnvc_kernels.hip b/gnn-mwvc_amd/csrc/gnnvc_kernels.hip
--- a/gnn-mwvc_amd/csrc/gnnvc_kernels.hip
+++ b/gnn-mwvc_amd/csrc/gnnvc_kernels.hip
@@ -276,7 +276,7 @@
 typedef float c4row __attribute__((ext_vector_type(4)));
 constexpr int kEmitSlots = 64, kEmitStride = 17;
 
-__device__ __forceinline__ void c4_emit_with(const float *trow, uint32_t nz, uint32_t u, bool mine, int lane, uint32_t spec_ok,
+__device__ __forceinline__ bool c4_emit_with(const float *trow, uint32_t nz, uint32_t u, bool mine, int lane, uint32_t spec_ok,
                                              uint32_t s0, uint32_t s1, uint32_t s2, uint32_t s3, c4row *__restrict__ table,
                                              unsigned long long *__restrict__ counts) {
     uint32_t my = 0;
@@ -292,17 +292,19 @@
         const float a = trow[s0], b = trow[s1], c = trow[s2], d = trow[s3];
         c4row out = {a == 0.0f ? 0.0f : a, b == 0.0f ? 0.0f : b, c == 0.0f ? 0.0f : c, d == 0.0f ? 0.0f : d};
         const bool odd = !(a >= 0.0f) || !(b >= 0.0f) || !(c >= 0.0f) || !(d >= 0.0f);
-        if (odd || (nz & ~((1u << s0) | (1u << s1) | (1u << s2) | (1u << s3))))
-            out[0] = __uint_as_float(__float_as_uint(out[0]) | 0x80000000u);
+        const bool flag = odd || (nz & ~((1u << s0) | (1u << s1) | (1u << s2) | (1u << s3))) != 0u;
+        if (flag) out[0] = __uint_as_float(__float_as_uint(out[0]) | 0x80000000u);
         if (odd) out[1] = __uint_as_float(__float_as_uint(out[1]) | 0x80000000u);
         table[u] = out;
-    }
-}
-__device__ __forceinline__ void c4_emit(const float *trow, uint32_t nz, uint32_t u, bool mine, int lane,
+        return !flag;
+    }
+    return false;
+}
+__device__ __forceinline__ bool c4_emit(const float *trow, uint32_t nz, uint32_t u, bool mine, int lane,
                                         const uint32_t *__restrict__ spec, c4row *__restrict__ table,
                                         unsigned long long *__restrict__ counts) {
     const uint32_t ok = spec[0];
-    c4_emit_with(trow, nz, u, mine, lane, ok, ok == 1u ? spec[1] : 0u, ok == 1u ? spec[2] : 0u, ok == 1u ? spec[3] : 0u,
+    return c4_emit_with(trow, nz, u, mine, lane, ok, ok == 1u ? spec[1] : 0u, ok == 1u ? spec[2] : 0u, ok == 1u ? spec[3] : 0u,
                  ok == 1u ? spec[4] : 0u, table, counts);
 }
 
@@ -321,7 +323,7 @@
         c4_count_cols<J + 1>(x, mm, tcols, my, stray);
     }
 }
-__device__ __forceinline__ void c4_emit_regs(const float (&x)[16], const float *trow, uint32_t u, bool mine, int lane,
+__device__ __forceinline__ bool c4_emit_regs(const float (&x)[16], const float *trow, uint32_t u, bool mine, int lane,
                                              const uint32_t *__restrict__ spec, c4row *__restrict__ table,
                                              unsigned long long *__restrict__ counts) {
     const uint32_t ok = spec[0];
@@ -337,25 +339,28 @@
         const float a = trow[s0], b = trow[s1], c = trow[s2], d = trow[s3];
         c4row out = {a == 0.0f ? 0.0f : a, b == 0.0f ? 0.0f : b, c == 0.0f ? 0.0f : c, d == 0.0f ? 0.0f : d};
         const bool odd = !(a >= 0.0f) || !(b >= 0.0f) || !(c >= 0.0f) || !(d >= 0.0f);
-        if (odd || (stray >> lane & 1ull)) out[0] = __uint_as_float(__float_as_uint(out[0]) | 0x80000000u);
+        const bool flag = odd || (stray >> lane & 1ull) != 0ull;
+        if (flag) out[0] = __uint_as_float(__float_as_uint(out[0]) | 0x80000000u);
         if (odd) out[1] = __uint_as_float(__float_as_uint(out[1]) | 0x80000000u);
         table[u] = out;
-    }
+        return !flag;
+    }
+    return false;
 }
 
 #ifndef GNNVC_EMIT_REGS
 #define GNNVC_EMIT_REGS 1
 #endif
-__device__ __forceinline__ void c4_emit_row(const float (&x)[16], const float *trow, uint32_t u, bool mine, int lane,
+__device__ __forceinline__ bool c4_emit_row(const float (&x)[16], const float *trow, uint32_t u, bool mine, int lane,
                                             const uint32_t *__restrict__ spec, c4row *__restrict__ table,
                                             unsigned long long *__restrict__ counts) {
     if constexpr (GNNVC_EMIT_REGS) {
-        c4_emit_regs(x, trow, u, mine, lane, spec, table, counts);
+        return c4_emit_regs(x, trow, u, mine, lane, spec, table, counts);
     } else {
         uint32_t nz = 0;
 #pragma unroll
         for (int j = 0; j < 16; ++j) nz |= (x[j] != 0.0f ? 1u : 0u) << j;
-        c4_emit(trow, nz, u, mine, lane, spec, table, counts);
+        return c4_emit(trow, nz, u, mine, lane, spec, table, counts);
     }
 }
 
@@ -678,7 +683,7 @@
                                                       const uint32_t *__restrict__ c4desc, const float4 *__restrict__ agg16,
                                                       const float4 *table_in , uint32_t long_thresh,
                                                       const uint32_t *__restrict__ emit_spec, c4row *__restrict__ emit_table,
-                                                      unsigned long long *__restrict__ emit_counts, uint32_t skip) {
+                                                      unsigned long long *__restrict__ emit_counts, uint32_t skip, uint32_t sparse) {
     static_assert(SIGMOID ? N3 == 1 : N3 == 16, "a feature stage writes 16 floats per row, the last stage one score");
     __shared__ float lds[SIGMOID ? 1 : kWavesPerBlock][SIGMOID ? 1 : kWave * kOutPitch];
     if (c4desc[0] == 0) return;
@@ -700,6 +705,8 @@
     float x1[N1];
     uint32_t live1;
     const bool ascending = (d0 < d1 || d1 == 0xFFFFFFFFu) && (d1 < d2 || d2 == 0xFFFFFFFFu) && (d2 < d3 || d3 == 0xFFFFFFFFu);
+    const bool own_fin = stray || (c4desc[7] & 1u) == 0u;
+    auto own_col = [&](uint32_t k) { return k == d0 ? t.x : k == d1 ? t.y : k == d2 ? t.z : k == d3 ? t.w : 0.0f; };
     if (!__any(stray) && (ascending || !__any(dirty))) {
         static_assert(N1 % 2 == 0, "outputs in pairs");
         f32x2 acc[N1 / 2];
@@ -771,18 +778,34 @@
         }
         size_t own = (size_t)u * 4;
         {
-            float s[4] = {fin[own].x, f_deg, f_w, f_nw};
+            float s[4] = {own_fin ? fin[own].x : own_col(0u), f_deg, f_w, f_nw};
             live_terms<4, N1>(acc, s, W1 + 16 * N1, all);
         }
         {
             asm volatile("" : "+v"(own));
-            const float4 h1 = fin[own + 1], h2 = fin[own + 2], h3 = fin[own + 3];
-            float s[12] = {h1.x, h1.y, h1.z, h1.w, h2.x, h2.y, h2.z, h2.w, h3.x, h3.y, h3.z, h3.w};
+            float s[12];
+            if (own_fin) {
+                const float4 h1 = fin[own + 1], h2 = fin[own + 2], h3 = fin[own + 3];
+                s[0] = h1.x; s[1] = h1.y; s[2] = h1.z; s[3] = h1.w;
+                s[4] = h2.x; s[5] = h2.y; s[6] = h2.z; s[7] = h2.w;
+                s[8] = h3.x; s[9] = h3.y; s[10] = h3.z; s[11] = h3.w;
+            } else {
+#pragma unroll
+                for (int k = 0; k < 12; ++k) s[k] = own_col(4u + (uint32_t)k);
+            }
             live_terms<12, N1>(acc, s, W1 + 20 * N1, all);
         }
         live1 = bias_relu<N1>(acc, x1, b1);
     } else {
-        const float4 h0 = fin[(size_t)u * 4], h1 = fin[(size_t)u * 4 + 1], h2 = fin[(size_t)u * 4 + 2], h3 = fin[(size_t)u * 4 + 3];
+        float4 h0, h1, h2, h3;
+        if (own_fin) {
+            h0 = fin[(size_t)u * 4]; h1 = fin[(size_t)u * 4 + 1]; h2 = fin[(size_t)u * 4 + 2]; h3 = fin[(size_t)u * 4 + 3];
+        } else {
+            h0 = make_float4(own_col(0u), 0.0f, 0.0f, 0.0f);
+            h1 = make_float4(own_col(4u), own_col(5u), own_col(6u), own_col(7u));
+            h2 = make_float4(own_col(8u), own_col(9u), own_col(10u), own_col(11u));
+            h3 = make_float4(own_col(12u), own_col(13u), own_col(14u), own_col(15u));
+        }
         float x0[32];
 #pragma unroll
         for (int k = 0; k < 16; ++k) x0[k] = 0.0f;
@@ -823,7 +846,11 @@
         float *T = lds[threadIdx.x >> 6];
 #pragma unroll
         for (int j = 0; j < 16; ++j) T[lane * kOutPitch + j] = x3[j];
-        if (emit_counts) c4_emit_row(x3, &T[lane * kOutPitch], u, mine, lane, emit_spec, emit_table, emit_counts);
+        bool full = mine;
+        if (emit_counts) {
+            const bool in_table = c4_emit_row(x3, &T[lane * kOutPitch], u, mine, lane, emit_spec, emit_table, emit_counts);
+            if (sparse != 0u && in_table) full = false;
+        }
         wave_lds_sync();
         const int q = lane >> 2, c = lane & 3;
 #pragma unroll
@@ -832,7 +859,7 @@
             const float *src = &T[src_lane * kOutPitch + 4 * c];
             const float4 o = make_float4(src[0], src[1], src[2], src[3]);
             const uint32_t row = __shfl(u, src_lane);
-            if (__shfl((int)mine, src_lane)) reinterpret_cast<float4 *>(fout)[(size_t)row * 4 + c] = o;
+            if (__shfl((int)full, src_lane)) reinterpret_cast<float4 *>(fout)[(size_t)row * 4 + c] = o;
         }
     }
 }
@@ -1318,7 +1345,8 @@
         const float *__restrict__ acc_in, uint32_t long_thresh, int interleave,
         const uint32_t *__restrict__ acc_bad,
         const uint32_t *__restrict__ emit_spec, c4row *__restrict__ emit_table, unsigned long long *__restrict__ emit_counts,
-        const uint32_t *__restrict__ srt_vertex, const uint4 *__restrict__ srt_meta, uint32_t n_sorted, uint32_t skip) {
+        const uint32_t *__restrict__ srt_vertex, const uint4 *__restrict__ srt_meta, uint32_t n_sorted, uint32_t skip,
+        uint32_t sparse) {
     static_assert(!(SLIM && MFMA), "the matrix cores' input tile needs the full region");
     __shared__ __attribute__((aligned(16))) float lds[kWavesPerBlock][SLIM ? kSlimRegionFloats : kRegionFloats];
     const bool acc_full = acc_bad && *acc_bad == 0;
@@ -1428,7 +1456,10 @@
         dense_live<N2, N3, 0, true>(x2, x3, W3, b3, (skip & 4u) != 0, live2);
 #pragma unroll
         for (int j = 0; j < 16; ++j) T[lane * kOutPitch + j] = x3[j];
-        if (emit_counts) c4_emit_row(x3, &T[lane * kOutPitch], u, mine, lane, emit_spec, emit_table, emit_counts);
+        if (emit_counts) {
+            const bool in_table = c4_emit_row(x3, &T[lane * kOutPitch], u, mine, lane, emit_spec, emit_table, emit_counts);
+            if (sparse != 0u && in_table) mine = false;
+        }
     }
     wave_lds_sync();
 #pragma unroll
@@ -2869,9 +2900,24 @@
 constexpr uint32_t kC4Rounds = 64;
 static_assert(kC4SliceRows < kC4NoRow - 1u, "row field too narrow");
 
+__device__ __forceinline__ uint32_t c4_pack_cols(uint32_t p1, uint32_t p2, uint32_t p3, uint32_t p4) {
+    return (p1 < 16u ? p1 : 31u) | (p2 < 16u ? p2 : 31u) << 5 | (p3 < 16u ? p3 : 31u) << 10 | (p4 < 16u ? p4 : 31u) << 15;
+}
+__device__ __forceinline__ float4 c4_row_quarter(f32x4 t, uint32_t cols, uint32_t c) {
+    float q[4] = {0.0f, 0.0f, 0.0f, 0.0f};
+#pragma unroll
+    for (int k = 0; k < 4; ++k) {
+        const uint32_t col = cols >> (5 * k) & 31u;
+#pragma unroll
+        for (int i = 0; i < 4; ++i) q[i] = (col == 4u * c + (uint32_t)i) ? t[k] : q[i];
+    }
+    return make_float4(q[0], q[1], q[2], q[3]);
+}
+__device__ __forceinline__ bool c4_flagged(f32x4 t) { return (__float_as_uint(t[0]) >> 31) != 0; }
+
 __global__ __launch_bounds__(64) void k_c4_choose(unsigned long long *__restrict__ counts, int slots, uint32_t n,
                                                   uint32_t *__restrict__ desc, uint32_t max_passes, uint32_t *__restrict__ round_counts,
-                                                  uint32_t round_stride, int clear_counts) {
+                                                  uint32_t round_stride, int clear_counts, uint32_t sparse_in) {
     const int lane = threadIdx.x;
     unsigned long long mine = 0;
     if (slots == 1) {
@@ -2900,10 +2946,12 @@
     if (lane == 0) desc[5] = 0u;
     const bool prev_ok = desc[0] == 1u;
     const uint32_t p1 = desc[1], p2 = desc[2], p3 = desc[3], p4 = desc[4];
+    const bool sparse = sparse_in != 0u && slots > 1 && prev_ok && rows == n;
     if (rows != n) {
         if (lane == 0) {
             desc[0] = 0;
             desc[6] = 0;
+            desc[7] = 0;
         }
         return;
     }
@@ -2937,13 +2985,17 @@
     if (lane == 0) {
         desc[0] = np;
         desc[6] = (np && !table_written) ? 1u : 0u;
-    }
-}
-
-__global__ __launch_bounds__(256) void k_c4_compact(const float4 *__restrict__ feat, uint32_t n, uint32_t *__restrict__ desc,
-                                                    f32x4 *__restrict__ table) {
-    if (!desc[0] || !desc[6]) return;
-    const uint32_t npass = desc[0];
+        desc[7] = !sparse ? 0u : (table_written ? 1u : (2u | c4_pack_cols(p1, p2, p3, p4) << 8));
+    }
+}
+
+__global__ __launch_bounds__(256) void k_c4_compact(const float4 *feat, uint32_t n, uint32_t *__restrict__ desc,
+                                                    f32x4 *__restrict__ table, float4 *expand) {
+    const uint32_t sp = expand ? desc[7] : 0u;
+    const bool rewrite = desc[0] && desc[6];
+    if (!(sp & 2u) && !rewrite) return;
+    const uint32_t npass = rewrite ? desc[0] : 0u;
+    const uint32_t old_cols = sp >> 8;
     uint32_t mask = 0;
     for (uint32_t q = 0; q < npass; ++q)
         for (int k = 0; k < 4; ++k) {
@@ -2955,7 +3007,15 @@
         uint32_t nz = 0;
         float r[16];
         if (v < n) {
-            const float4 q0 = feat[v * 4], q1 = feat[v * 4 + 1], q2 = feat[v * 4 + 2], q3 = feat[v * 4 + 3];
+            float4 q0, q1, q2, q3;
+            const f32x4 told = (sp & 2u) ? table[v] : f32x4{-0.0f, 0.0f, 0.0f, 0.0f};
+            if (!c4_flagged(told)) {
+                q0 = c4_row_quarter(told, old_cols, 0u); q1 = c4_row_quarter(told, old_cols, 1u);
+                q2 = c4_row_quarter(told, old_cols, 2u); q3 = c4_row_quarter(told, old_cols, 3u);
+                expand[v * 4] = q0; expand[v * 4 + 1] = q1; expand[v * 4 + 2] = q2; expand[v * 4 + 3] = q3;
+            } else {
+                q0 = feat[v * 4]; q1 = feat[v * 4 + 1]; q2 = feat[v * 4 + 2]; q3 = feat[v * 4 + 3];
+            }
             const float rr[16] = {q0.x, q0.y, q0.z, q0.w, q1.x, q1.y, q1.z, q1.w, q2.x, q2.y, q2.z, q2.w, q3.x, q3.y, q3.z, q3.w};
 #pragma unroll
             for (int i = 0; i < 16; ++i) {
@@ -2968,11 +3028,12 @@
             f32x4 out = {0.0f, 0.0f, 0.0f, 0.0f};
             if (v < n) {
                 const uint32_t *dc = desc + (q == 0 ? 1 : 4 + 4 * q);
-                const float *row = reinterpret_cast<const float *>(feat) + v * 16;
 #pragma unroll
                 for (int k = 0; k < 4; ++k) {
                     const uint32_t cc = dc[k];
-                    const float a = cc < 16u ? row[cc] : 0.0f;
+                    float a = 0.0f;
+#pragma unroll
+                    for (int i = 0; i < 16; ++i) a = cc == (uint32_t)i ? r[i] : a;
                     out[k] = a == 0.0f ? 0.0f : a;
                 }
                 if (nz & ~mask) out[0] = __uint_as_float(__float_as_uint(out[0]) | 0x80000000u);
@@ -3168,27 +3229,55 @@
 
 __global__ __launch_bounds__(256) void k_c4_fix(GraphDev g, const float4 *__restrict__ fin, uint32_t *__restrict__ desc,
                                                 const uint32_t *__restrict__ dirty_rows, uint32_t dirty_cap,
-                                                float4 *__restrict__ agg16, const uint32_t *__restrict__ dirty_count, uint32_t slot_base) {
+                                                float4 *__restrict__ agg16, const uint32_t *__restrict__ dirty_count, uint32_t slot_base,
+                                                const f32x4 *__restrict__ table) {
     if (!desc[0]) return;
+    const bool sparse = table != nullptr && (desc[7] & 1u) != 0u;
+    const uint32_t cols = c4_pack_cols(desc[1], desc[2], desc[3], desc[4]);
     const uint32_t first = min(slot_base, dirty_cap);
     const uint32_t count = min(*dirty_count, dirty_cap);
     if (dirty_count != desc + 5 && blockIdx.x == 0 && threadIdx.x == 0) atomicAdd(&desc[5], *dirty_count - slot_base);
     const uint32_t c = threadIdx.x & 3;
+    auto quarter = [&](uint32_t v) -> float4 {
+        if (sparse) {
+            const f32x4 t = table[v];
+            if (!c4_flagged(t)) return c4_row_quarter(t, cols, c);
+        }
+        return fin[(size_t)v * 4 + c];
+    };
     for (uint32_t slot = first + ((blockIdx.x * blockDim.x + threadIdx.x) >> 2); slot < count; slot += (gridDim.x * blockDim.x) >> 2) {
         const uint32_t u = dirty_rows[slot];
         uint32_t e = g.rowptr[u];
         const uint32_t end = g.rowptr[u + 1];
         float4 a = make_float4(0.f, 0.f, 0.f, 0.f);
         for (; e + 1 < end; e += 2) {
-            const float4 r0 = fin[(size_t)g.col[e] * 4 + c], r1 = fin[(size_t)g.col[e + 1] * 4 + c];
+            const float4 r0 = quarter(g.col[e]), r1 = quarter(g.col[e + 1]);
             a.x += r0.x; a.y += r0.y; a.z += r0.z; a.w += r0.w;
             a.x += r1.x; a.y += r1.y; a.z += r1.z; a.w += r1.w;
         }
         if (e < end) {
-            const float4 r0 = fin[(size_t)g.col[e] * 4 + c];
+            const float4 r0 = quarter(g.col[e]);
             a.x += r0.x; a.y += r0.y; a.z += r0.z; a.w += r0.w;
         }
         agg16[(size_t)slot * 4 + c] = a;
+    }
+}
+
+__global__ __launch_bounds__(256) void k_c4_expand(float4 *__restrict__ feat, uint32_t n, const uint32_t *__restrict__ desc,
+                                                   const f32x4 *__restrict__ table, const unsigned long long *__restrict__ counts) {
+    if (desc[0] != 1u) return;
+    static_assert(kEmitSlots == 64, "one lane per slot");
+    unsigned long long rows = counts[(threadIdx.x & 63) * kEmitStride + 16];
+#pragma unroll
+    for (int off = 32; off; off >>= 1)
+        rows += ((unsigned long long)__shfl_xor((unsigned)(rows >> 32), off) << 32) | __shfl_xor((unsigned)rows, off);
+    if (rows != n) return;
+    const uint32_t cols = c4_pack_cols(desc[1], desc[2], desc[3], desc[4]);
+    for (size_t v = (size_t)blockIdx.x * blockDim.x + threadIdx.x; v < n; v += (size_t)gridDim.x * blockDim.x) {
+        const f32x4 t = table[v];
+        if (c4_flagged(t)) continue;
+#pragma unroll
+        for (uint32_t c = 0; c < 4; ++c) feat[v * 4 + c] = c4_row_quarter(t, cols, c);
     }
 }
 
@@ -4319,7 +4408,7 @@
     GNNVC_LAUNCH((k_dense_f16<32, 16, 1, true>), grid, block, 0, c.stream, *c.g, c.ws, reinterpret_cast<const float4 *>(c.in), c.out,
                        c.logits, c.params + c.sp->param_offset, c.row_lo, c.row_hi, reinterpret_cast<const float4 *>(s.acc4), s.c4desc,
                        reinterpret_cast<const float4 *>(s.agg16), reinterpret_cast<const float4 *>(s.table_in), long_thresh,
-                       (const uint32_t *)nullptr, (c4row *)nullptr, (unsigned long long *)nullptr, c.skip);
+                       (const uint32_t *)nullptr, (c4row *)nullptr, (unsigned long long *)nullptr, c.skip, 0u);
     return hipGetLastError();
 }
 
@@ -4347,14 +4436,14 @@
         GNNVC_LAUNCH((k_stage_f1<32, 32, 16, 4, false>), grid, block, 0, c.stream, g, c.ws, c.in, c.out, P,
                            c.row_lo, c.row_hi, g.rowptr, g.col, nofloat, a.long_thresh, il, (const uint32_t *)nullptr,
                            a.emit.spec, reinterpret_cast<c4row *>(a.emit.table), a.emit.counts, sorted ? so->vertex : nullptr,
-                           sorted ? reinterpret_cast<const uint4 *>(so->meta) : nullptr, sorted ? so->n : 0u, c.skip);
+                           sorted ? reinterpret_cast<const uint4 *>(so->meta) : nullptr, sorted ? so->n : 0u, c.skip, 0u);
         break;
     case 1:
         GNNVC_LAUNCH((k_stage_f1<32, 32, 16, 4, true>), grid, block, 0, c.stream, g, c.ws, c.in, c.out, P,
                            c.row_lo, c.row_hi, g.rowptr, g.col, nofloat, a.long_thresh, il, (const uint32_t *)nullptr,
                            (const uint32_t *)nullptr, (c4row *)nullptr, (unsigned long long *)nullptr,
                            sorted ? so->vertex : nullptr, sorted ? reinterpret_cast<const uint4 *>(so->meta) : nullptr,
-                           sorted ? so->n : 0u, c.skip);
+                           sorted ? so->n : 0u, c.skip, 0u);
         break;
 #ifndef GNNVC_GATHER_S
 #define GNNVC_GATHER_S 2
@@ -4421,7 +4510,8 @@
                 GNNVC_LAUNCH((k_dense_f16<32, 32, 16, false>), dgrid, block, 0, c.stream, g, c.ws, in4, c.out, (float *)nullptr, P, c.row_lo, c.row_hi,
                                    reinterpret_cast<const float4 *>(s.acc4), s.c4desc, reinterpret_cast<const float4 *>(s.agg16),
                                    reinterpret_cast<const float4 *>(s.table_in), a.long_thresh, a.emit.spec,
-                                   reinterpret_cast<c4row *>(a.emit.table), a.emit.counts, c.skip);
+                                   reinterpret_cast<c4row *>(a.emit.table), a.emit.counts, c.skip,
+                                   (a.sparse_out && a.emit.counts) ? 1u : 0u);
             }
         } else {
             if (a.mfma_agg) GNNVC_LAUNCH_AGG(16, 1, true, true, c.logits);
@@ -4629,12 +4719,12 @@
         GNNVC_LAUNCH((k_stage_f1<32, 32, 16, 4, true>), grid, block, 0, c.stream, g, c.ws, c.in, c.out,
                            c.params + sp.param_offset, c.row_lo, c.row_hi, ep, bp.colb, acc_in, a.long_thresh, a.interleave ? 1 : 0,
                            (const uint32_t *)nullptr, (const uint32_t *)nullptr, (c4row *)nullptr, (unsigned long long *)nullptr,
-                           (const uint32_t *)nullptr, (const uint4 *)nullptr, 0u, c.skip);
+                           (const uint32_t *)nullptr, (const uint4 *)nullptr, 0u, c.skip, 0u);
     else
         GNNVC_LAUNCH((k_stage_f1<32, 32, 16, 4, false>), grid, block, 0, c.stream, g, c.ws, c.in, c.out,
                            c.params + sp.param_offset, c.row_lo, c.row_hi, ep, bp.colb, acc_in, a.long_thresh, a.interleave ? 1 : 0,
                            (const uint32_t *)nullptr, a.emit.spec, reinterpret_cast<c4row *>(a.emit.table), a.emit.counts,
-                           (const uint32_t *)nullptr, (const uint4 *)nullptr, 0u, c.skip);
+                           (const uint32_t *)nullptr, (const uint4 *)nullptr, 0u, c.skip, (a.sparse_out && a.emit.counts) ? 1u : 0u);
     return hipGetLastError();
 }
 
@@ -4853,12 +4943,12 @@
         GNNVC_LAUNCH((k_stage_f1<32, 32, 16, 4, true>), grid, block, 0, c.stream, g, c.ws, c.in, c.out, c.params + sp.param_offset,
                            c.row_lo, c.row_hi, g.rowptr, g.col, acc, a.long_thresh, a.interleave ? 1 : 0, (const uint32_t *)bad,
                            (const uint32_t *)nullptr, (c4row *)nullptr, (unsigned long long *)nullptr,
-                           (const uint32_t *)nullptr, (const uint4 *)nullptr, 0u, c.skip);
+                           (const uint32_t *)nullptr, (const uint4 *)nullptr, 0u, c.skip, 0u);
     else
         GNNVC_LAUNCH((k_stage_f1<32, 32, 16, 4, false, GNNVC_STAGE0_SLIM != 0>), grid, block, 0, c.stream, g, c.ws, c.in, c.out, c.params + sp.param_offset,
                            c.row_lo, c.row_hi, g.rowptr, g.col, acc, a.long_thresh, a.interleave ? 1 : 0, (const uint32_t *)bad,
                            a.emit.spec, reinterpret_cast<c4row *>(a.emit.table), a.emit.counts,
-                           (const uint32_t *)nullptr, (const uint4 *)nullptr, 0u, c.skip);
+                           (const uint32_t *)nullptr, (const uint4 *)nullptr, 0u, c.skip, (a.sparse_out && a.emit.counts) ? 1u : 0u);
     return hipGetLastError();
 }
 
@@ -4872,15 +4962,17 @@
 hipError_t launch_compact_gather(const GraphDev &g, const CompactPlan &cp, const float *in, unsigned long long *counts,
                                  int count_slots, uint32_t *desc, float *table, float *acc4, uint32_t row_lo, uint32_t row_hi,
                                  uint32_t *dirty_rows, uint32_t dirty_cap, float *agg16, hipStream_t stream, int what,
-                                 uint32_t *round_counts, uint32_t round_stride, bool clear_counts) {
+                                 uint32_t *round_counts, uint32_t round_stride, bool clear_counts, float *sparse_rows) {
     if (row_hi <= row_lo || g.nnz == 0 || row_lo < cp.plan_base || row_hi > cp.plan_end) return hipErrorInvalidValue;
     if (cp.rows_per_chunk == 0 || cp.rows_per_chunk > kC4MaxRows || cp.rows_per_chunk % kC4Slices) return hipErrorInvalidValue;
     if (cp.max_passes < 1 || cp.max_passes > kC4MaxPasses) return hipErrorInvalidValue;
     if (what & 1) {
+        if (sparse_rows && sparse_rows != in) return hipErrorInvalidValue;
         GNNVC_LAUNCH(k_c4_choose, dim3(1), dim3(64), 0, stream, counts, count_slots, g.n, desc, cp.max_passes, round_counts,
-                     round_stride, clear_counts ? 1 : 0);
+                     round_stride, clear_counts ? 1 : 0, sparse_rows ? 1u : 0u);
         GNNVC_LAUNCH(k_c4_compact, dim3(std::min<unsigned>((g.n + 256) / 256, 4096u)), dim3(256), 0, stream,
-                           reinterpret_cast<const float4 *>(in), g.n, desc, reinterpret_cast<f32x4 *>(table));
+                           reinterpret_cast<const float4 *>(in), g.n, desc, reinterpret_cast<f32x4 *>(table),
+                           reinterpret_cast<float4 *>(sparse_rows));
     }
     if (!(what & 2)) return hipGetLastError();
     hipError_t rc0 = hipSuccess;
@@ -4888,13 +4980,13 @@
     if (rc0 != hipSuccess) return rc0;
     rc0 = compact_sums(g, cp, desc, table, acc4, row_lo, row_hi, dirty_rows, dirty_cap, stream);
     if (rc0 != hipSuccess) return rc0;
-    return compact_fix(g, in, desc, dirty_rows, dirty_cap, agg16, desc + 5, 0, stream);
+    return compact_fix(g, in, desc, dirty_rows, dirty_cap, agg16, desc + 5, 0, stream, 1024, sparse_rows ? table : nullptr);
 }
 
 hipError_t compact_choose(unsigned long long *counts, int count_slots, uint32_t rows, uint32_t *desc, uint32_t max_passes,
                           hipStream_t stream, bool clear_counts) {
     GNNVC_LAUNCH(k_c4_choose, dim3(1), dim3(64), 0, stream, counts, count_slots, rows, desc, max_passes, (uint32_t *)nullptr,
-                 0u, clear_counts ? 1 : 0);
+                 0u, clear_counts ? 1 : 0, 0u);
     return hipGetLastError();
 }
 
@@ -4935,10 +5027,20 @@
 }
 
 hipError_t compact_fix(const GraphDev &g, const float *in, uint32_t *desc, const uint32_t *dirty_rows, uint32_t dirty_cap,
-                       float *agg16, const uint32_t *dirty_count, uint32_t slot_base, hipStream_t stream, uint32_t blocks) {
+                       float *agg16, const uint32_t *dirty_count, uint32_t slot_base, hipStream_t stream, uint32_t blocks,
+                       const float *table) {
     GNNVC_LAUNCH(k_c4_fix, dim3(std::min<uint32_t>((dirty_cap + 63) / 64, blocks)), dim3(256), 0, stream, g,
                        reinterpret_cast<const float4 *>(in), desc, dirty_rows, dirty_cap, reinterpret_cast<float4 *>(agg16), dirty_count,
-                       slot_base);
+                       slot_base, reinterpret_cast<const f32x4 *>(table));
+    return hipGetLastError();
+}
+
+hipError_t compact_expand(float *rows, uint32_t n, const uint32_t *desc, const float *table, const unsigned long long *counts,
+                          hipStream_t stream) {
+    if (!rows || !desc || !table || !counts) return hipErrorInvalidValue;
+    if (!n) return hipSuccess;
+    GNNVC_LAUNCH(k_c4_expand, dim3(std::min<unsigned>((n + 255) / 256, 4096u)), dim3(256), 0, stream, reinterpret_cast<float4 *>(rows),
+                 n, desc, reinterpret_cast<const f32x4 *>(table), counts);
     return hipGetLastError();
 }
 
```

Result: no change. 25.68 billion (-0.6%).
